# yzslab/gaussian-splatting-lightning

Hardware: AMD Instinct MI355X
Metric: training images/sec + fwd/bwd ms @1080p, 1M Gaussians, 1/2/4/8 MI355X (higher is better)
Workload: dtype f32

## Files before the change

gaussian-splatting-lightning_amd/csrc/composite_bwd.hip:

```cpp
#include "gspl_composite.h"

namespace gspl {

template <int D> struct BwdRec { static constexpr int STRIDE = 8 + ((D + 1 + 3) & ~3); static constexpr int HC = 8 + D; };

#ifndef GSPL_BWD2_CHUNK
#define GSPL_BWD2_CHUNK 64
#endif
#ifndef GSPL_BWD2_WAVES
#define GSPL_BWD2_WAVES 5
#endif
static constexpr int B2CHUNK = GSPL_BWD2_CHUNK;
static constexpr int P2_SLOTS = 4;
static constexpr int B2_NW = 2;
static constexpr int B2_NT = 64 * B2_NW;
static_assert(B2CHUNK <= B2_NT || B2_NW == 2, "a round is staged by one pass of the workgroup's threads");


template <int D, int MODE, bool CHW, bool ABS, bool PACKED, int SEGM = 0>
__global__ __launch_bounds__(B2_NT, GSPL_BWD2_WAVES) void composite_bwd2_kernel(
    int n_tiles, int tile_w, int width, int height, int64_t n_isects,
    const float* __restrict__ means2d, const float* __restrict__ conics, const float* __restrict__ colors,
    const float* __restrict__ opacities, const float* __restrict__ backgrounds,
    const int32_t* __restrict__ offsets, const int32_t* __restrict__ flatten_ids,
    const float* __restrict__ final_Ts, const int32_t* __restrict__ last_ids,
    const float* __restrict__ v_out_colors, const float* __restrict__ v_out_alphas,
    float* __restrict__ v_means2d, float* __restrict__ v_means2d_abs,
    float* __restrict__ v_conics, float* __restrict__ v_colors, float* __restrict__ v_opacities, int packed_stride,
    uint8_t* __restrict__ hit_flags, SegState seg) {
    using TR = ModeTraits<MODE>;
    constexpr int NV = BwdVals<D, ABS>::N;
    constexpr int RS = BwdRec<D>::STRIDE;
    constexpr bool VO_REGS = D <= 4;
    constexpr int SLAB = 2 * P2_SLOTS * 128;
    static_assert(NV <= 16, "one ds_add round per batch");
    __shared__ int s_id[B2CHUNK];
    __shared__ __attribute__((aligned(16))) float s_rec[B2CHUNK * RS];
    __shared__ float s_acc[B2CHUNK * NV];
    __shared__ __attribute__((aligned(16))) float s_slab[B2_NW * SLAB];
    __shared__ __attribute__((aligned(16))) float s_vo_keep[VO_REGS ? 4 : B2_NW * 128 * D];
    static_assert(!VO_REGS || B2_NW * 128 * D <= B2_NW * SLAB, "s_vo alias too small");
    float* s_vo = VO_REGS ? s_slab : s_vo_keep;
    __shared__ int s_last;

    const int t = threadIdx.x, w = t >> 6, l = t & 63;
    const int ws = w;
    int tile = 0, segidx = 0;
    if constexpr (SEGM == 2) {
        if (blockIdx.x >= min(*seg.count(), seg.slots)) return;
        const uint32_t item = seg.work()[blockIdx.x];
        tile = (int)(item >> 8); segidx = (int)(item & 255u);
    } else {
        tile = xcd_remap(blockIdx.x, n_tiles);
    }
    {
    const int tx = (tile % tile_w) * TILE, ty = (tile / tile_w) * TILE;
    const int pxA = tx + (l & 7), pxB = pxA + 8;
    const int py = ty + w * 8 + (l >> 3);
    const bool insideA = (pxA < width) && (py < height), insideB = (pxB < width) && (py < height);
    const v2f pxf2 = {(float)pxA + TR::kPixelCentre, (float)pxB + TR::kPixelCentre};
    const float pyf = (float)py + TR::kPixelCentre;
    const float hx0 = (float)tx + TR::kPixelCentre;
    const float hy0 = (float)(ty + w * 8) + TR::kPixelCentre;
    const int64_t pixA = (int64_t)py * width + pxA, pixB = pixA + 8;
    const int tl = (l & 7) * 8 + (l >> 3);
    constexpr int TLB = 64;
    const int ps = l >> 4, pc = l & 15;
    float* slab = s_slab + ws * SLAB;

    int start, end;
    tile_range(tile, n_tiles, n_isects, offsets, start, end);

    const int lastA = insideA ? last_ids[pixA] : start, lastB = insideB ? last_ids[pixB] : start;
    v2f T2 = {insideA ? final_Ts[pixA] : 1.f, insideB ? final_Ts[pixB] : 1.f};
    v2f vo[D];
    v2f bgdot = {0.f, 0.f};
#pragma unroll
    for (int c = 0; c < D; ++c) {
        vo[c] = (v2f){0.f, 0.f};
        if (insideA) vo[c].x = CHW ? v_out_colors[(int64_t)c * width * height + pixA] : v_out_colors[pixA * D + c];
        if (insideB) vo[c].y = CHW ? v_out_colors[(int64_t)c * width * height + pixB] : v_out_colors[pixB * D + c];
        if (backgrounds) bgdot += backgrounds[c] * vo[c];
        s_vo[((ws * 16 + (l & 7)) * D + c) * 8 + (l >> 3)] = vo[c].x;
        s_vo[((ws * 16 + 8 + (l & 7)) * D + c) * 8 + (l >> 3)] = vo[c].y;
    }
    const v2f v_out_a = {(insideA && v_out_alphas) ? v_out_alphas[pixA] : 0.f, (insideB && v_out_alphas) ? v_out_alphas[pixB] : 0.f};
    v2f R2 = T2 * (v_out_a - bgdot);

    if (t == 0) s_last = start;
    for (int k = t; k < B2CHUNK * NV; k += B2_NT) s_acc[k] = 0.f;
    __syncthreads();
    v2f vo2[VO_REGS ? 4 : 1][VO_REGS ? D : 1];
    if constexpr (VO_REGS) {
#pragma unroll
        for (int c = 0; c < D; ++c) {
            const float4* vp = reinterpret_cast<const float4*>(s_vo + ((ws * 16 + pc) * D + c) * 8);
            const float4 v0 = vp[0], v1 = vp[1];
            vo2[0][c] = (v2f){v0.x, v0.y}; vo2[1][c] = (v2f){v0.z, v0.w};
            vo2[2][c] = (v2f){v1.x, v1.y}; vo2[3][c] = (v2f){v1.z, v1.w};
        }
    }
    int wl = max(lastA, lastB);
#pragma unroll
    for (int off = 32; off > 0; off >>= 1) wl = max(wl, __shfl_xor(wl, off));
    if (l == 0) atomicMax(&s_last, wl);
    __syncthreads();
    const int block_last = s_last;
    const int wave_last = wl;
    int seg_lo = start, seg_hi = block_last;
    if constexpr (SEGM != 2) {
        if (seg.walk && t == 0 && block_last > start) {
            uint32_t* row = seg.walk + (size_t)((unsigned)tile & (SEG_WALK_SLOTS - 1)) * 4u;
            atomicAdd(row + 0, (uint32_t)(block_last - start));
            atomicMax(row + 1, (uint32_t)(block_last - start));
            atomicAdd(row + 2, 1u);
        }
    }
    if constexpr (SEGM != 0) {
        const int walked = block_last - start;
        const int nseg = walked > 0 ? min((walked + SEG - 1) >> SEG_LOG2, SEG_MAX) : 0;
        if constexpr (SEGM == 1) {
            if (nseg > 1 && t == 0) {
                const uint32_t pos = atomicAdd(seg.count(), (uint32_t)(nseg - 1));
                for (int sgm = 1; sgm < nseg; ++sgm)
                    if (pos + (uint32_t)(sgm - 1) < seg.slots) seg.work()[pos + (uint32_t)(sgm - 1)] = ((uint32_t)tile << 8) | (uint32_t)sgm;
            }
        }
        if (nseg > 1) {
            seg_lo = start + segidx * SEG;
            seg_hi = (segidx + 1 < nseg) ? start + (segidx + 1) * SEG : block_last;
            if (seg_hi < block_last) {
                const size_t slot = (size_t)((unsigned)seg_hi >> SEG_LOG2) * 256u;
                const int lasts[2] = {lastA, lastB};
                float Tn[2] = {T2.x, T2.y}, Rn[2] = {R2.x, R2.y};
#pragma unroll
                for (int e = 0; e < 2; ++e) {
                    if (lasts[e] > seg_hi) {
                        const float4 ck = seg.ckpt[slot + (unsigned)((2 * w + e) * 64 + l)];
                        const float ckc[4] = {ck.y, ck.z, ck.w, D == 4 ? seg.ckpt_x[slot + (unsigned)((2 * w + e) * 64 + l)] : 0.f};
                        float behind = 0.f;
#pragma unroll
                        for (int c = 0; c < D; ++c) behind = fmaf(e == 0 ? vo[c].x : vo[c].y, ckc[c < 4 ? c : 0], behind);
                        Tn[e] = ck.x;
                        Rn[e] = Rn[e] - behind;
                    }
                }
                T2 = (v2f){Tn[0], Tn[1]}; R2 = (v2f){Rn[0], Rn[1]};
            }
        } else if (segidx > 0) {
            seg_lo = seg_hi = start;
        }
    }

    int nb = 0;
    int batch_j = 0;

    auto phase2 = [&](int count) {
        __builtin_amdgcn_wave_barrier();
        float vals[NV];
#pragma unroll
        for (int k = 0; k < NV; ++k) vals[k] = 0.f;
        const int j = __builtin_amdgcn_ds_bpermute(ps << 2, batch_j);
        const bool live = ps < count;
        float ca = 0.f, cb = 0.f, cc_ = 0.f, co_ = 1.f;
        if (live) {
            const float* rec = s_rec + j * RS;
            const float4 r0 = *reinterpret_cast<const float4*>(rec);
            const float4 r1 = *reinterpret_cast<const float4*>(rec + 4);
            ca = 2.f * r0.z; cb = r1.w; cc_ = 2.f * rec[BwdRec<D>::HC]; co_ = r1.y;
            const float dx = r0.x - (hx0 + (float)pc);
            const float dy0 = r0.y - hy0;
            const v2f dy0v = {dy0, dy0};
            const float4* Fp = reinterpret_cast<const float4*>(slab + ps * 128 + pc * 8);
            const float4* Sp = reinterpret_cast<const float4*>(slab + P2_SLOTS * 128 + ps * 128 + pc * 8);
            const float4 f0 = Fp[0], f1 = Fp[1], q0 = Sp[0], q1 = Sp[1];
            const v2f F2[4] = {{f0.x, f0.y}, {f0.z, f0.w}, {f1.x, f1.y}, {f1.z, f1.w}};
            const v2f S2[4] = {{q0.x, q0.y}, {q0.z, q0.w}, {q1.x, q1.y}, {q1.z, q1.w}};
            v2f s02 = {0.f, 0.f}, sy2 = {0.f, 0.f}, syy2 = {0.f, 0.f};
            v2f rgb2[D];
            float ax = 0.f, ay = 0.f;
#pragma unroll
            for (int c = 0; c < D; ++c) rgb2[c] = (v2f){0.f, 0.f};
#pragma unroll
            for (int k = 0; k < 4; ++k) {
                const v2f dy2 = dy0v - (v2f){(float)(2 * k), (float)(2 * k + 1)};
#pragma unroll
                for (int c = 0; c < D; ++c) {
                    v2f vv;
                    if constexpr (VO_REGS) vv = vo2[k][c];
                    else vv = *reinterpret_cast<const v2f*>(s_vo + ((ws * 16 + pc) * D + c) * 8 + 2 * k);
                    rgb2[c] = __builtin_elementwise_fma(F2[k], vv, rgb2[c]);
                }
                s02 += S2[k];
                const v2f tq = S2[k] * dy2;
                sy2 += tq;
                syy2 = __builtin_elementwise_fma(tq, dy2, syy2);
                if constexpr (ABS) {
                    ax += fabsf(S2[k].x * (ca * dx + cb * dy2.x)) + fabsf(S2[k].y * (ca * dx + cb * dy2.y));
                    ay += fabsf(S2[k].x * (cb * dx + cc_ * dy2.x)) + fabsf(S2[k].y * (cb * dx + cc_ * dy2.y));
                }
            }
            const float S0 = s02.x + s02.y, Sy = sy2.x + sy2.y;
            const float Sx = S0 * dx;
            vals[0] = ca * Sx + cb * Sy;
            vals[1] = cb * Sx + cc_ * Sy;
            vals[2] = 0.5f * (Sx * dx);
            vals[3] = Sy * dx;
            vals[4] = 0.5f * (syy2.x + syy2.y);
            vals[5] = (co_ != 0.f) ? -S0 * __builtin_amdgcn_rcpf(co_) : 0.f;
#pragma unroll
            for (int c = 0; c < D; ++c) vals[6 + c] = rgb2[c].x + rgb2[c].y;
            if constexpr (ABS) { vals[6 + D] = ax; vals[7 + D] = ay; }
        }
#pragma unroll
        for (int k = 0; k < NV; ++k) {
            vals[k] = dpp_add<0xB1, 0xF>(vals[k]);
            vals[k] = dpp_add<0x4E, 0xF>(vals[k]);
        }
        constexpr int NK = (NV + 3) / 4;
        const int pq = pc & 3;
        float kept[NK];
#pragma unroll
        for (int m = 0; m < NK; ++m) {
            float v = vals[4 * m];
#pragma unroll
            for (int q = 1; q < 4; ++q) v = (pq == q) ? ((4 * m + q < NV) ? vals[(4 * m + q < NV) ? 4 * m + q : 0] : 0.f) : v;
            kept[m] = dpp_add<0x124, 0xF>(v);
        }
        row_ror8_add<NK>(kept);
#pragma unroll
        for (int m = 0; m < NK; ++m)
            if (live && pc < 4 && 4 * m + pc < NV) atomicAdd(&s_acc[j * NV + 4 * m + pc], kept[m]);
    };

    int g_next = (seg_hi - 1 - t >= seg_lo && t < B2CHUNK) ? flatten_ids[seg_hi - 1 - t] : 0;
    for (int hi = seg_hi; hi > seg_lo; hi -= B2CHUNK) {
        const int lo = max(seg_lo, hi - B2CHUNK);
        const int cnt = hi - lo;
        const int g = g_next;
        {
            const int i_next = hi - B2CHUNK - 1 - t;
            if (i_next >= seg_lo && t < B2CHUNK) g_next = flatten_ids[i_next];
        }
        if (t < cnt) {
            s_id[t] = g;
            const float ca = conics[g * 3 + 0], cb = conics[g * 3 + 1], cc = conics[g * 3 + 2], op = opacities[g];
            const float mx = means2d[g * 2 + 0], my = means2d[g * 2 + 1];
            const unsigned qm = band_half_mask<2>(mx, my, ca, cb, cc, op, (float)tx + TR::kPixelCentre, (float)ty + TR::kPixelCentre);
            float* rec = s_rec + t * RS;
            const SigmaCoef sc = sigma_coef(ca, cb, cc);
            *reinterpret_cast<float4*>(rec) = make_float4(mx, my, sc.ha, sc.k);
            *reinterpret_cast<float4*>(rec + 4) = make_float4(sc.hd, op, __uint_as_float(qm), cb);
#pragma unroll
            for (int c = 0; c < D; ++c) rec[8 + c] = colors[(int64_t)g * D + c];
            rec[BwdRec<D>::HC] = 0.5f * cc;
        }
        __syncthreads();
        if (wave_last > lo) {
#pragma unroll 1
            for (int kk = 0; kk < (B2CHUNK + 63) / 64; ++kk) {
                const int slot = kk * 64 + l;
                const unsigned qm = (slot < B2CHUNK) ? __float_as_uint(s_rec[slot * RS + 6]) : 0u;
                const bool cand = (slot < cnt) && (hi - 1 - slot < wave_last) && ((qm >> (2 * w)) & 3u);
                unsigned long long mask = __ballot(cand);
                while (mask) {
                    const int j = kk * 64 + (int)__builtin_ctzll(mask);
                    mask &= mask - 1;
                    const int idx = hi - 1 - j;
                    const float* rec = s_rec + j * RS;
                    const float4 r0 = *reinterpret_cast<const float4*>(rec);
                    const float2 r1 = *reinterpret_cast<const float2*>(rec + 4);
                    float col[D];
#pragma unroll
                    for (int c = 0; c < D; ++c) col[c] = rec[8 + c];
                    const v2f dx2 = (v2f){r0.x, r0.x} - pxf2;
                    const float dy = r0.y - pyf;
                    const float e = (r1.x * dy) * dy;
                    const v2f u2 = __builtin_elementwise_fma((v2f){r0.w, r0.w}, (v2f){dy, dy}, dx2);
                    const v2f sigma2 = __builtin_elementwise_fma((v2f){r0.z, r0.z} * u2, u2, (v2f){e, e});
                    const v2f arg2 = sigma2 * (v2f){-1.4426950408889634f, -1.4426950408889634f};
                    const v2f vis2 = {__builtin_amdgcn_exp2f(arg2.x), __builtin_amdgcn_exp2f(arg2.y)};
                    const v2f raw2 = (v2f){r1.y, r1.y} * vis2;
                    const bool validA = (idx < lastA) && (sigma2.x >= 0.f) && (raw2.x >= kAlphaMin);
                    const bool validB = (idx < lastB) && (sigma2.y >= 0.f) && (raw2.y >= kAlphaMin);
                    if (!__any(validA || validB)) continue;
                    if (hit_flags && l == 0) atomicOr(&s_id[j], (int)0x80000000);
                    const v2f rv2 = {validA ? raw2.x : 0.f, validB ? raw2.y : 0.f};
                    const v2f a2 = {fminf(TR::kAlphaMax, rv2.x), fminf(TR::kAlphaMax, rv2.y)};
                    v2f rw2 = rv2;
                    if (TR::kClampKillsGrad) rw2 = (v2f){(rv2.x <= TR::kAlphaMax) ? rv2.x : 0.f, (rv2.y <= TR::kAlphaMax) ? rv2.y : 0.f};
                    const v2f om2 = (v2f){1.f, 1.f} - a2;
                    v2f ra2 = {__builtin_amdgcn_rcpf(om2.x), __builtin_amdgcn_rcpf(om2.y)};
                    ra2 = __builtin_elementwise_fma(ra2, __builtin_elementwise_fma(-om2, ra2, (v2f){1.f, 1.f}), ra2);
                    T2 *= ra2;
                    const v2f fac2 = a2 * T2;
                    v2f cdot2 = (v2f){col[0], col[0]} * vo[0];
#pragma unroll
                    for (int c = 1; c < D; ++c) cdot2 = __builtin_elementwise_fma((v2f){col[c], col[c]}, vo[c], cdot2);
                    const v2f v_alpha2 = __builtin_elementwise_fma(cdot2, T2, R2 * ra2);
                    R2 = __builtin_elementwise_fma(-cdot2, fac2, R2);
                    const v2f sp2 = -rw2 * v_alpha2;
                    float* F = slab + nb * 128 + tl;
                    F[0] = fac2.x; F[TLB] = fac2.y;
                    F[P2_SLOTS * 128] = sp2.x; F[P2_SLOTS * 128 + TLB] = sp2.y;
                    batch_j = gspl_writelane_i32(j, nb, batch_j);
                    if (++nb == P2_SLOTS) { phase2(P2_SLOTS); nb = 0; }
                }
            }
            if (nb) { phase2(nb); nb = 0; }
        }
        __syncthreads();
        if constexpr (PACKED) {
            float* __restrict__ v_packed = v_means2d;
            const bool by_entry = packed_stride < 0;
            const int ps = by_entry ? -packed_stride : packed_stride;
            for (int e = t; e < cnt * NV; e += B2_NT) {
                const float v = s_acc[e];
                s_acc[e] = 0.f;
                const int row = e / NV;
                const int64_t dst_row = by_entry ? (int64_t)(hi - 1 - row) : (int64_t)(s_id[row] & 0x7fffffff);
                if (v != 0.f) atomicAdd(&v_packed[dst_row * ps + (e - row * NV)], v);
            }
        } else if (t < cnt) {
            const int g = s_id[t] & 0x7fffffff;
            float v[NV];
            bool any_nz = false;
#pragma unroll
            for (int k = 0; k < NV; ++k) {
                v[k] = s_acc[t * NV + k];
                s_acc[t * NV + k] = 0.f;
                any_nz = any_nz || (v[k] != 0.f);
            }
            if (any_nz) {
                atomicAdd(&v_means2d[g * 2 + 0], v[0]);
                atomicAdd(&v_means2d[g * 2 + 1], v[1]);
                atomicAdd(&v_conics[g * 3 + 0], v[2]);
                atomicAdd(&v_conics[g * 3 + 1], v[3]);
                atomicAdd(&v_conics[g * 3 + 2], v[4]);
                atomicAdd(&v_opacities[g], v[5]);
#pragma unroll
                for (int c = 0; c < D; ++c) atomicAdd(&v_colors[(int64_t)g * D + c], v[6 + c]);
                if constexpr (ABS) {
                    atomicAdd(&v_means2d_abs[g * 2 + 0], v[6 + D]);
                    atomicAdd(&v_means2d_abs[g * 2 + 1], v[7 + D]);
                }
            }
        }
        if (hit_flags && t < cnt && s_id[t] < 0) hit_flags[s_id[t] & 0x7fffffff] = 1;
        __syncthreads();
    }
    }
}

template <int D, int MODE, bool CHW, bool ABS, bool PACKED>
__global__ __launch_bounds__(64) void composite_bwd_block_kernel(
    int n_tiles, int tile_w, int width, int height, int64_t n_isects,
    const float* __restrict__ means2d, const float* __restrict__ conics, const float* __restrict__ colors,
    const float* __restrict__ opacities, const float* __restrict__ backgrounds,
    const int32_t* __restrict__ offsets, const int32_t* __restrict__ flatten_ids,
    const float* __restrict__ final_Ts, const int32_t* __restrict__ last_ids,
    const float* __restrict__ v_out_colors, const float* __restrict__ v_out_alphas,
    float* __restrict__ v_means2d, float* __restrict__ v_means2d_abs,
    float* __restrict__ v_conics, float* __restrict__ v_colors, float* __restrict__ v_opacities, int packed_stride,
    uint8_t* __restrict__ hit_flags, ListTiles lt) {
    using TR = ModeTraits<MODE>;
    constexpr int NV = BwdVals<D, ABS>::N;
    __shared__ float s_x[64], s_y[64], s_ha[64], s_b[64], s_hc[64], s_op[64], s_k[64], s_hd[64];
    __shared__ float s_col[64 * D];
    __shared__ int s_g[64], s_idx[64];

    const int unit = xcd_remap(blockIdx.x, 4 * n_tiles, 4 * GSPL_XCD_RUN);
    const int tile = unit >> 2, w = unit & 3, l = threadIdx.x;
    const int bx = (tile % tile_w) * 2 + (w & 1), by = (tile / tile_w) * 2 + (w >> 1);
    const int px = bx * 8 + (l & 7), py = by * 8 + (l >> 3);
    const bool inside = (px < width) && (py < height);
    const float pxf = (float)px + TR::kPixelCentre, pyf = (float)py + TR::kPixelCentre;
    const float qx0 = (float)(bx * 8) + TR::kPixelCentre, qy0 = (float)(by * 8) + TR::kPixelCentre;
    int start, end;
    block_list_range(lt, bx, by, width, height, n_isects, offsets, start, end);

    const int64_t pix = (int64_t)py * width + px;
    const int last = inside ? last_ids[pix] : start;
    float T = inside ? final_Ts[pix] : 1.f;
    float vo[D];
    float bgdot = 0.f;
#pragma unroll
    for (int c = 0; c < D; ++c) {
        vo[c] = inside ? (CHW ? v_out_colors[(int64_t)c * width * height + pix] : v_out_colors[pix * D + c]) : 0.f;
        if (backgrounds) bgdot += backgrounds[c] * vo[c];
    }
    float R = T * (((inside && v_out_alphas) ? v_out_alphas[pix] : 0.f) - bgdot);
    int block_last = last;
#pragma unroll
    for (int off = 32; off > 0; off >>= 1) block_last = max(block_last, __shfl_xor(block_last, off));

    for (int hi = block_last; hi > start; hi -= 64) {
        const int idx = hi - 1 - l;
        bool cand = false;
        int g = 0;
        float mx = 0.f, my = 0.f, ca = 0.f, cb = 0.f, cc = 0.f, op = 0.f;
        if (idx >= start) {
            g = flatten_ids[idx];
            ca = conics[g * 3 + 0]; cb = conics[g * 3 + 1]; cc = conics[g * 3 + 2]; op = opacities[g];
            mx = means2d[g * 2 + 0]; my = means2d[g * 2 + 1];
            cand = box_reachable(mx, my, ca, cb, cc, op, qx0, qx0 + 7.f, qy0, qy0 + 7.f);
        }
        const unsigned long long mask = __ballot(cand);
        const int ncand = __builtin_popcountll(mask);
        const int slot = __builtin_amdgcn_mbcnt_hi((unsigned)(mask >> 32), __builtin_amdgcn_mbcnt_lo((unsigned)mask, 0u));
        __syncthreads();
        if (cand) {
            const SigmaCoef sc = sigma_coef(ca, cb, cc);
            s_x[slot] = mx; s_y[slot] = my; s_ha[slot] = sc.ha; s_b[slot] = cb; s_hc[slot] = 0.5f * cc; s_op[slot] = op;
            s_k[slot] = sc.k; s_hd[slot] = sc.hd;
            s_g[slot] = g; s_idx[slot] = idx;
#pragma unroll
            for (int c = 0; c < D; ++c) s_col[slot * D + c] = colors[(int64_t)g * D + c];
        }
        __syncthreads();
        for (int k = 0; k < ncand; ++k) {
            const int kidx = s_idx[k];
            const float ha = s_ha[k], b = s_b[k], hc = s_hc[k], o = s_op[k];
            const float dx = s_x[k] - pxf, dy = s_y[k] - pyf;
            const float sigma = eval_sigma(ha, s_k[k], s_hd[k], dx, dy);
            const float vis = __builtin_amdgcn_exp2f(sigma * -1.4426950408889634f);
            const float raw = o * vis;
            const bool valid = (kidx < last) && (sigma >= 0.f) && (raw >= kAlphaMin);
            if (!__any(valid)) continue;
            const float rv = valid ? raw : 0.f;
            const float a = fminf(TR::kAlphaMax, rv);
            float rw = rv;
            if (TR::kClampKillsGrad) rw = (rv <= TR::kAlphaMax) ? rv : 0.f;
            const float om = 1.f - a;
            float ra = __builtin_amdgcn_rcpf(om);
            ra = fmaf(ra, fmaf(-om, ra, 1.f), ra);
            T *= ra;
            const float fac = a * T;
            float cdot = s_col[k * D] * vo[0];
#pragma unroll
            for (int c = 1; c < D; ++c) cdot = fmaf(s_col[k * D + c], vo[c], cdot);
            const float v_alpha = fmaf(cdot, T, R * ra);
            R = fmaf(-cdot, fac, R);
            const float sp = -rw * v_alpha;
            const float fa = 2.f * ha, fc = 2.f * hc;
            float vals[NV];
            vals[0] = sp * fmaf(fa, dx, b * dy);
            vals[1] = sp * fmaf(b, dx, fc * dy);
            vals[2] = 0.5f * sp * dx * dx;
            vals[3] = sp * dx * dy;
            vals[4] = 0.5f * sp * dy * dy;
            vals[5] = (o != 0.f) ? -sp * __builtin_amdgcn_rcpf(o) : 0.f;
#pragma unroll
            for (int c = 0; c < D; ++c) vals[6 + c] = fac * vo[c];
            if constexpr (ABS) { vals[6 + D] = fabsf(vals[0]); vals[7 + D] = fabsf(vals[1]); }
#pragma unroll
            for (int v = 0; v < NV; ++v) vals[v] = wave_sum_to_lane63(vals[v]);
            if (l == 63) {
                const int gk = s_g[k];
                if constexpr (PACKED) {
                    float* row = v_means2d + (int64_t)gk * packed_stride;
#pragma unroll
                    for (int v = 0; v < NV; ++v) if (vals[v] != 0.f) atomicAdd(&row[v], vals[v]);
                } else {
                    atomicAdd(&v_means2d[gk * 2 + 0], vals[0]);
                    atomicAdd(&v_means2d[gk * 2 + 1], vals[1]);
                    atomicAdd(&v_conics[gk * 3 + 0], vals[2]);
                    atomicAdd(&v_conics[gk * 3 + 1], vals[3]);
                    atomicAdd(&v_conics[gk * 3 + 2], vals[4]);
                    atomicAdd(&v_opacities[gk], vals[5]);
#pragma unroll
                    for (int c = 0; c < D; ++c) atomicAdd(&v_colors[(int64_t)gk * D + c], vals[6 + c]);
                    if constexpr (ABS) {
                        atomicAdd(&v_means2d_abs[gk * 2 + 0], vals[6 + D]);
                        atomicAdd(&v_means2d_abs[gk * 2 + 1], vals[7 + D]);
                    }
                }
                if (hit_flags) hit_flags[gk] = 1;
            }
        }
    }
}

template <int D, int MODE, bool CHW, bool PACKED = false>
static int launch_bwd(bool absgrad, int n_tiles, int tile_w, ImageSize image, const CompositeSplats& sp, const TileLists& lists,
                      const float* final_Ts, const int32_t* last_ids,
                      const float* v_out_colors, const float* v_out_alphas,
                      float* v_means2d, float* v_means2d_abs, float* v_conics, float* v_colors, float* v_opacities,
                      hipStream_t s, int packed_stride, uint8_t* hit_flags, ListTiles lt, const SegState* seg_in = nullptr) {
#define GSPL_BWD_ARGS n_tiles, tile_w, image.width, image.height, lists.n_isects, sp.means2d, sp.conics, sp.colors, sp.opacities, sp.backgrounds, \
                      lists.offsets, lists.flatten_ids, final_Ts, last_ids, v_out_colors, v_out_alphas, v_means2d, v_means2d_abs, v_conics, v_colors, v_opacities,   \
                      packed_stride, hit_flags
    if (lt.log2 != 4) {
        if (absgrad) hipLaunchKernelGGL((composite_bwd_block_kernel<D, MODE, CHW, true, PACKED>), dim3(4 * n_tiles), dim3(64), 0, s, GSPL_BWD_ARGS, lt);
        else hipLaunchKernelGGL((composite_bwd_block_kernel<D, MODE, CHW, false, PACKED>), dim3(4 * n_tiles), dim3(64), 0, s, GSPL_BWD_ARGS, lt);
        return check_launch("composite_bwd");
    }
    SegState plain = {};
    if (seg_in) { plain.host_flag = seg_in->host_flag; plain.walk = seg_in->walk; }
    if constexpr ((D == 3 || (D == 4 && MODE == GSPL_MODE_INRIA)) && CHW && PACKED) {
        if (seg_in && seg_in->ckpt && (D == 3 || seg_in->ckpt_x) && !absgrad && packed_stride > 0) {
            hipLaunchKernelGGL((composite_bwd2_kernel<D, MODE, CHW, false, PACKED, 1>), dim3(n_tiles), dim3(B2_NT), 0, s, GSPL_BWD_ARGS, *seg_in);
            hipLaunchKernelGGL((composite_bwd2_kernel<D, MODE, CHW, false, PACKED, 2>), dim3(seg_in->slots), dim3(B2_NT), 0, s, GSPL_BWD_ARGS, *seg_in);
            return check_launch("composite_bwd(segmented)");
        }
    }
    if (absgrad) hipLaunchKernelGGL((composite_bwd2_kernel<D, MODE, CHW, true, PACKED>), dim3(n_tiles), dim3(B2_NT), 0, s, GSPL_BWD_ARGS, plain);
    else hipLaunchKernelGGL((composite_bwd2_kernel<D, MODE, CHW, false, PACKED>), dim3(n_tiles), dim3(B2_NT), 0, s, GSPL_BWD_ARGS, plain);
#undef GSPL_BWD_ARGS
    return check_launch("composite_bwd");
}

}

extern "C" int gspl_composite_bwd(int N, int64_t n_isects, int D, int mode, int layout,
                                  const float* means2d, const float* conics, const float* colors,
                                  const float* opacities, const float* backgrounds,
                                  int width, int height, int tile_size, int tile_w, int tile_h,
                                  const int32_t* offsets, const int32_t* flatten_ids,
                                  const float* final_Ts, const int32_t* last_ids,
                                  const float* v_out_colors, const float* v_out_alphas,
                                  float* v_means2d, float* v_means2d_abs,
                                  float* v_conics, float* v_colors, float* v_opacities, uint8_t* hit_flags, void* stream) {
    using namespace gspl;
    const ImageSize image{width, height};
    const TileGrid grid{tile_size, tile_w, tile_h};
    int rc = check_composite_args(N, n_isects, D, mode, layout, image, grid, "composite_bwd: bad argument");
    if (rc != GSPL_OK) return rc;
    if (n_isects == 0 || N == 0) return GSPL_OK;
    if (!means2d || !conics || !colors || !opacities || !offsets || !flatten_ids || !final_Ts || !last_ids ||
        !v_out_colors || !v_means2d || !v_conics || !v_colors || !v_opacities)
        return fail_arg("composite_bwd: NULL required pointer");
    const ListTiles lt = list_tiles(grid);
    const int ctw = (width + TILE - 1) / TILE, n_tiles = ctw * ((height + TILE - 1) / TILE);
    hipStream_t s = (hipStream_t)stream;
    const bool absgrad = v_means2d_abs != nullptr;
    return dispatch_composite(D, mode, layout, [&](auto d, auto m, auto chw) {
        return launch_bwd<d(), m(), chw()>(absgrad, n_tiles, ctw, image, CompositeSplats{means2d, conics, colors, opacities, backgrounds},
                                           TileLists{offsets, flatten_ids, n_isects}, final_Ts, last_ids, v_out_colors, v_out_alphas, v_means2d, v_means2d_abs, v_conics, v_colors, v_opacities, s, 0,
                                           hit_flags, lt);
    });
}

#include "gspl_sort.h"
namespace gspl {
static int g_deterministic = 0;

__global__ __launch_bounds__(256) void iota_ids_kernel(int64_t n, const int32_t* __restrict__ ids, uint32_t* __restrict__ keys, uint32_t* __restrict__ pos) {
    const int64_t i = (int64_t)blockIdx.x * 256 + threadIdx.x;
    if (i < n) { keys[i] = (uint32_t)ids[i]; pos[i] = (uint32_t)i; }
}
static constexpr int ORDERED_MAX_NV = 18;
__global__ __launch_bounds__(256) void ordered_reduce_kernel(int64_t n, const uint32_t* __restrict__ keys, const uint32_t* __restrict__ pos,
                                                             const float* __restrict__ entries, int nv, float* __restrict__ rows, int row_stride) {
    const int64_t i = (int64_t)blockIdx.x * 256 + threadIdx.x;
    if (i >= n) return;
    const uint32_t g = keys[i];
    if (i > 0 && keys[i - 1] == g) return;
    float acc[ORDERED_MAX_NV];
#pragma unroll
    for (int k = 0; k < ORDERED_MAX_NV; ++k) acc[k] = 0.f;
    for (int64_t j = i; j < n && keys[j] == g; ++j) {
        const float* row = entries + (int64_t)pos[j] * nv;
#pragma unroll
        for (int k = 0; k < ORDERED_MAX_NV; ++k) if (k < nv) acc[k] += row[k];
    }
    float* out = rows + (int64_t)g * row_stride;
#pragma unroll
    for (int k = 0; k < ORDERED_MAX_NV; ++k) if (k < nv) out[k] += acc[k];
}

OrderedScratch ordered_scratch(int N, int64_t n_isects, int nv) {
    OrderedScratch o;
    o.id_bits = 1;
    while (o.id_bits < 32 && (1ll << o.id_bits) < (long long)N) ++o.id_bits;
    o.sort_ws_bytes = gspl_radix_sort_workspace_bytes(n_isects, 4, 0, o.id_bits);
    Carve c;
    (void)c.take((size_t)n_isects * nv * sizeof(float));
    o.keys = c.take((size_t)n_isects * 4 * sizeof(uint32_t));
    o.sort_ws = c.take(o.sort_ws_bytes ? o.sort_ws_bytes : 16);
    o.total = c.off;
    return o;
}

int ordered_reduce(int N, int64_t n_isects, int nv, const int32_t* flatten_ids, void* block, float* rows, int row_stride, hipStream_t s, const char* who) {
    if (nv > ORDERED_MAX_NV) return fail_arg(who);
    const OrderedScratch o = ordered_scratch(N, n_isects, nv);
    uint32_t *k0 = (uint32_t*)((char*)block + o.keys), *k1 = k0 + n_isects, *p0 = k1 + n_isects, *p1 = p0 + n_isects;
    const unsigned grid = (unsigned)((n_isects + 255) / 256);
    hipLaunchKernelGGL(iota_ids_kernel, dim3(grid), dim3(256), 0, s, n_isects, flatten_ids, k0, p0);
    int which = 0;
    const int rc = gspl_radix_sort_pairs_u32(n_isects, k0, k1, p0, p1, 0, o.id_bits, &which, (char*)block + o.sort_ws, o.sort_ws_bytes, s);
    if (rc != GSPL_OK) return rc;
    hipLaunchKernelGGL(ordered_reduce_kernel, dim3(grid), dim3(256), 0, s, n_isects, which ? k1 : k0, which ? p1 : p0,
                       (const float*)block, nv, rows, row_stride);
    return check_launch(who);
}
}

extern "C" int gspl_set_deterministic(int on) { const int was = gspl::g_deterministic; gspl::g_deterministic = on ? 1 : 0; return was; }
extern "C" int gspl_get_deterministic(void) { return gspl::g_deterministic; }

extern "C" int gspl_composite_bwd_packed(int N, int64_t n_isects, int D, int mode, int layout,
                                         const float* means2d, const float* conics, const float* colors,
                                         const float* opacities, const float* backgrounds,
                                         int width, int height, int tile_size, int tile_w, int tile_h,
                                         const int32_t* offsets, const int32_t* flatten_ids,
                                         const float* final_Ts, const int32_t* last_ids,
                                         const float* v_out_colors, const float* v_out_alphas,
                                         float* v_packed, int packed_stride, int absgrad, uint8_t* hit_flags, void* stream) {
    using namespace gspl;
    return composite_bwd_packed_impl(N, D, mode, layout, CompositeSplats{means2d, conics, colors, opacities, backgrounds}, ImageSize{width, height},
                                     TileGrid{tile_size, tile_w, tile_h}, TileLists{offsets, flatten_ids, n_isects}, final_Ts, last_ids, v_out_colors,
                                     v_out_alphas, v_packed, packed_stride, absgrad, hit_flags, stream, nullptr);
}

int gspl::composite_bwd_packed_impl(int N, int D, int mode, int layout, const CompositeSplats& sp, ImageSize image, TileGrid grid, const TileLists& lists,
                                    const float* final_Ts, const int32_t* last_ids, const float* v_out_colors, const float* v_out_alphas,
                                    float* v_packed, int packed_stride, int absgrad, uint8_t* hit_flags, void* stream, const SegState* seg) {
    using namespace gspl;
    const int64_t n_isects = lists.n_isects;
    int rc = check_composite_args(N, n_isects, D, mode, layout, image, grid, "composite_bwd_packed: bad argument");
    if (rc != GSPL_OK) return rc;
    if (packed_stride < 6 + D + (absgrad ? 2 : 0)) return fail_arg("composite_bwd_packed: packed_stride smaller than the row");
    if (n_isects == 0 || N == 0) return GSPL_OK;
    if (!sp.means2d || !sp.conics || !sp.colors || !sp.opacities || !lists.offsets || !lists.flatten_ids || !final_Ts || !last_ids || !v_out_colors || !v_packed)
        return fail_arg("composite_bwd_packed: NULL required pointer");
    const ListTiles lt = list_tiles(grid);
    const int ctw = (image.width + TILE - 1) / TILE, n_tiles = ctw * ((image.height + TILE - 1) / TILE);
    hipStream_t s = (hipStream_t)stream;
    const bool ag = absgrad != 0;
    const int nv = 6 + D + (ag ? 2 : 0);
    const bool ordered = gspl_get_deterministic() != 0 && lt.log2 == 4 && n_isects > 0;
    float* entries = nullptr;
    float* const v_packed_out = v_packed;
    const int packed_stride_out = packed_stride;
    if (ordered) {
        if (n_isects < 0) return fail_arg("composite_bwd_packed: the deterministic mode needs the list length on the host (n_isects >= 0)");
        hipError_t e = hipMallocAsync((void**)&entries, ordered_scratch(N, n_isects, nv).total, s);
        if (e == hipSuccess) e = hipMemsetAsync(entries, 0, (size_t)n_isects * nv * sizeof(float), s);
        if (e != hipSuccess) return check_hip(e, "composite_bwd_packed(deterministic): scratch");
        v_packed = entries;
        packed_stride = -nv;
        seg = nullptr;
    }
    rc = dispatch_composite(D, mode, layout, [&](auto d, auto m, auto chw) {
        return launch_bwd<d(), m(), chw(), true>(ag, n_tiles, ctw, image, sp, lists,
                                                 final_Ts, last_ids, v_out_colors, v_out_alphas, v_packed, nullptr, nullptr, nullptr, nullptr, s, packed_stride,
                                                 hit_flags, lt, seg);
    });
    if (ordered) {
        if (rc == GSPL_OK) rc = ordered_reduce(N, n_isects, nv, lists.flatten_ids, entries, v_packed_out, packed_stride_out, s, "composite_bwd_packed(ordered reduce)");
        (void)hipFreeAsync(entries, s);
    }
    return rc;
}

extern "C" const char* gspl_composite_bwd_kernel_name(void) { return "composite_bwd2_kernel"; }
```

gaussian-splatting-lightning_amd/csrc/fused.hip:

```cpp
#include <cstdlib>
#include <cstring>
#include <mutex>
#include <unordered_map>
#include <utility>
#include <vector>
#include "gspl_composite.h"
#include "gspl_sort.h"

namespace gspl {

struct GeomLayout {
    size_t radii, means2d, depths, conics, colors, clamped, cov3d, sh_jac, order, cum, big_list, spans, opac, colors4, total;
};
static GeomLayout geom_layout(size_t n, bool invdepth = false) {
    GeomLayout g;
    Carve c;
    g.means2d = c.take(8 * n); g.depths = c.take(4 * n); g.conics = c.take(12 * n); g.colors = c.take(12 * n);
    g.clamped = c.take(3 * n); g.cov3d = c.take(24 * n); g.sh_jac = c.take(36 * n);
    g.order = c.take(4 * n); g.cum = c.take(8 * (n + 1)); g.big_list = c.take(4 * n); g.spans = c.take((size_t)GSPL_BIN_SPAN_BYTES * n);
    g.opac = c.take(4 * n);
    g.colors4 = invdepth ? c.take(16 * n) : 0;
    g.radii = 0;
    g.total = c.off;
    return g;
}
struct ImageLayout { size_t alphas, final_Ts, last_ids, offsets, total; };
static ImageLayout image_layout(size_t pixels, size_t tiles) {
    ImageLayout m;
    Carve c;
    m.alphas = c.take(4 * pixels); m.final_Ts = c.take(4 * pixels); m.last_ids = c.take(4 * pixels); m.offsets = c.take(4 * (tiles + 1));
    m.total = c.off;
    return m;
}

static bool wait_for_ticket(const int64_t* host, unsigned long long ticket, hipStream_t s) {
    const volatile unsigned long long* flag = (const volatile unsigned long long*)(host + 2);
    for (unsigned spins = 1;; ++spins) {
        if (__atomic_load_n((const unsigned long long*)flag, __ATOMIC_ACQUIRE) == ticket) return true;
        __builtin_ia32_pause();
        if ((spins & 0xffffu) == 0u) {
            const hipError_t q = hipStreamQuery(s);
            if (q == hipSuccess) return __atomic_load_n((const unsigned long long*)flag, __ATOMIC_ACQUIRE) == ticket;
            if (q != hipErrorNotReady) { (void)hipGetLastError(); return false; }
        }
    }
}
template <class T>
struct PerDevice {
    std::mutex mu;
    T slot[64] = {};
    bool ready[64] = {};
    template <class R, class Init, class F>
    R with(R fallback, Init&& init, F&& f) {
        int dev = 0;
        if (hipGetDevice(&dev) != hipSuccess || dev < 0 || dev >= 64) return fallback;
        std::lock_guard<std::mutex> lk(mu);
        if (!ready[dev]) {
            if (!init(slot[dev])) { (void)hipGetLastError(); return fallback; }
            ready[dev] = true;
        }
        return f(slot[dev]);
    }
};

static constexpr unsigned SEG_RING = 16;
struct SegAdaptive {
    uint32_t* ring = nullptr;
    uint32_t slot_ticket[SEG_RING] = {};
    uintptr_t slot_view[SEG_RING] = {};
    uint32_t next = 1;
    uintptr_t prev_view = 0;
    int sticky = 0;
    std::unordered_map<uintptr_t, uint8_t> verdict;
};
static PerDevice<SegAdaptive> g_seg;
static bool seg_decide(bool force, uintptr_t view, uint32_t** slot_out, uint32_t* ticket_out) {
    *slot_out = nullptr; *ticket_out = 0u;
    auto ring = [](SegAdaptive& a) {
        void* q = nullptr;
        if (hipHostMalloc(&q, SEG_RING * sizeof(uint32_t), hipHostMallocDefault) != hipSuccess) return false;
        a.ring = (uint32_t*)q;
        for (unsigned i = 0; i < SEG_RING; ++i) a.ring[i] = 0u;
        return true;
    };
    return g_seg.with(force, ring, [&](SegAdaptive& a) {
        for (unsigned i = 0; i < SEG_RING; ++i) {
            if (!a.slot_ticket[i]) continue;
            const uint32_t v = __atomic_load_n(a.ring + i, __ATOMIC_RELAXED);
            if ((v >> 1) != (a.slot_ticket[i] & 0x7fffffffu)) continue;
            const bool tail = (v & 1u) != 0u;
            if (a.slot_view[i]) {
                if (a.verdict.size() > 65536) a.verdict.clear();
                a.verdict[a.slot_view[i]] = tail ? 1 : 0;
            }
            if (tail) a.sticky = 64;
            a.slot_ticket[i] = 0u;
        }
        bool on = force;
        const auto it = view ? a.verdict.find(view) : a.verdict.end();
        if (it != a.verdict.end()) on = on || it->second != 0;
        else on = on || a.sticky > 0;
        if (a.sticky > 0) --a.sticky;
        const unsigned slot = a.next % SEG_RING;
        const uint32_t ticket = a.next & 0x7fffffffu;
        ++a.next; if ((a.next & 0x7fffffffu) == 0u) a.next = 1;
        a.slot_ticket[slot] = ticket;
        a.slot_view[slot] = a.prev_view;
        a.prev_view = view;
        *slot_out = a.ring + slot; *ticket_out = ticket;
        return on;
    });
}
static PerDevice<uint32_t*> g_seg_walk;
static uint32_t* seg_walk_words() {
    auto zeroed = [](uint32_t*& words) {
        void* q = nullptr;
        const size_t bytes = (size_t)SEG_WALK_SLOTS * 4 * sizeof(uint32_t);
        if (hipMalloc(&q, bytes) != hipSuccess || hipMemset(q, 0, bytes) != hipSuccess || hipDeviceSynchronize() != hipSuccess) {
            if (q) (void)hipFree(q);
            return false;
        }
        words = (uint32_t*)q;
        return true;
    };
    return g_seg_walk.with((uint32_t*)nullptr, zeroed, [](uint32_t* words) { return words; });
}

static unsigned long long next_ticket() {
    static thread_local unsigned long long t = 0ull;
    return ++t;
}

#ifndef GSPL_EVENT_FLAGS
#define GSPL_EVENT_FLAGS hipEventDisableTiming
#endif
struct FrameEvents { hipEvent_t geo = nullptr, col = nullptr, cnt = nullptr, fork = nullptr, filled = nullptr; bool ok = false; };
static FrameEvents& frame_events() {
    static thread_local FrameEvents ev;
    if (!ev.ok)
        ev.ok = hipEventCreateWithFlags(&ev.geo, GSPL_EVENT_FLAGS) == hipSuccess && hipEventCreateWithFlags(&ev.col, GSPL_EVENT_FLAGS) == hipSuccess &&
                hipEventCreateWithFlags(&ev.cnt, hipEventDisableTiming) == hipSuccess &&
                hipEventCreateWithFlags(&ev.fork, GSPL_EVENT_FLAGS) == hipSuccess && hipEventCreateWithFlags(&ev.filled, GSPL_EVENT_FLAGS) == hipSuccess;
    return ev;
}

static PerDevice<hipStream_t> g_low_priority_streams;
extern "C" void* gspl_low_priority_stream(void) {
    auto create = [](hipStream_t& st) {
        int least = 0, greatest = 0;
        (void)hipDeviceGetStreamPriorityRange(&least, &greatest);
        if (hipStreamCreateWithPriority(&st, hipStreamNonBlocking, least) == hipSuccess) return true;
        st = nullptr;
        return false;
    };
    return g_low_priority_streams.with((void*)nullptr, create, [](hipStream_t st) { return (void*)st; });
}

struct ProfSlot { std::vector<std::pair<hipEvent_t, hipEvent_t>> ev; };
static int g_prof_period[2] = {0, 0};
static unsigned g_prof_seen[2] = {0u, 0u};
static std::mutex g_prof_mu;
static ProfSlot g_prof[2];
struct ProfScope {
    int which; hipStream_t s; hipEvent_t a = nullptr, b = nullptr;
    ProfScope(int w, hipStream_t st) : which(w), s(st) {
        if (g_prof_period[w] <= 0) return;
        if ((g_prof_seen[w]++ % (unsigned)g_prof_period[w]) != 0u) return;
        if (hipEventCreate(&a) != hipSuccess || hipEventCreate(&b) != hipSuccess) { a = b = nullptr; return; }
        (void)hipEventRecord(a, s);
    }
    ~ProfScope() {
        if (!a) return;
        (void)hipEventRecord(b, s);
        std::lock_guard<std::mutex> lk(g_prof_mu);
        g_prof[which].ev.emplace_back(a, b);
    }
};

}

extern "C" int gspl_profile_enable2(int period_fwd, int period_bwd) {
    std::lock_guard<std::mutex> lk(gspl::g_prof_mu);
    gspl::g_prof_period[0] = period_fwd > 0 ? period_fwd : 0;
    gspl::g_prof_period[1] = period_bwd > 0 ? period_bwd : 0;
    gspl::g_prof_seen[0] = gspl::g_prof_seen[1] = 0u;
    for (auto& slot : gspl::g_prof) {
        for (auto& e : slot.ev) { (void)hipEventDestroy(e.first); (void)hipEventDestroy(e.second); }
        slot.ev.clear();
    }
    return GSPL_OK;
}

extern "C" int gspl_profile_enable(int period) { return gspl_profile_enable2(period, period); }

extern "C" int gspl_profile_read(int which, int* count, float* total_ms) {
    using namespace gspl;
    if (which < 0 || which > 1 || !count || !total_ms) return fail_arg("profile_read: bad argument");
    std::lock_guard<std::mutex> lk(g_prof_mu);
    float tot = 0.f;
    for (auto& e : g_prof[which].ev) {
        float ms = 0.f;
        if (hipEventSynchronize(e.second) != hipSuccess || hipEventElapsedTime(&ms, e.first, e.second) != hipSuccess) return check_hip(hipGetLastError(), "profile_read");
        tot += ms;
    }
    *count = (int)g_prof[which].ev.size();
    *total_ms = tot;
    return GSPL_OK;
}

extern "C" size_t gspl_rasterize_inria_geometry_bytes(int N) { return gspl::geom_layout((size_t)(N > 0 ? N : 1)).total; }
extern "C" size_t gspl_rasterize_inria_image_bytes(int width, int height) {
    return gspl::image_layout((size_t)width * height, (size_t)((width + 15) / 16) * ((height + 15) / 16)).total;
}

namespace gspl {

static void carve_inria_state(gspl_inria_state* st, char* geom, const GeomLayout& g, char* img, const ImageLayout& im) {
    st->means2d = (float*)(geom + g.means2d); st->depths = (float*)(geom + g.depths); st->conics = (float*)(geom + g.conics);
    st->colors = (float*)(geom + g.colors); st->clamped = (uint8_t*)(geom + g.clamped); st->cov3d = (float*)(geom + g.cov3d);
    st->sh_jac = (float*)(geom + g.sh_jac);
    st->alphas = (float*)(img + im.alphas); st->final_Ts = (float*)(img + im.final_Ts); st->last_ids = (int32_t*)(img + im.last_ids);
    st->offsets = (int32_t*)(img + im.offsets);
}

struct TicketWait {
    const int64_t* host; hipStream_t s;
    const unsigned long long ticket = next_ticket();
    bool waited = false, arrived = false;
    TicketWait(const int64_t* h, hipStream_t st) : host(h), s(st) {}
    TicketWait(const TicketWait&) = delete;
    bool wait() {
        if (!waited) { arrived = wait_for_ticket(host, ticket, s); waited = true; }
        return arrived;
    }
    ~TicketWait() { (void)wait(); }
};
static int list_length_never_arrived(hipStream_t s) {
    const char* what = "rasterize_inria_fwd: the list length never arrived";
    return check_hip(hipStreamSynchronize(s), what) ? GSPL_ERR_LAUNCH : fail_arg(what);
}

struct SegPlan {
    bool adaptive = false, want = false;
    uint32_t* verdict_slot = nullptr;
    uint32_t verdict_ticket = 0u;
    uint4* packed_zero = nullptr;
    uint32_t packed_n16 = 0u;
    SegState seg = {};
    void ask_packed_rows(size_t row_bytes, gspl_alloc_fn alloc, void* alloc_ctx, gspl_inria_state* st) {
        const size_t bytes = (row_bytes + 15) & ~(size_t)15;
        packed_zero = (uint4*)alloc(alloc_ctx, GSPL_BUF_PACKED, bytes);
        if (packed_zero && bytes / 16 <= 0xffffffffull) { packed_n16 = (uint32_t)(bytes / 16); st->flags |= GSPL_INRIA_PACKED_READY; }
        else packed_zero = nullptr;
    }
    const SegState* for_capacity(int64_t cap, bool invd, gspl_alloc_fn alloc, void* alloc_ctx, gspl_inria_state* st) {
        seg = SegState{};
        seg.zero_p = packed_zero; seg.zero_n16 = packed_n16;
        if (adaptive) { seg.walk = seg_walk_words(); seg.host_flag = verdict_slot; seg.ticket = verdict_ticket; }
        st->seg_ckpt = nullptr; st->seg_words = nullptr; st->seg_slots = 0u;
        if (!want || cap <= SEG) return (adaptive || packed_zero) ? &seg : nullptr;
        const uint32_t slots = (uint32_t)(cap >> SEG_LOG2) + 2u;
        const size_t words = 2 + (size_t)slots;
        const size_t head = up256(words * sizeof(uint32_t));
        char* blk = (char*)alloc(alloc_ctx, GSPL_BUF_CHECKPOINTS, head + (size_t)slots * 256 * (sizeof(float4) + (invd ? sizeof(float) : 0)));
        if (!blk) return (adaptive || packed_zero) ? &seg : nullptr;
        uint32_t* wds = (uint32_t*)blk;
        seg.words = wds; seg.slots = slots;
        seg.ckpt = (float4*)(blk + head);
        seg.ckpt_x = invd ? (float*)(seg.ckpt + (size_t)slots * 256) : nullptr;
        st->seg_ckpt = seg.ckpt; st->seg_words = wds; st->seg_slots = slots;
        return &seg;
    }
};

static int inria_colours_launch(int N, const InriaParams& p, const InriaCamera& cam, const float* colors_precomp, int32_t* radii, gspl_inria_state* st,
                                float* colors3, hipStream_t s, hipStream_t ss, hipEvent_t* ev_col) {
    FrameEvents& fe = frame_events();
    if (!fe.ok) return check_hip(hipGetLastError(), "rasterize_inria_fwd: event");
    const bool side = ss && ss != s;
    if (side) {
        (void)hipEventRecord(fe.geo, s);
        (void)hipStreamWaitEvent(ss, fe.geo, 0);
    }
    hipStream_t cs = side ? ss : s;
    int rc = gspl_inria_preprocess_fwd(N, p.degree, p.n_coeffs, p.means, p.scales, p.quats, p.cov3d, p.shs, p.shs_rest, colors_precomp, cam.viewmatrix,
                                       cam.projmatrix, cam.campos, cam.width, cam.height, 16, cam.tanfovx, cam.tanfovy, cam.scale_modifier, radii, st->means2d,
                                       st->depths, st->conics, colors3, st->clamped, st->cov3d, st->sh_jac, GSPL_INRIA_COLOURS, cs);
    if (rc == GSPL_OK && (st->flags & GSPL_INRIA_INVDEPTH)) rc = inria_invdepth_rows_launch(N, radii, colors3, st->depths, st->colors, cs);
    if (rc == GSPL_OK && side) { (void)hipEventRecord(fe.col, cs); *ev_col = fe.col; }
    return rc;
}

static int inria_composite_launch(int N, int D, const gspl_inria_state* st, const float* bg, int64_t n_isects, float* out_color,
                                  hipEvent_t ev_col, hipStream_t s, const SegState* sg) {
    if (ev_col) (void)hipStreamWaitEvent(s, ev_col, 0);
    ProfScope prof(0, s);
    return composite_fwd_impl(N, D, GSPL_MODE_INRIA, GSPL_LAYOUT_CHW, CompositeSplats{st->means2d, st->conics, st->colors, st->opacities, bg},
                              ImageSize{st->width, st->height}, tile_grid16(st->width, st->height), TileLists{st->offsets, st->flatten_ids, n_isects},
                              out_color, st->alphas, st->final_Ts, st->last_ids, nullptr, s, sg);
}

}

extern "C" int gspl_rasterize_inria_fwd(
    int N, int degree, int n_coeffs,
    const float* means3D, const float* scales, const float* rotations, const float* cov3D_precomp,
    const float* shs, const float* shs_rest, const float* colors_precomp, const float* opacities,
    const float* viewmatrix, const float* projmatrix, const float* campos, const float* bg,
    int width, int height, float tanfovx, float tanfovy, float scale_modifier,
    gspl_alloc_fn alloc, void* alloc_ctx, int64_t capacity_hint,
    float* out_color, int32_t* radii, gspl_inria_state* st, void* stream, void* side_stream) {
    using namespace gspl;
    const char* no_block = "rasterize_inria_fwd: allocation call-back returned NULL";
    if (N < 0 || width <= 0 || height <= 0 || !alloc || !st || !out_color) return fail_arg("rasterize_inria_fwd: bad argument");
    if (N > 0 && (!means3D || !opacities || !radii || !viewmatrix || !projmatrix || !campos)) return fail_arg("rasterize_inria_fwd: NULL required pointer");
    const TileGrid grid = tile_grid16(width, height);
    hipStream_t s = (hipStream_t)stream, ss = (hipStream_t)side_stream;
    const int flags = st->flags;
    if (flags & ~(GSPL_INRIA_RAW_PARAMS | GSPL_INRIA_NO_SEGMENTS | GSPL_INRIA_FORCE_SEGMENTS | GSPL_INRIA_WILL_BACKWARD | GSPL_INRIA_ANTIALIAS |
                  GSPL_INRIA_INVDEPTH)) return fail_arg("rasterize_inria_fwd: unknown state->flags (zero the struct before the call)");
    const bool raw = (flags & GSPL_INRIA_RAW_PARAMS) != 0;
    const bool aa = (flags & GSPL_INRIA_ANTIALIAS) != 0, invd = (flags & GSPL_INRIA_INVDEPTH) != 0;
    const int D = invd ? 4 : 3;
    const int prow = invd ? 10 : 9;
    if (raw && (cov3D_precomp || (N > 0 && (!scales || !rotations)))) return fail_arg("rasterize_inria_fwd: raw parameters need scales and rotations");
    memset(st, 0, sizeof(*st));
    st->flags = flags;
    st->N = N; st->width = width; st->height = height;
    const size_t n = (size_t)(N > 0 ? N : 1);
    const GeomLayout g = geom_layout(n, invd);
    const ImageLayout im = image_layout((size_t)width * height, (size_t)grid.n());
    char* geom = (char*)alloc(alloc_ctx, GSPL_BUF_GEOMETRY, g.total);
    char* img = (char*)alloc(alloc_ctx, GSPL_BUF_IMAGE, im.total);
    if (!geom || !img) return fail_arg(no_block);
    carve_inria_state(st, geom, g, img, im);
    float* colors3 = st->colors;
    if (invd) st->colors = (float*)(geom + g.colors4);
    const float* raw_opacities = (raw || aa) ? opacities : nullptr;
    if (raw || aa) opacities = (float*)(geom + g.opac);
    st->opacities = const_cast<float*>(opacities);
    SegPlan plan;
    plan.adaptive = !(flags & GSPL_INRIA_NO_SEGMENTS) && gspl_get_deterministic() == 0;
    plan.want = plan.adaptive && seg_decide((flags & GSPL_INRIA_FORCE_SEGMENTS) != 0, (uintptr_t)viewmatrix, &plan.verdict_slot, &plan.verdict_ticket);
    if ((flags & GSPL_INRIA_WILL_BACKWARD) && N > 0) plan.ask_packed_rows((size_t)N * prow * sizeof(float), alloc, alloc_ctx, st);
    const BinSplats bins{N, GSPL_MODE_INRIA, st->means2d, radii, st->depths, st->conics, opacities};
    const BinOrder ord{(int32_t*)(geom + g.order), (int64_t*)(geom + g.cum), (int32_t*)(geom + g.big_list), geom + g.spans};
    if (N == 0) {
        const int rc = bin_lists_known(BinSplats{0, GSPL_MODE_INRIA}, BinOrder{}, grid, 0, alloc, alloc_ctx, &st->flatten_ids, st->offsets, s, "rasterize_inria_fwd");
        return rc != GSPL_OK ? rc : inria_composite_launch(N, D, st, bg, 0, out_color, nullptr, s, nullptr);
    }
    const size_t ws1_bytes = gspl_bin_workspace_bytes(N, 0);
    char* ws1 = (char*)alloc(alloc_ctx, GSPL_BUF_BINNING, ws1_bytes);
    if (!ws1) return fail_arg(no_block);
    const int64_t capacity = capacity_hint > 0 ? capacity_hint : 0;
    const size_t ws2_bytes = capacity ? gspl_bin_workspace_bytes(N, capacity) : 0;
    char* ws2 = capacity ? (char*)alloc(alloc_ctx, GSPL_BUF_LISTS_WORK, ws2_bytes) : nullptr;
    if (capacity && !ws2) return fail_arg(no_block);
    int64_t* host = pinned_words();
    if (!host) return fail_arg("rasterize_inria_fwd: no pinned host word");
    if (!viewmatrix || !projmatrix) return fail_arg("rasterize_inria_fwd: NULL required pointer");
    if (!cov3D_precomp && (!scales || !rotations)) return fail_arg("rasterize_inria_fwd: need scales+rotations or cov3D_precomp");
    ZeroJob zero_depth, zero_tile;
    int rc = bin_depth_header(N, grid.n(), ws1, zero_depth);
    if (rc == GSPL_OK && ws2) rc = bin_tile_header(N, capacity, grid.n(), ws2, zero_tile);
    if (rc != GSPL_OK) return rc;
    const InriaParams params{means3D, scales, rotations, cov3D_precomp, shs, shs_rest, degree, n_coeffs};
    const InriaCamera cam{viewmatrix, projmatrix, campos, width, height, tanfovx, tanfovy, scale_modifier};
    rc = inria_geometry_launch(N, params, cam, grid.size, radii, st->means2d, st->depths, st->conics, st->cov3d, raw_opacities, st->opacities, s, zero_depth,
                               flags & (GSPL_INRIA_RAW_PARAMS | GSPL_INRIA_ANTIALIAS));
    if (rc != GSPL_OK) return rc;
    hipEvent_t ev_col = nullptr;
    rc = inria_colours_launch(N, params, cam, colors_precomp, radii, st, colors3, s, ss, &ev_col);
    if (rc != GSPL_OK) return rc;
    TicketWait scan(host, s);
    rc = bin_count_ticket(bins, grid, ord, host, ws1, ws1_bytes, s, scan.ticket, true, zero_tile);
    if (rc != GSPL_OK) return rc;
    int64_t n_isects = 0;
    if (ws2) {
        rc = bin_emit_impl(bins, ord, grid, capacity, ws2, ws2_bytes, s, true);
        if (rc != GSPL_OK) return rc;
        st->flatten_ids = (int32_t*)alloc(alloc_ctx, GSPL_BUF_LISTS, 4 * (size_t)capacity);
        if (!st->flatten_ids) return fail_arg(no_block);
        const SegState* sg = plan.for_capacity(capacity, invd, alloc, alloc_ctx, st);
        rc = gspl_bin_sort_device_count(N, grid.w, grid.h, ord.cum + (N - 1), capacity, st->flatten_ids, st->offsets, ws2, ws2_bytes, s);
        if (rc != GSPL_OK) return rc;
        rc = inria_composite_launch(N, D, st, bg, -1, out_color, ev_col, s, sg);
        const bool arrived = scan.wait();
        n_isects = host[0];
        if (rc != GSPL_OK) return rc;
        if (!arrived) return list_length_never_arrived(s);
        if (n_isects <= capacity) { st->n_isects = n_isects; return GSPL_OK; }
    } else {
        if (!scan.wait()) return list_length_never_arrived(s);
        n_isects = host[0];
    }
    rc = bin_lists_known(bins, ord, grid, n_isects, alloc, alloc_ctx, &st->flatten_ids, st->offsets, s, "rasterize_inria_fwd");
    if (rc != GSPL_OK) return rc;
    st->n_isects = n_isects;
    return inria_composite_launch(N, D, st, bg, n_isects, out_color, ev_col, s, plan.for_capacity(n_isects, invd, alloc, alloc_ctx, st));
}

namespace gspl {
#ifndef GSPL_FILL_BLOCKS
#define GSPL_FILL_BLOCKS 32
#endif
static int fill_blocks() {
    static const int n = [] { const char* e = getenv("GSPL_FILL_BLOCKS"); const int v = e ? atoi(e) : 0; return v > 0 && v <= 65536 ? v : GSPL_FILL_BLOCKS; }();
    return n;
}
struct FillJob {
    struct Span { float* p; uint64_t n; } a[9];
    int count = 0;
    void add(float* p, uint64_t n) { if (p && n) a[count++] = Span{p, n}; }
};
__global__ __launch_bounds__(256) void zero_fill_kernel(FillJob job) {
    typedef float v4f __attribute__((ext_vector_type(4)));
    const uint64_t tid = (uint64_t)blockIdx.x * 256 + threadIdx.x, stride = (uint64_t)gridDim.x * 256;
    for (int k = 0; k < job.count; ++k) {
        float* p = job.a[k].p;
        const uint64_t n = job.a[k].n;
        const uint64_t head = min(n, (uint64_t)(((16u - (unsigned)((uintptr_t)p & 15u)) & 15u) >> 2));
        const uint64_t n4 = (n - head) >> 2, tail0 = head + (n4 << 2);
        v4f* q = reinterpret_cast<v4f*>(p + head);
        const v4f z = {0.f, 0.f, 0.f, 0.f};
        for (uint64_t i = tid; i < n4; i += stride) __builtin_nontemporal_store(z, q + i);
        if (tid < head) p[tid] = 0.f;
        if (tid < n - tail0) p[tail0 + tid] = 0.f;
    }
}
struct FillJoin {
    hipStream_t s; hipEvent_t ev = nullptr;
    explicit FillJoin(hipStream_t st) : s(st) {}
    FillJoin(const FillJoin&) = delete;
    void join() { if (ev) (void)hipStreamWaitEvent(s, ev, 0); ev = nullptr; }
    ~FillJoin() { join(); }
};
static int zero_grads_beside(int N, const InriaParams& p, const InriaGrads& v, hipStream_t s, FillJoin& fill) {
    FillJob job;
    const uint64_t n = (uint64_t)N, sh_rows = (uint64_t)(p.n_coeffs > 0 ? p.n_coeffs : 0);
    job.add(v.means, 3 * n); job.add(v.means2d_ndc, 3 * n); job.add(v.opacities, n);
    job.add(v.scales, 3 * n); job.add(v.quats, 4 * n); job.add(v.cov3d_precomp, 6 * n); job.add(v.colors_precomp, 3 * n);
    if (v.shs_rest) { job.add(v.shs, 3 * n); job.add(v.shs_rest, 3 * (sh_rows > 0 ? sh_rows - 1 : 0) * n); }
    else job.add(v.shs, 3 * sh_rows * n);
    FrameEvents& fe = frame_events();
    if (!fe.ok) return check_hip(hipGetLastError(), "rasterize_inria_bwd: event");
    hipStream_t ls = (hipStream_t)gspl_low_priority_stream();
    const bool side = ls && ls != s;
    if (side) {
        (void)hipEventRecord(fe.fork, s);
        (void)hipStreamWaitEvent(ls, fe.fork, 0);
    }
    hipLaunchKernelGGL(zero_fill_kernel, dim3(fill_blocks()), dim3(256), 0, side ? ls : s, job);
    const int rc = check_launch("rasterize_inria_bwd: clear the gradients");
    if (side) { (void)hipEventRecord(fe.filled, ls); fill.ev = fe.filled; }
    return rc;
}

static int rasterize_inria_bwd_impl(InriaParams p, const float* opacities, InriaCamera cam, const float* bg,
                                    const int32_t* radii, const gspl_inria_state* st, const float* v_out_color,
                                    float* packed , uint8_t* hit_flags,
                                    const InriaGrads& v, void* stream, const gspl_bwd_adam_plan* plan, uint8_t* grad_rows = nullptr) {
    if (!st || st->N < 0) return fail_arg("rasterize_inria_bwd: bad state");
    const int N = st->N;
    if (N == 0) return GSPL_OK;
    if (!packed || !v_out_color || !v.means || !v.means2d_ndc || !v.opacities) return fail_arg("rasterize_inria_bwd: NULL required pointer");
    cam.width = st->width; cam.height = st->height;
    p.cov3d = st->cov3d;
    hipStream_t s = (hipStream_t)stream;
    hipError_t e = hipSuccess;
    const bool aa = (st->flags & GSPL_INRIA_ANTIALIAS) != 0, invd = (st->flags & GSPL_INRIA_INVDEPTH) != 0;
    const int D = invd ? 4 : 3, prow = invd ? 10 : 9;
    const float* caller_opacities = opacities;
    FillJoin fill(s);
    if (grad_rows) {
        if (plan) return fail_arg("rasterize_inria_bwd: grad_rows and the optimizer inside the backward exclude each other");
        const int rc = zero_grads_beside(N, p, v, s, fill);
        if (rc != GSPL_OK) return rc;
    }
    if (!(st->flags & GSPL_INRIA_PACKED_READY)) {
        e = hipMemsetAsync(packed, 0, (size_t)N * prow * sizeof(float), s);
        if (e != hipSuccess) return check_hip(e, "rasterize_inria_bwd: clear");
    }
    if (hit_flags) {
        e = hipMemsetAsync(hit_flags, 0, (size_t)N, s);
        if (e != hipSuccess) return check_hip(e, "rasterize_inria_bwd: clear");
    }
    const bool raw = (st->flags & GSPL_INRIA_RAW_PARAMS) != 0;
    if (raw) {
        if (!st->opacities || !v.scales || !v.quats) return fail_arg("rasterize_inria_bwd: raw parameters need the forward's state, v_scales and v_rotations");
        opacities = st->opacities;
    }
    if (aa) {
        if (!st->opacities) return fail_arg("rasterize_inria_bwd: anti-aliasing needs the forward's state");
        opacities = st->opacities;
    }
    if (st->n_isects > 0) {
        SegState seg = {};
        if (st->seg_ckpt && st->seg_words) {
            seg.ckpt = (float4*)st->seg_ckpt;
            seg.words = st->seg_words; seg.slots = st->seg_slots;
            if (invd) seg.ckpt_x = (float*)(seg.ckpt + (size_t)seg.slots * 256);
        }
        if (!(st->flags & GSPL_INRIA_NO_SEGMENTS) && gspl_get_deterministic() == 0) seg.walk = seg_walk_words();
        ProfScope prof(1, s);
        const int rc = composite_bwd_packed_impl(N, D, GSPL_MODE_INRIA, GSPL_LAYOUT_CHW, CompositeSplats{st->means2d, st->conics, st->colors, opacities, bg},
                                                 ImageSize{cam.width, cam.height}, tile_grid16(cam.width, cam.height),
                                                 TileLists{st->offsets, st->flatten_ids, st->n_isects}, st->final_Ts, st->last_ids, v_out_color, nullptr,
                                                 packed, prow, 0, hit_flags, s, &seg);
        if (rc != GSPL_OK) return rc;
    }
    fill.join();
    return inria_preprocess_bwd_impl(N, p, cam, radii, st->clamped, SplatGradRows::packed(packed, prow), v, st->sh_jac,
                                     aa ? caller_opacities : (raw ? st->opacities : nullptr), s, plan, BwdStats{st->stats_accum, st->stats_denom, st->stats_max_radii},
                                     st->flags & (GSPL_INRIA_RAW_PARAMS | GSPL_INRIA_ANTIALIAS | GSPL_INRIA_INVDEPTH), grad_rows);
}
}

extern "C" int gspl_rasterize_inria_bwd(
    int degree, int n_coeffs,
    const float* means3D, const float* scales, const float* rotations, const float* shs, const float* shs_rest, const float* opacities,
    const float* viewmatrix, const float* projmatrix, const float* campos, const float* bg,
    float tanfovx, float tanfovy, float scale_modifier,
    const int32_t* radii, const gspl_inria_state* st, const float* v_out_color,
    float* packed, uint8_t* hit_flags,
    float* v_means3D, float* v_means2D_ndc, float* v_shs, float* v_shs_rest, float* v_colors_precomp, float* v_opacities,
    float* v_scales, float* v_rotations, float* v_cov3D, void* stream) {
    using namespace gspl;
    return rasterize_inria_bwd_impl(InriaParams{means3D, scales, rotations, nullptr, shs, shs_rest, degree, n_coeffs}, opacities,
                                    InriaCamera{viewmatrix, projmatrix, campos, 0, 0, tanfovx, tanfovy, scale_modifier}, bg, radii, st, v_out_color, packed, hit_flags,
                                    InriaGrads{v_means3D, v_scales, v_rotations, v_cov3D, v_shs, v_shs_rest, v_colors_precomp, v_means2D_ndc, v_opacities}, stream, nullptr);
}

extern "C" int gspl_rasterize_inria_bwd_sparse(
    int degree, int n_coeffs,
    const float* means3D, const float* scales, const float* rotations, const float* shs, const float* shs_rest, const float* opacities,
    const float* viewmatrix, const float* projmatrix, const float* campos, const float* bg,
    float tanfovx, float tanfovy, float scale_modifier,
    const int32_t* radii, const gspl_inria_state* st, const float* v_out_color,
    float* packed, uint8_t* hit_flags,
    float* v_means3D, float* v_means2D_ndc, float* v_shs, float* v_shs_rest, float* v_colors_precomp, float* v_opacities,
    float* v_scales, float* v_rotations, float* v_cov3D, uint8_t* grad_rows, void* stream) {
    using namespace gspl;
    if (!grad_rows) return fail_arg("rasterize_inria_bwd_sparse: NULL grad_rows");
    return rasterize_inria_bwd_impl(InriaParams{means3D, scales, rotations, nullptr, shs, shs_rest, degree, n_coeffs}, opacities,
                                    InriaCamera{viewmatrix, projmatrix, campos, 0, 0, tanfovx, tanfovy, scale_modifier}, bg, radii, st, v_out_color, packed, hit_flags,
                                    InriaGrads{v_means3D, v_scales, v_rotations, v_cov3D, v_shs, v_shs_rest, v_colors_precomp, v_means2D_ndc, v_opacities}, stream, nullptr,
                                    grad_rows);
}

extern "C" int gspl_rasterize_inria_bwd_adam(
    int degree, int n_coeffs,
    float* means3D, float* scales, float* rotations, float* shs, float* shs_rest, float* opacities,
    const float* viewmatrix, const float* projmatrix, const float* campos, const float* bg,
    float tanfovx, float tanfovy, float scale_modifier,
    const int32_t* radii, const gspl_inria_state* st, const float* v_out_color,
    float* packed, uint8_t* hit_flags, float* scratch_means, float* v_means2D_ndc, const gspl_bwd_adam_plan* plan, void* stream) {
    using namespace gspl;
    if (!plan) return fail_arg("rasterize_inria_bwd_adam: NULL plan");
    if (!scales || !rotations || !shs || !opacities) return fail_arg("rasterize_inria_bwd_adam: needs scales, rotations, SH coefficients and opacities");
    if (st && (st->flags & (GSPL_INRIA_ANTIALIAS | GSPL_INRIA_INVDEPTH)))
        return fail_arg("rasterize_inria_bwd_adam: a frame rendered with GSPL_INRIA_ANTIALIAS or GSPL_INRIA_INVDEPTH takes gspl_rasterize_inria_bwd and a separate optimizer");
    return rasterize_inria_bwd_impl(InriaParams{means3D, scales, rotations, nullptr, shs, shs_rest, degree, n_coeffs}, opacities,
                                    InriaCamera{viewmatrix, projmatrix, campos, 0, 0, tanfovx, tanfovy, scale_modifier}, bg, radii, st, v_out_color, packed, hit_flags,
                                    InriaGrads{scratch_means, scales, rotations, nullptr, shs, shs_rest, nullptr, v_means2D_ndc, opacities}, stream, plan);
}
```

gaussian-splatting-lightning_amd/csrc/gspl_composite.h:

```cpp
#pragma once
#include "gspl_device.h"
#include "gspl_host.h"

namespace gspl {

static constexpr int TILE = 16;

typedef float v2f __attribute__((ext_vector_type(2)));

struct SigmaCoef { float ha, k, hd; };
__device__ __forceinline__ SigmaCoef sigma_coef(float a, float b, float c) {
    SigmaCoef s;
    s.ha = 0.5f * a;
    if (a != 0.f) {
        s.k = b / a;
        s.hd = (0.5f * conic_det(a, b, c)) * __builtin_amdgcn_rcpf(a);
    } else {
        s.k = 0.f;
        s.hd = (b == 0.f) ? 0.5f * c : __builtin_nanf("");
    }
    return s;
}
__device__ __forceinline__ float eval_sigma(float ha, float k, float hd, float dx, float dy) {
    const float u = fmaf(k, dy, dx);
    return fmaf(ha * u, u, (hd * dy) * dy);
}

__device__ __forceinline__ v2f eval_sigma2(v2f ha, v2f k, v2f hd, v2f dx, v2f dy) {
    const v2f u = __builtin_elementwise_fma(k, dy, dx);
    return __builtin_elementwise_fma(ha * u, u, (hd * dy) * dy);
}

__device__ __forceinline__ bool box_reachable(float mx, float my, float a, float b, float c, float opacity,
                                              float x0, float x1, float y0, float y1) {
    const float tau = __logf(255.f * opacity) * 1.0002f + 2e-4f;
    if (!(tau > 0.f)) return false;
    const float det = conic_det(a, b, c);
    if (!(det > 0.f) || !(a > 0.f) || !(c > 0.f)) return true;
    const float two_tau = 2.f * tau;
    const float rdet = __builtin_amdgcn_rcpf(det);
    const float hy = __builtin_amdgcn_sqrtf(two_tau * a * rdet) * 1.0004f + 1e-3f;
    float lo = y0 - my, hi = y1 - my;
    if (hi < -hy || lo > hy) return false;
    lo = fmaxf(lo, -hy); hi = fminf(hi, hy);
    const float tta = two_tau * a;
    const float rlo = __builtin_amdgcn_sqrtf(fmaxf(0.f, tta - det * lo * lo));
    const float rhi = __builtin_amdgcn_sqrtf(fmaxf(0.f, tta - det * hi * hi));
    const float hx = __builtin_amdgcn_sqrtf(two_tau * c * rdet);
    const float dys = b * __builtin_amdgcn_sqrtf(two_tau * rdet * __builtin_amdgcn_rcpf(c));
    const float inv_a = __builtin_amdgcn_rcpf(a);
    const float right = (-dys >= lo && -dys <= hi) ? hx : fmaxf((-b * lo + rlo) * inv_a, (-b * hi + rhi) * inv_a);
    const float left = (dys >= lo && dys <= hi) ? -hx : fminf((-b * lo - rlo) * inv_a, (-b * hi - rhi) * inv_a);
    const float eps = 2e-3f + 5e-4f * hx;
    return (mx + right + eps >= x0) && (mx + left - eps <= x1);
}

template <int BANDS>
__device__ __forceinline__ unsigned band_half_mask(float mx, float my, float a, float b, float c, float opacity, float tx0, float ty0) {
    constexpr float BH = (float)(TILE / BANDS);
    const float tau = __logf(255.f * opacity) * 1.0002f + 2e-4f;
    if (!(tau > 0.f)) return 0u;
    const float det = conic_det(a, b, c);
    if (!(det > 0.f) || !(a > 0.f) || !(c > 0.f)) return (1u << (2 * BANDS)) - 1u;
    const float two_tau = 2.f * tau;
    const float rdet = __builtin_amdgcn_rcpf(det);
    const float hy = __builtin_amdgcn_sqrtf(two_tau * a * rdet) * 1.0004f + 1e-3f;
    const float tta = two_tau * a;
    const float hx = __builtin_amdgcn_sqrtf(two_tau * c * rdet);
    const float dys = b * __builtin_amdgcn_sqrtf(two_tau * rdet * __builtin_amdgcn_rcpf(c));
    const float inv_a = __builtin_amdgcn_rcpf(a);
    const float eps = 2e-3f + 5e-4f * hx;
    unsigned m = 0u;
#pragma unroll
    for (int band = 0; band < BANDS; ++band) {
        const float y0 = ty0 + BH * (float)band;
        float lo = y0 - my, hi = (y0 + (BH - 1.f)) - my;
        if (hi < -hy || lo > hy) continue;
        lo = fmaxf(lo, -hy); hi = fminf(hi, hy);
        const float rlo = __builtin_amdgcn_sqrtf(fmaxf(0.f, tta - det * lo * lo));
        const float rhi = __builtin_amdgcn_sqrtf(fmaxf(0.f, tta - det * hi * hi));
        const float right = (-dys >= lo && -dys <= hi) ? hx : fmaxf((-b * lo + rlo) * inv_a, (-b * hi + rhi) * inv_a);
        const float left = (dys >= lo && dys <= hi) ? -hx : fminf((-b * lo - rlo) * inv_a, (-b * hi - rhi) * inv_a);
        const float xr = mx + right + eps, xl = mx + left - eps;
        if (xr >= tx0 && xl <= tx0 + 7.f) m |= 1u << (2 * band);
        if (xr >= tx0 + 8.f && xl <= tx0 + 15.f) m |= 2u << (2 * band);
    }
    return m;
}

#ifndef GSPL_SEG_LOG2
#define GSPL_SEG_LOG2 8
#endif
static constexpr int SEG_LOG2 = GSPL_SEG_LOG2;
static constexpr int SEG = 1 << SEG_LOG2;
static constexpr int SEG_TRIGGER = 3 * SEG;
static constexpr int SEG_TAIL_X2 = 9;
static constexpr int SEG_WALK_SLOTS = 64;
static constexpr int SEG_MAX = 255;
struct SegState {
    float4* ckpt;
    uint32_t* words;
    uint32_t* host_flag;
    uint32_t ticket;
    uint32_t* walk;
    uint4* zero_p;
    uint32_t zero_n16;
    uint32_t slots;
    float* ckpt_x;
    __host__ __device__ uint32_t* count() const { return words; }
    __host__ __device__ uint32_t* work() const { return words + 2; }
};

__device__ __forceinline__ void tile_range(int tile, int n_tiles, int64_t n_isects,
                                           const int32_t* __restrict__ offsets, int& start, int& end) {
    start = offsets[tile];
    end = (tile + 1 < n_tiles || n_isects < 0) ? offsets[tile + 1] : (int)n_isects;
}

struct ListTiles {
    int log2;
    int w;
    int n;
};
static inline ListTiles list_tiles(TileGrid grid) {
    ListTiles lt;
    lt.log2 = grid.size == 8 ? 3 : (grid.size == 32 ? 5 : 4);
    lt.w = grid.w;
    lt.n = grid.n();
    return lt;
}
__device__ __forceinline__ void block_list_range(const ListTiles& lt, int bx, int by, int width, int height, int64_t n_isects,
                                                 const int32_t* __restrict__ offsets, int& start, int& end) {
    if (bx * 8 >= width || by * 8 >= height) { start = end = 0; return; }
    const int t = (by >> (lt.log2 - 3)) * lt.w + (bx >> (lt.log2 - 3));
    start = offsets[t];
    end = (t + 1 < lt.n || n_isects < 0) ? offsets[t + 1] : (int)n_isects;
}

template <int D, bool ABS> struct BwdVals { static constexpr int N = 6 + D + (ABS ? 2 : 0); };

struct CompositeSplats { const float* means2d; const float* conics; const float* colors; const float* opacities; const float* backgrounds; };
struct ImageSize { int width, height; };
struct TileLists { const int32_t* offsets; const int32_t* flatten_ids; int64_t n_isects; };

int check_composite_args(int N, int64_t n_isects, int D, int mode, int layout, ImageSize image, TileGrid grid, const char* who);

int composite_fwd_impl(int N, int D, int mode, int layout, const CompositeSplats& splats, ImageSize image, TileGrid grid, const TileLists& lists,
                       float* out_colors, float* out_alphas, float* final_Ts, int32_t* last_ids, uint8_t* hit_flags, void* stream, const SegState* seg);
int composite_bwd_packed_impl(int N, int D, int mode, int layout, const CompositeSplats& splats, ImageSize image, TileGrid grid, const TileLists& lists,
                              const float* final_Ts, const int32_t* last_ids, const float* v_out_colors, const float* v_out_alphas,
                              float* v_packed, int packed_stride, int absgrad, uint8_t* hit_flags, void* stream, const SegState* seg);

template <class F>
static int dispatch_composite(int D, int mode, int layout, F&& f) {
    auto with_d = [&](auto mode_c, auto chw_c) -> int {
        switch (D) {
            case 1: return f(std::integral_constant<int, 1>{}, mode_c, chw_c);
            case 2: return f(std::integral_constant<int, 2>{}, mode_c, chw_c);
            case 3: return f(std::integral_constant<int, 3>{}, mode_c, chw_c);
            case 4: return f(std::integral_constant<int, 4>{}, mode_c, chw_c);
            case 8: return f(std::integral_constant<int, 8>{}, mode_c, chw_c);
        }
        return GSPL_ERR_UNSUPPORTED;
    };
    return dispatch_bools([&](auto inria, auto chw) { return with_d(std::integral_constant<int, decltype(inria)::value ? GSPL_MODE_INRIA : GSPL_MODE_GSPLAT>{}, chw); },
                          mode != GSPL_MODE_GSPLAT, layout != GSPL_LAYOUT_HWC);
}

struct OrderedScratch { size_t keys, sort_ws, sort_ws_bytes, total; int id_bits; };
OrderedScratch ordered_scratch(int N, int64_t n_isects, int nv);
int ordered_reduce(int N, int64_t n_isects, int nv, const int32_t* flatten_ids, void* block, float* rows, int row_stride, hipStream_t s, const char* who);

}
```

gaussian-splatting-lightning_amd/csrc/gspl_device.h:

```cpp
#pragma once
#include <hip/hip_runtime.h>
#include <stdint.h>

#include "../../include/gspl_hip.h"

namespace gspl {

template <int MODE> struct ModeTraits;
template <> struct ModeTraits<GSPL_MODE_GSPLAT> {
    static constexpr float kAlphaMax = 0.999f;
    static constexpr float kPixelCentre = 0.5f;
    static constexpr bool kStopInclusive = true;
    static constexpr bool kClampKillsGrad = true;
};
template <> struct ModeTraits<GSPL_MODE_INRIA> {
    static constexpr float kAlphaMax = 0.99f;
    static constexpr float kPixelCentre = 0.0f;
    static constexpr bool kStopInclusive = false;
    static constexpr bool kClampKillsGrad = false;
};
static constexpr float kAlphaMin = 1.0f / 255.0f;
static constexpr float kTStop = 1e-4f;

template <int MODE>
// ... 61 lines not shown
    float tx, ty;
    bool  in_x, in_y;
    float ux, uy;
};

__device__ __forceinline__ void ewa_fwd(const float pc[3], const float S6[6], const float W[9],
                                        float fx, float fy, float limx, float limy,
                                        float& a0, float& b0, float& c0, EwaCtx& ctx) {
    const float z = pc[2];
    const float rz = 1.f / z;
    const float txtz = pc[0] * rz, tytz = pc[1] * rz;
    ctx.in_x = (txtz >= -limx) && (txtz <= limx);
    ctx.in_y = (tytz >= -limy) && (tytz <= limy);
    ctx.ux = fminf(limx, fmaxf(-limx, txtz));
    ctx.uy = fminf(limy, fmaxf(-limy, tytz));
    ctx.tx = ctx.ux * z;
    ctx.ty = ctx.uy * z;
    const float J00 = fx * rz, J02 = -fx * ctx.tx * rz * rz;
    const float J11 = fy * rz, J12 = -fy * ctx.ty * rz * rz;
#pragma unroll
    for (int j = 0; j < 3; ++j) {
        ctx.T0[j] = J00 * W[0 * 3 + j] + J02 * W[2 * 3 + j];
        ctx.T1[j] = J11 * W[1 * 3 + j] + J12 * W[2 * 3 + j];
    }
    const float s0x = S6[0] * ctx.T0[0] + S6[1] * ctx.T0[1] + S6[2] * ctx.T0[2];
    const float s0y = S6[1] * ctx.T0[0] + S6[3] * ctx.T0[1] + S6[4] * ctx.T0[2];
    const float s0z = S6[2] * ctx.T0[0] + S6[4] * ctx.T0[1] + S6[5] * ctx.T0[2];
    const float s1x = S6[0] * ctx.T1[0] + S6[1] * ctx.T1[1] + S6[2] * ctx.T1[2];
    const float s1y = S6[1] * ctx.T1[0] + S6[3] * ctx.T1[1] + S6[4] * ctx.T1[2];
    const float s1z = S6[2] * ctx.T1[0] + S6[4] * ctx.T1[1] + S6[5] * ctx.T1[2];
    a0 = ctx.T0[0] * s0x + ctx.T0[1] * s0y + ctx.T0[2] * s0z;
    b0 = ctx.T0[0] * s1x + ctx.T0[1] * s1y + ctx.T0[2] * s1z;
    c0 = ctx.T1[0] * s1x + ctx.T1[1] * s1y + ctx.T1[2] * s1z;
}

template <bool EXACT_CLAMP>
__device__ __forceinline__ void ewa_bwd(const float pc[3], const float S6[6], const float W[9],
                                        float fx, float fy, const EwaCtx& ctx,
                                        float va, float vb, float vc,
                                        float v_pc[3], float G6[6]) {
    const float* T0 = ctx.T0;
    const float* T1 = ctx.T1;
    const float hb = 0.5f * vb;
    G6[0] = va * T0[0] * T0[0] + vb * T0[0] * T1[0] + vc * T1[0] * T1[0];
    G6[3] = va * T0[1] * T0[1] + vb * T0[1] * T1[1] + vc * T1[1] * T1[1];
    G6[5] = va * T0[2] * T0[2] + vb * T0[2] * T1[2] + vc * T1[2] * T1[2];
    G6[1] = va * T0[0] * T0[1] + hb * (T0[0] * T1[1] + T1[0] * T0[1]) + vc * T1[0] * T1[1];
    G6[2] = va * T0[0] * T0[2] + hb * (T0[0] * T1[2] + T1[0] * T0[2]) + vc * T1[0] * T1[2];
    G6[4] = va * T0[1] * T0[2] + hb * (T0[1] * T1[2] + T1[1] * T0[2]) + vc * T1[1] * T1[2];

    const float s0[3] = {S6[0] * T0[0] + S6[1] * T0[1] + S6[2] * T0[2],
                         S6[1] * T0[0] + S6[3] * T0[1] + S6[4] * T0[2],
                         S6[2] * T0[0] + S6[4] * T0[1] + S6[5] * T0[2]};
    const float s1[3] = {S6[0] * T1[0] + S6[1] * T1[1] + S6[2] * T1[2],
                         S6[1] * T1[0] + S6[3] * T1[1] + S6[4] * T1[2],
                         S6[2] * T1[0] + S6[4] * T1[1] + S6[5] * T1[2]};
    float vT0[3], vT1[3];
#pragma unroll
    for (int j = 0; j < 3; ++j) {
        vT0[j] = 2.f * va * s0[j] + vb * s1[j];
        vT1[j] = 2.f * vc * s1[j] + vb * s0[j];
    }
    const float vJ00 = vT0[0] * W[0] + vT0[1] * W[1] + vT0[2] * W[2];
    const float vJ02 = vT0[0] * W[6] + vT0[1] * W[7] + vT0[2] * W[8];
    const float vJ11 = vT1[0] * W[3] + vT1[1] * W[4] + vT1[2] * W[5];
    const float vJ12 = vT1[0] * W[6] + vT1[1] * W[7] + vT1[2] * W[8];

    const float z = pc[2];
    const float rz = 1.f / z, rz2 = rz * rz, rz3 = rz2 * rz;
    float vz = -fx * rz2 * vJ00 - fy * rz2 * vJ11 + 2.f * fx * ctx.tx * rz3 * vJ02 + 2.f * fy * ctx.ty * rz3 * vJ12;
    const float vtx = -fx * rz2 * vJ02;
    const float vty = -fy * rz2 * vJ12;
    if (EXACT_CLAMP) {
        if (ctx.in_x) v_pc[0] += vtx; else vz += vtx * ctx.ux;
        if (ctx.in_y) v_pc[1] += vty; else vz += vty * ctx.uy;
    } else {
        if (ctx.in_x) v_pc[0] += vtx;
        if (ctx.in_y) v_pc[1] += vty;
    }
    v_pc[2] += vz;
}

enum { GSPL_CAM_PINHOLE_ = 0, GSPL_CAM_ORTHO_ = 1, GSPL_CAM_FISHEYE_ = 2 };
static constexpr float FISHEYE_EPS = 1e-7f;

struct FisheyeTerms { float x, y, z, r, x2, y2, xy, s, q, theta, a, b; };

__device__ __forceinline__ void fisheye_terms(const float pc[3], FisheyeTerms& t) {
    t.x = pc[0]; t.y = pc[1]; t.z = pc[2];
    t.r = sqrtf(t.x * t.x + t.y * t.y) + FISHEYE_EPS;
    t.x2 = t.x * t.x + FISHEYE_EPS;
    t.y2 = t.y * t.y;
    t.xy = t.x * t.y;
    t.s = t.x2 + t.y2;
    t.q = 1.f / (t.s + t.z * t.z);
    t.theta = atan2f(t.r, t.z);
    t.b = t.theta / t.r / t.s;
    t.a = t.z * t.q / t.s;
}

template <int CAM>
__device__ __forceinline__ void cam_project(const float pc[3], float fx, float fy, float J[6], float& mx, float& my) {
    if (CAM == GSPL_CAM_ORTHO_) {
        J[0] = fx; J[1] = 0.f; J[2] = 0.f; J[3] = 0.f; J[4] = fy; J[5] = 0.f;
        mx = fx * pc[0]; my = fy * pc[1];
    } else {
        FisheyeTerms t;
        fisheye_terms(pc, t);
        const float thm = atan2f(t.r, t.z + FISHEYE_EPS);
        mx = t.x * fx * thm / t.r;
        my = t.y * fy * thm / t.r;
        J[0] = fx * (t.x2 * t.a + t.y2 * t.b); J[1] = fx * t.xy * (t.a - t.b); J[2] = -fx * t.x * t.q;
        J[3] = fy * t.xy * (t.a - t.b); J[4] = fy * (t.y2 * t.a + t.x2 * t.b); J[5] = -fy * t.y * t.q;
    }
}

template <int CAM>
__device__ __forceinline__ void cam_project_bwd(const float pc[3], float fx, float fy, const float vJ[6], float vmx, float vmy, float v_pc[3]) {
    if (CAM == GSPL_CAM_ORTHO_) {
        v_pc[0] += fx * vmx;
        v_pc[1] += fy * vmy;
        return;
    }
    FisheyeTerms t;
    fisheye_terms(pc, t);
    const float x = t.x, y = t.y, z = t.z, r = t.r;
    const float r0 = fmaxf(r - FISHEYE_EPS, 1e-30f);
    const float drdx = x / r0, drdy = y / r0;
    {
        const float ze = z + FISHEYE_EPS;
        const float den = 1.f / (r * r + ze * ze);
        const float thm = atan2f(r, ze);
        const float g = thm / r;
        const float dg_dr = (ze * den) / r - thm / (r * r);
        const float dg_dz = (-r * den) / r;
        const float wx = fx * vmx, wy = fy * vmy;
        const float common = (wx * x + wy * y) * dg_dr;
        v_pc[0] += wx * g + common * drdx;
        v_pc[1] += wy * g + common * drdy;
        v_pc[2] += (wx * x + wy * y) * dg_dz;
    }
    const float s = t.s, q = t.q, a = t.a, b = t.b, th = t.theta;
    const float den = 1.f / (r * r + z * z);
    const float dth_dr = z * den, dth_dz = -r * den;
    const float dq[3] = {-q * q * 2.f * x, -q * q * 2.f * y, -q * q * 2.f * z};
    const float ds[3] = {2.f * x, 2.f * y, 0.f};
    const float dr[3] = {drdx, drdy, 0.f};
    float da[3], db[3];
#pragma unroll
    for (int k = 0; k < 3; ++k) {
        da[k] = z * dq[k] / s - z * q / (s * s) * ds[k];
        db[k] = dth_dr * dr[k] / (r * s) - th / (r * r * s) * dr[k] - th / (r * s * s) * ds[k];
    }
    da[2] += q / s;
    db[2] += dth_dz / (r * s);
    const float amb = a - b;
    const float dx2[3] = {2.f * x, 0.f, 0.f}, dy2[3] = {0.f, 2.f * y, 0.f}, dxy[3] = {y, x, 0.f};
    const float dxk[3] = {1.f, 0.f, 0.f}, dyk[3] = {0.f, 1.f, 0.f};
#pragma unroll
    for (int k = 0; k < 3; ++k) {
        const float dJ00 = fx * (dx2[k] * a + t.x2 * da[k] + dy2[k] * b + t.y2 * db[k]);
        const float dJ01 = fx * (dxy[k] * amb + t.xy * (da[k] - db[k]));
        const float dJ02 = -fx * (dxk[k] * q + x * dq[k]);
        const float dJ10 = fy * (dxy[k] * amb + t.xy * (da[k] - db[k]));
        const float dJ11 = fy * (dy2[k] * a + t.y2 * da[k] + dx2[k] * b + t.x2 * db[k]);
        const float dJ12 = -fy * (dyk[k] * q + y * dq[k]);
        v_pc[k] += vJ[0] * dJ00 + vJ[1] * dJ01 + vJ[2] * dJ02 + vJ[3] * dJ10 + vJ[4] * dJ11 + vJ[5] * dJ12;
    }
}

__device__ __forceinline__ void ewa_fwd_general(const float J[6], const float S6[6], const float W[9],
                                                float& a0, float& b0, float& c0, float T0[3], float T1[3]) {
#pragma unroll
    for (int j = 0; j < 3; ++j) {
        T0[j] = J[0] * W[0 * 3 + j] + J[1] * W[1 * 3 + j] + J[2] * W[2 * 3 + j];
        T1[j] = J[3] * W[0 * 3 + j] + J[4] * W[1 * 3 + j] + J[5] * W[2 * 3 + j];
    }
    const float s0x = S6[0] * T0[0] + S6[1] * T0[1] + S6[2] * T0[2];
    const float s0y = S6[1] * T0[0] + S6[3] * T0[1] + S6[4] * T0[2];
    const float s0z = S6[2] * T0[0] + S6[4] * T0[1] + S6[5] * T0[2];
    const float s1x = S6[0] * T1[0] + S6[1] * T1[1] + S6[2] * T1[2];
    const float s1y = S6[1] * T1[0] + S6[3] * T1[1] + S6[4] * T1[2];
    const float s1z = S6[2] * T1[0] + S6[4] * T1[1] + S6[5] * T1[2];
    a0 = T0[0] * s0x + T0[1] * s0y + T0[2] * s0z;
    b0 = T0[0] * s1x + T0[1] * s1y + T0[2] * s1z;
    c0 = T1[0] * s1x + T1[1] * s1y + T1[2] * s1z;
}

__device__ __forceinline__ void ewa_bwd_general(const float S6[6], const float W[9], const float T0[3], const float T1[3],
                                                float va, float vb, float vc, float vJ[6], float G6[6]) {
    const float hb = 0.5f * vb;
    G6[0] = va * T0[0] * T0[0] + vb * T0[0] * T1[0] + vc * T1[0] * T1[0];
    G6[3] = va * T0[1] * T0[1] + vb * T0[1] * T1[1] + vc * T1[1] * T1[1];
    G6[5] = va * T0[2] * T0[2] + vb * T0[2] * T1[2] + vc * T1[2] * T1[2];
    G6[1] = va * T0[0] * T0[1] + hb * (T0[0] * T1[1] + T1[0] * T0[1]) + vc * T1[0] * T1[1];
    G6[2] = va * T0[0] * T0[2] + hb * (T0[0] * T1[2] + T1[0] * T0[2]) + vc * T1[0] * T1[2];
    G6[4] = va * T0[1] * T0[2] + hb * (T0[1] * T1[2] + T1[1] * T0[2]) + vc * T1[1] * T1[2];
    const float s0[3] = {S6[0] * T0[0] + S6[1] * T0[1] + S6[2] * T0[2],
                         S6[1] * T0[0] + S6[3] * T0[1] + S6[4] * T0[2],
                         S6[2] * T0[0] + S6[4] * T0[1] + S6[5] * T0[2]};
    const float s1[3] = {S6[0] * T1[0] + S6[1] * T1[1] + S6[2] * T1[2],
                         S6[1] * T1[0] + S6[3] * T1[1] + S6[4] * T1[2],
                         S6[2] * T1[0] + S6[4] * T1[1] + S6[5] * T1[2]};
#pragma unroll
    for (int k = 0; k < 3; ++k) {
        float v0 = 0.f, v1 = 0.f;
#pragma unroll
        for (int j = 0; j < 3; ++j) {
            v0 += (2.f * va * s0[j] + vb * s1[j]) * W[k * 3 + j];
            v1 += (2.f * vc * s1[j] + vb * s0[j]) * W[k * 3 + j];
        }
        vJ[k] = v0;
        vJ[3 + k] = v1;
    }
}

__device__ __forceinline__ void conic_bwd(float a, float b, float c, float vA, float vB, float vC,
                                          float& va, float& vb, float& vc) {
    const float det = a * c - b * b;
    const float rd2 = 1.f / (det * det);
    va = rd2 * (-c * c * vA + b * c * vB - b * b * vC);
    vc = rd2 * (-b * b * vA + a * b * vB - a * a * vC);
    vb = rd2 * (2.f * b * c * vA - (a * c + b * b) * vB + 2.f * a * b * vC);
}

__device__ int gspl_writelane_i32(int value, int lane, int old) __asm("llvm.amdgcn.writelane.i32");
template <int CTRL, int ROW_MASK>
__device__ __forceinline__ float dpp_add(float v) {
    const int moved = __builtin_amdgcn_update_dpp(0, __float_as_int(v), CTRL, ROW_MASK, 0xF, false);
    return v + __int_as_float(moved);
}
__device__ __forceinline__ float row_sum(float v) {
    v = dpp_add<0xB1, 0xF>(v);
    v = dpp_add<0x4E, 0xF>(v);
    v = dpp_add<0x141, 0xF>(v);
    v = dpp_add<0x140, 0xF>(v);
    return v;
}
#define GSPL_DPP_ADD_INPLACE(NAME, CTRL)                                                                         \
    template <int N>                                                                                             \
    __device__ __forceinline__ void NAME(float (&v)[N]) {                                                        \
        int k = 0;                                                                                               \
        _Pragma("unroll") for (; k + 4 <= N; k += 4)                                                             \
            asm volatile("s_nop 1\n\t"                                                                           \
                         "v_add_f32_dpp %0, %0, %0 " CTRL " row_mask:0xf bank_mask:0xf bound_ctrl:1\n\t"         \
                         "v_add_f32_dpp %1, %1, %1 " CTRL " row_mask:0xf bank_mask:0xf bound_ctrl:1\n\t"         \
                         "v_add_f32_dpp %2, %2, %2 " CTRL " row_mask:0xf bank_mask:0xf bound_ctrl:1\n\t"         \
                         "v_add_f32_dpp %3, %3, %3 " CTRL " row_mask:0xf bank_mask:0xf bound_ctrl:1"               \
                         : "+v"(v[k]), "+v"(v[k + 1]), "+v"(v[k + 2]), "+v"(v[k + 3]));                          \
        _Pragma("unroll") for (; k < N; ++k)                                                                     \
            asm volatile("s_nop 1\n\tv_add_f32_dpp %0, %0, %0 " CTRL " row_mask:0xf bank_mask:0xf bound_ctrl:1"  \
                         : "+v"(v[k]));                                                                          \
    }
GSPL_DPP_ADD_INPLACE(row_mirror_add, "row_mirror")
GSPL_DPP_ADD_INPLACE(row_ror8_add, "row_ror:8")
GSPL_DPP_ADD_INPLACE(quad_xor1_add, "quad_perm:[1,0,3,2]")
GSPL_DPP_ADD_INPLACE(quad_xor2_add, "quad_perm:[2,3,0,1]")
GSPL_DPP_ADD_INPLACE(half_mirror_add, "row_half_mirror")

__device__ __forceinline__ float wave_sum_to_lane63(float v) {
    v = dpp_add<0xB1, 0xF>(v);
    v = dpp_add<0x4E, 0xF>(v);
    v = dpp_add<0x141, 0xF>(v);
    v = dpp_add<0x140, 0xF>(v);
    v = dpp_add<0x142, 0xA>(v);
    v = dpp_add<0x143, 0xC>(v);
    return v;
}

__device__ __forceinline__ void zero_table(uint4* __restrict__ p, uint32_t n16) {
    const uint32_t stride = gridDim.x * blockDim.x;
    for (uint32_t i = blockIdx.x * blockDim.x + threadIdx.x; i < n16; i += stride) p[i] = make_uint4(0u, 0u, 0u, 0u);
}

__device__ __forceinline__ float conic_det(float a, float b, float c) {
    const float w = b * b;
    const float e = fmaf(-b, b, w);
    const float f = fmaf(a, c, -w);
    return f + e;
}

struct AdamHyper { float step, b1, b2, inv_bc2, eps; };
struct AdamTarget { float* p; float* m; float* v; AdamHyper h; };
__device__ __forceinline__ void adam_elem(float& p, float g, float& m, float& v, float step, float b1, float b2, float inv_bc2, float eps) {
    m = fmaf(b1, m, (1.f - b1) * g);
    v = fmaf(b2, v, ((1.f - b2) * g) * g);
    p -= (step * m) / fmaf(sqrtf(v), inv_bc2, eps);
}
__device__ __forceinline__ void adam_elem(float& p, float g, float& m, float& v, const AdamHyper& h) {
    adam_elem(p, g, m, v, h.step, h.b1, h.b2, h.inv_bc2, h.eps);
}

#ifndef GSPL_XCD_RUN
#define GSPL_XCD_RUN 32
#endif
__device__ __forceinline__ int xcd_remap(int b, int n, int run = GSPL_XCD_RUN) {
    const int group = 8 * run;
    const int body = (n / group) * group;
    if (b >= body) return b;
    const int x = b & 7, i = b >> 3;
    return ((i / run) * 8 + x) * run + (i % run);
}

}
```

gaussian-splatting-lightning_amd/csrc/gspl_host.h:

```cpp
#pragma once
#include <hip/hip_runtime.h>
#include <type_traits>
#include "../../include/gspl_hip.h"

namespace gspl {

void set_error(const char* where, const char* what);

inline int fail_arg(const char* msg) {
    set_error(msg, "invalid argument");
    return GSPL_ERR_INVALID_ARG;
}
inline int fail_ws(const char* msg) {
    set_error(msg, "workspace too small");
    return GSPL_ERR_WORKSPACE;
}
inline int check_launch(const char* where) {
    const hipError_t e = hipGetLastError();
    if (e != hipSuccess) {
        set_error(where, hipGetErrorString(e));
        return GSPL_ERR_LAUNCH;
    }
    return GSPL_OK;
}
inline int check_hip(hipError_t e, const char* where) {
    if (e != hipSuccess) {
        set_error(where, hipGetErrorString(e));
        return GSPL_ERR_LAUNCH;
    }
    return GSPL_OK;
}

inline size_t up256(size_t x) { return (x + 255) & ~(size_t)255; }

struct Carve {
    size_t off = 0;
    size_t take(size_t bytes) { const size_t o = off; off = up256(off + bytes); return o; }
};

template <class F>
auto dispatch_bools(F&& f) { return f(); }
template <class F, class... Bs>
auto dispatch_bools(F&& f, bool b, Bs... rest) {
    auto bound = [&](auto c) { return dispatch_bools([&](auto... cs) { return f(c, cs...); }, rest...); };
    return b ? bound(std::true_type{}) : bound(std::false_type{});
}

template <class F>
auto dispatch_mode(int mode, F&& f) {
    if (mode == GSPL_MODE_GSPLAT) return f(std::integral_constant<int, GSPL_MODE_GSPLAT>{});
    return f(std::integral_constant<int, GSPL_MODE_INRIA>{});
}

inline int64_t* pinned_words() {
    static thread_local int64_t* p = nullptr;
    if (!p) {
        void* q = nullptr;
        if (hipHostMalloc(&q, 4 * sizeof(int64_t), hipHostMallocDefault) != hipSuccess) { (void)hipGetLastError(); return nullptr; }
        p = (int64_t*)q;
    }
    return p;
}

}

namespace gspl {
struct TileGrid {
    int size, w, h;
    int n() const { return w * h; }
};
inline TileGrid tile_grid16(int width, int height) { return TileGrid{16, (width + 15) / 16, (height + 15) / 16}; }
struct BinSplats { int N, mode; const float* means2d; const int32_t* radii; const float* depths; const float* conics; const float* opacities; };
struct BinOrder { int32_t* order; int64_t* cum; int32_t* big_list; void* spans; };

struct ShCoeffs { const float* dc; int dc_stride; const float* rest; int rest_stride; };
struct ShGrads { float* dc; float* rest; };
inline ShCoeffs sh_coeffs(const float* shs, const float* shs_rest, int n_coeffs) {
    const int stride = 3 * n_coeffs;
    return shs_rest ? ShCoeffs{shs, 3, shs_rest, stride - 3} : ShCoeffs{shs, stride, shs + 3, stride};
}
inline ShGrads sh_grads(float* v_shs, float* v_shs_rest) { return v_shs_rest ? ShGrads{v_shs, v_shs_rest} : ShGrads{v_shs, v_shs + 3}; }

struct InriaCamera {
    const float* viewmatrix; const float* projmatrix; const float* campos;
    int width, height;
    float tanfovx, tanfovy, scale_modifier;
};
struct InriaParams {
    const float* means; const float* scales; const float* quats; const float* cov3d;
    const float* shs; const float* shs_rest;
    int degree, n_coeffs;
};
struct SplatGradRows {
    const float* xy; const float* conic; const float* colour; const float* opacity; int stride;
    static SplatGradRows packed(const float* base, int stride) { return SplatGradRows{base, base + 2, base + 6, base + 5, stride}; }
};
struct InriaGrads {
    float* means; float* scales; float* quats; float* cov3d_precomp; float* shs; float* shs_rest; float* colors_precomp;
    float* means2d_ndc; float* opacities;
};
}

namespace gspl {
int sh_fwd_launch(int N, int C, int degree, const float* dirs, const float* origin, ShCoeffs sh,
                  const uint8_t* mask, const int32_t* mask32, int flags,
                  float* colors, uint8_t* clamped, void* stream, float* jac );
typedef gspl_bwd_adam_tensor ShAdamTargetHost;
struct ShAdamHost { ShAdamTargetHost dc, rest; };
int sh_bwd_launch(int N, int C, int degree, int n_coeffs, const float* dirs, const float* origin, ShCoeffs sh,
                  const uint8_t* mask, const int32_t* mask32, int flags, const uint8_t* clamped,
                  const float* v_colors, int vc_stride, ShGrads v_sh, float* v_dirs, void* stream,
                  const float* jac ,
                  const ShAdamHost* adam ,
                  bool prezeroed = false );
struct ZeroJob { uint4* p = nullptr; uint32_t n16 = 0; };
int bin_count_ticket(const BinSplats& in, TileGrid grid, const BinOrder& ord, int64_t* host_counts,
                     void* workspace, size_t workspace_bytes, void* stream, unsigned long long ticket,
                     bool depth_header_zeroed = false, ZeroJob then_zero = ZeroJob());
int bin_depth_header(int N, int n_tiles, void* count_workspace, ZeroJob& job);
int bin_tile_header(int N, int64_t capacity, int n_tiles, void* workspace, ZeroJob& job);
int bin_emit_impl(const BinSplats& in, const BinOrder& ord, TileGrid grid, int64_t capacity, void* workspace, size_t workspace_bytes, void* stream,
                  bool tile_header_zeroed);
int bin_lists_known(const BinSplats& in, const BinOrder& ord, TileGrid grid, int64_t n_isects, gspl_alloc_fn alloc, void* alloc_ctx,
                    int32_t** flatten_ids, int32_t* offsets, void* stream, const char* who);
struct BwdStats { float* accum = nullptr; float* denom = nullptr; float* max_radii = nullptr; };
int inria_geometry_launch(int N, const InriaParams& p, const InriaCamera& cam, int tile_size,
                          int32_t* radii, float* means2d, float* depths, float* conics, float* cov3d,
                          const float* raw_opacities , float* opacities_out,
                          hipStream_t s, ZeroJob zero = ZeroJob() ,
                          int ext = 0 );
int inria_invdepth_rows_launch(int N, const int32_t* radii, const float* colors3, const float* depths, float* colors4, hipStream_t s);
int inria_preprocess_bwd_impl(int N, const InriaParams& p, const InriaCamera& cam,
                              const int32_t* radii, const uint8_t* clamped, const SplatGradRows& rows, const InriaGrads& v, const float* sh_jac,
                              const float* opac_act , void* stream,
                              const gspl_bwd_adam_plan* adam = nullptr ,
                              BwdStats stats = BwdStats(),
                              int ext = 0 ,
                              uint8_t* grad_rows = nullptr );
}
```

gaussian-splatting-lightning_amd/csrc/inria.hip:

```cpp
#pragma clang fp contract(on)
#include "gspl_device.h"
#include "gspl_host.h"

namespace gspl {

struct InriaCam {
    float V[16];
    float P[16];
};

__device__ __forceinline__ void load_inria_cam(const float* __restrict__ viewmatrix, const float* __restrict__ projmatrix, InriaCam& c) {
#pragma unroll
    for (int i = 0; i < 16; ++i) { c.V[i] = viewmatrix[i]; c.P[i] = projmatrix[i]; }
}

template <int NT>
__device__ __forceinline__ void rows_to_lds(const float* __restrict__ g, int64_t row0, int rows, int W, float* __restrict__ s) {
    const float* base = g + row0 * W;
    const int total = rows * W;
    if ((reinterpret_cast<uintptr_t>(base) & 15) == 0) {
        const int n4 = total >> 2;
        typedef float v4f_ __attribute__((ext_vector_type(4)));
        for (int i = threadIdx.x; i < n4; i += NT) reinterpret_cast<v4f_*>(s)[i] = __builtin_nontemporal_load(reinterpret_cast<const v4f_*>(base) + i);
        for (int i = (n4 << 2) + threadIdx.x; i < total; i += NT) s[i] = base[i];
    } else {
        for (int i = threadIdx.x; i < total; i += NT) s[i] = base[i];
    }
}
template <int NT>
__device__ __forceinline__ void lds_to_rows(float* __restrict__ g, int64_t row0, int rows, int W, const float* __restrict__ s) {
    float* base = g + row0 * W;
    const int total = rows * W;
    if ((reinterpret_cast<uintptr_t>(base) & 15) == 0) {
        const int n4 = total >> 2;
        for (int i = threadIdx.x; i < n4; i += NT) reinterpret_cast<float4*>(base)[i] = reinterpret_cast<const float4*>(s)[i];
        for (int i = (n4 << 2) + threadIdx.x; i < total; i += NT) base[i] = s[i];
    } else {
        for (int i = threadIdx.x; i < total; i += NT) base[i] = s[i];
    }
}

struct InriaGeom {
    float pv[3];
    float hom[4];
    float S6[6];
    float Wstd[9];
    EwaCtx ctx;
    float a, b, c;
    float a0, c0;
    float det;
    float fx, fy;
};

__device__ __forceinline__ bool inria_geom(const InriaCam& cam, const float p[3], const float* S6_in,
                                           int width, int height, float tanfovx, float tanfovy, InriaGeom& G) {
#pragma unroll
    for (int c = 0; c < 3; ++c) G.pv[c] = p[0] * cam.V[0 * 4 + c] + p[1] * cam.V[1 * 4 + c] + p[2] * cam.V[2 * 4 + c] + cam.V[12 + c];
    if (G.pv[2] <= 0.2f) return false;
#pragma unroll
    for (int c = 0; c < 4; ++c) G.hom[c] = p[0] * cam.P[0 * 4 + c] + p[1] * cam.P[1 * 4 + c] + p[2] * cam.P[2 * 4 + c] + cam.P[12 + c];
#pragma unroll
    for (int k = 0; k < 6; ++k) G.S6[k] = S6_in[k];
#pragma unroll
    for (int i = 0; i < 3; ++i)
#pragma unroll
        for (int j = 0; j < 3; ++j) G.Wstd[i * 3 + j] = cam.V[j * 4 + i];
    G.fx = (float)width / (2.f * tanfovx);
    G.fy = (float)height / (2.f * tanfovy);
    float a0, b0, c0;
    ewa_fwd(G.pv, G.S6, G.Wstd, G.fx, G.fy, 1.3f * tanfovx, 1.3f * tanfovy, a0, b0, c0, G.ctx);
    G.a0 = a0; G.c0 = c0;
    G.a = a0 + 0.3f; G.b = b0; G.c = c0 + 0.3f;
    G.det = G.a * G.c - G.b * G.b;
    return G.det != 0.f;
}

__device__ __forceinline__ float act_sigmoid(float x) { return 1.f / (1.f + expf(-x)); }
__device__ __forceinline__ float act_quat_norm(const float q[4]) { return fmaxf(sqrtf(q[0] * q[0] + q[1] * q[1] + q[2] * q[2] + q[3] * q[3]), 1e-12f); }

__device__ __forceinline__ float aa_compensation(const InriaGeom& G, float& ratio) {
    const float det0 = G.a0 * G.c0 - G.b * G.b;
    ratio = det0 / G.det;
    return sqrtf(fmaxf(2.5e-5f, ratio));
}

template <bool RAW, bool AA = false>
__global__ __launch_bounds__(256) void inria_preprocess_fwd_kernel(
    int N,
    const float* __restrict__ means, const float* __restrict__ scales, const float* __restrict__ quats,
    const float* __restrict__ cov3d_precomp,
    const float* __restrict__ viewmatrix, const float* __restrict__ projmatrix,
    int width, int height, int tile_size, float tanfovx, float tanfovy, float scale_modifier,
    int32_t* __restrict__ radii, float* __restrict__ means2d, float* __restrict__ depths,
    float* __restrict__ conics, float* __restrict__ cov3d,
    const float* __restrict__ raw_opacities, float* __restrict__ opacities_out, uint4* __restrict__ zero_p, uint32_t zero_n16) {
    zero_table(zero_p, zero_n16);
    __shared__ __attribute__((aligned(16))) float s_buf[256 * 11];
    const int t = threadIdx.x;
    const int64_t row0 = (int64_t)blockIdx.x * 256;
    const int rows = (int)min((int64_t)256, (int64_t)N - row0);
    const int g = (int)row0 + t;
    float* s_means = s_buf;
    float* s_a = s_buf + 256 * 3;
    float* s_q = s_buf + 256 * 6;
    rows_to_lds<256>(means, row0, rows, 3, s_means);
    if (cov3d_precomp) rows_to_lds<256>(cov3d_precomp, row0, rows, 6, s_a);
    else { rows_to_lds<256>(scales, row0, rows, 3, s_a); rows_to_lds<256>(quats, row0, rows, 4, s_q); }
    __syncthreads();

    float S6[6] = {0.f, 0.f, 0.f, 0.f, 0.f, 0.f};
    int o_radius = 0;
    float o_xy[2] = {0.f, 0.f}, o_depth = 0.f, o_conic[3] = {0.f, 0.f, 0.f};
    float o_comp = 1.f;
    if (t < rows) {
        InriaCam cam;
        load_inria_cam(viewmatrix, projmatrix, cam);
        const float p[3] = {s_means[t * 3 + 0], s_means[t * 3 + 1], s_means[t * 3 + 2]};
        if (cov3d_precomp) {
#pragma unroll
            for (int k = 0; k < 6; ++k) S6[k] = s_a[t * 6 + k];
        } else {
            float s[3] = {s_a[t * 3 + 0], s_a[t * 3 + 1], s_a[t * 3 + 2]};
            const float4 qv = *reinterpret_cast<const float4*>(s_q + t * 4);
            float q[4] = {qv.x, qv.y, qv.z, qv.w};
            if constexpr (RAW) {
#pragma unroll
                for (int j = 0; j < 3; ++j) s[j] = expf(s[j]);
                const float inv = 1.f / act_quat_norm(q);
#pragma unroll
                for (int j = 0; j < 4; ++j) q[j] *= inv;
            }
#pragma unroll
            for (int j = 0; j < 3; ++j) s[j] *= scale_modifier;
            float R[9];
            quat_to_rotmat(q, R);
            cov3d_from_scale_rot(s, R, S6);
        }
        InriaGeom G;
        if (inria_geom(cam, p, S6, width, height, tanfovx, tanfovy, G)) {
            if constexpr (AA) { float ratio; o_comp = aa_compensation(G, ratio); }
            const float inv_det = 1.f / G.det;
            const float mid = 0.5f * (G.a + G.c);
            const float lambda = mid + sqrtf(fmaxf(0.1f, mid * mid - G.det));
            const int radius = (int)ceilf(3.f * sqrtf(lambda));
            const float pw = 1.f / (G.hom[3] + 1e-7f);
            const float x2d = ((G.hom[0] * pw + 1.f) * (float)width - 1.f) * 0.5f;
            const float y2d = ((G.hom[1] * pw + 1.f) * (float)height - 1.f) * 0.5f;
            int minx, miny, maxx, maxy;
            tile_rect<GSPL_MODE_INRIA>(x2d, y2d, radius, tile_size, (width + tile_size - 1) / tile_size, (height + tile_size - 1) / tile_size,
                                       minx, miny, maxx, maxy);
            if ((maxx - minx) * (maxy - miny) > 0) {
                o_radius = radius;
                o_xy[0] = x2d; o_xy[1] = y2d;
                o_depth = G.pv[2];
                o_conic[0] = G.c * inv_det; o_conic[1] = -G.b * inv_det; o_conic[2] = G.a * inv_det;
            }
        }
        radii[g] = o_radius;
        depths[g] = o_depth;
        if constexpr (AA) opacities_out[g] = (RAW ? act_sigmoid(raw_opacities[g]) : raw_opacities[g]) * o_comp;
        else if constexpr (RAW) opacities_out[g] = act_sigmoid(raw_opacities[g]);
    }
    __syncthreads();
    float* s_cov = s_buf;
    float* s_xy = s_buf + 256 * 6;
    float* s_con = s_buf + 256 * 8;
    if (t < rows) {
#pragma unroll
        for (int k = 0; k < 6; ++k) s_cov[t * 6 + k] = S6[k];
        s_xy[t * 2 + 0] = o_xy[0]; s_xy[t * 2 + 1] = o_xy[1];
        s_con[t * 3 + 0] = o_conic[0]; s_con[t * 3 + 1] = o_conic[1]; s_con[t * 3 + 2] = o_conic[2];
    }
    __syncthreads();
    lds_to_rows<256>(cov3d, row0, rows, 6, s_cov);
    lds_to_rows<256>(means2d, row0, rows, 2, s_xy);
    lds_to_rows<256>(conics, row0, rows, 3, s_con);
}

struct PreAdam { AdamTarget means, scales, quats, opac; };
__device__ __forceinline__ void pre_adam_pass(const AdamTarget& T, int64_t base, int total, const float* grad) {
    const int t = threadIdx.x;
    float* gp = T.p + base;
    float* gm = T.m + base;
    float* gv = T.v + base;
    int done = 0;
    if ((((uintptr_t)gp | (uintptr_t)gm | (uintptr_t)gv) & 15u) == 0) {
        const int n4 = total >> 2;
        for (int e4 = t; e4 < n4; e4 += 256) {
            float4 p = reinterpret_cast<const float4*>(gp)[e4], m = reinterpret_cast<const float4*>(gm)[e4], v = reinterpret_cast<const float4*>(gv)[e4];
            const float4 g = reinterpret_cast<const float4*>(grad)[e4];
            adam_elem(p.x, g.x, m.x, v.x, T.h);
            adam_elem(p.y, g.y, m.y, v.y, T.h);
            adam_elem(p.z, g.z, m.z, v.z, T.h);
            adam_elem(p.w, g.w, m.w, v.w, T.h);
            reinterpret_cast<float4*>(gp)[e4] = p;
            reinterpret_cast<float4*>(gm)[e4] = m;
            reinterpret_cast<float4*>(gv)[e4] = v;
        }
        done = n4 << 2;
    }
    for (int e = done + t; e < total; e += 256) {
        float p = gp[e], m = gm[e], v = gv[e];
        adam_elem(p, grad[e], m, v, T.h);
        gp[e] = p; gm[e] = m; gv[e] = v;
    }
}
template <bool ACCUM, bool RAW, bool ADAM = false, bool AA = false, bool INVD = false, bool PREZEROED = false>
__global__ __launch_bounds__(256) void inria_preprocess_bwd_kernel(
    int N,
    const float* means, const float* scales, const float* quats,
    const float* __restrict__ cov3d,
    const float* __restrict__ viewmatrix, const float* __restrict__ projmatrix,
    int width, int height, float tanfovx, float tanfovy, float scale_modifier,
    const int32_t* __restrict__ radii,
    const float* __restrict__ v_means2d, const float* __restrict__ v_conics, int gs2, int gs3,
    float* __restrict__ v_means, float* __restrict__ v_scales, float* __restrict__ v_quats,
    float* __restrict__ v_cov3d_precomp, float* __restrict__ v_means2d_ndc,
    const float* __restrict__ v_opac_src, float* __restrict__ v_opac_dst, const float* __restrict__ opac_act, PreAdam adam, BwdStats stats,
    uint8_t* __restrict__ grad_rows) {
    __shared__ __attribute__((aligned(16))) float s_grad[ADAM ? 256 * 11 : 4];
    int g = blockIdx.x * blockDim.x + threadIdx.x;
    if (!ADAM && !PREZEROED && g >= N) return;
    static_assert(!(ADAM && (AA || INVD)), "the optimizer inside the backward takes neither anti-aliasing nor inverse depth");
    static_assert(!(ADAM && PREZEROED), "the optimizer inside the backward writes no gradient rows");
    if constexpr (PREZEROED) {
        __shared__ int s_rows[256], s_wave[4];
        bool nz = false;
        if (g < N) {
            const float* prow = v_means2d + (int64_t)g * gs2;
            float pv[INVD ? 10 : 9];
#pragma unroll
            for (int k = 0; k < (INVD ? 10 : 9); ++k) pv[k] = prow[k];
            const int32_t radius = radii[g];
            const float denom = stats.accum ? stats.denom[g] : 0.f;
            const float max_radius = (stats.accum && stats.max_radii) ? stats.max_radii[g] : 0.f;
#pragma unroll
            for (int k = 0; k < (INVD ? 10 : 9); ++k) nz = nz || pv[k] != 0.f;
            grad_rows[g] = nz ? 1 : 0;
            if (!nz && stats.accum && radius > 0) {
                stats.denom[g] = denom + 1.f;
                if (stats.max_radii) stats.max_radii[g] = fmaxf(max_radius, (float)radius);
            }
        }
        const unsigned long long mine = __ballot(nz);
        const int lane = threadIdx.x & 63, wave = threadIdx.x >> 6;
        if (lane == 0) s_wave[wave] = __popcll(mine);
        __syncthreads();
        int before = 0, total = 0;
#pragma unroll
        for (int k = 0; k < 4; ++k) { before += k < wave ? s_wave[k] : 0; total += s_wave[k]; }
        if (nz) s_rows[before + __popcll(mine & ((1ull << lane) - 1ull))] = g;
        __syncthreads();
        if ((int)threadIdx.x >= total) return;
        g = s_rows[threadIdx.x];
    }
    const bool row = g < N;
    float aa_g = 0.f, aa_o = 0.f, aa_comp = 1.f;
    if constexpr (AA) { aa_g = v_opac_src[(int64_t)g * gs2]; aa_o = RAW ? act_sigmoid(opac_act[g]) : opac_act[g]; }
    if (!AA && (ADAM || v_opac_dst)) {
        float v = row ? v_opac_src[(int64_t)g * gs2] : 0.f;
        if constexpr (RAW) { const float o = row ? opac_act[g] : 0.f; v *= o * (1.f - o); }
        if constexpr (ADAM) s_grad[256 * 10 + threadIdx.x] = v;
        else v_opac_dst[g] = v;
    }
    float vp[3] = {0.f, 0.f, 0.f}, vs[3] = {0.f, 0.f, 0.f}, vq[4] = {0.f, 0.f, 0.f, 0.f};
    float G6[6] = {0.f, 0.f, 0.f, 0.f, 0.f, 0.f};
    float ndc[2] = {0.f, 0.f};
    if (row && radii[g] > 0) {
        InriaCam cam;
        load_inria_cam(viewmatrix, projmatrix, cam);
        const float p[3] = {means[g * 3 + 0], means[g * 3 + 1], means[g * 3 + 2]};
        float S6[6];
#pragma unroll
        for (int k = 0; k < 6; ++k) S6[k] = cov3d[g * 6 + k];
        InriaGeom G;
        inria_geom(cam, p, S6, width, height, tanfovx, tanfovy, G);

        ndc[0] = v_means2d[(int64_t)g * gs2 + 0] * 0.5f * (float)width;
        ndc[1] = v_means2d[(int64_t)g * gs2 + 1] * 0.5f * (float)height;
        if (stats.accum) {
            stats.accum[g] += sqrtf(fmaf(ndc[0], ndc[0], ndc[1] * ndc[1]));
            stats.denom[g] += 1.f;
            if (stats.max_radii) stats.max_radii[g] = fmaxf(stats.max_radii[g], (float)radii[g]);
        }
        const float mw = 1.f / (G.hom[3] + 1e-7f);
        const float vh0 = ndc[0] * mw, vh1 = ndc[1] * mw;
        const float vh3 = -(ndc[0] * G.hom[0] + ndc[1] * G.hom[1]) * mw * mw;
#pragma unroll
        for (int r = 0; r < 3; ++r) vp[r] = cam.P[r * 4 + 0] * vh0 + cam.P[r * 4 + 1] * vh1 + cam.P[r * 4 + 3] * vh3;

        float va, vb, vc;
        conic_bwd(G.a, G.b, G.c, v_conics[(int64_t)g * gs3 + 0], v_conics[(int64_t)g * gs3 + 1], v_conics[(int64_t)g * gs3 + 2], va, vb, vc);
        if constexpr (AA) {
            float ratio;
            aa_comp = aa_compensation(G, ratio);
            if (ratio > 2.5e-5f) {
                const float k = aa_g * aa_o * 0.5f / aa_comp / G.det;
                va += k * (G.c0 - ratio * G.c);
                vc += k * (G.a0 - ratio * G.a);
                vb += k * 2.f * G.b * (ratio - 1.f);
            }
        }
        float vpv[3] = {0.f, 0.f, 0.f};
        ewa_bwd<false>(G.pv, S6, G.Wstd, G.fx, G.fy, G.ctx, va, vb, vc, vpv, G6);
        if constexpr (INVD) vpv[2] -= v_means2d[(int64_t)g * gs2 + 9] / (G.pv[2] * G.pv[2]);
#pragma unroll
        for (int r = 0; r < 3; ++r) vp[r] += cam.V[r * 4 + 0] * vpv[0] + cam.V[r * 4 + 1] * vpv[1] + cam.V[r * 4 + 2] * vpv[2];

        if (ADAM || v_scales) {
            float s[3] = {scales[g * 3 + 0], scales[g * 3 + 1], scales[g * 3 + 2]};
            float q[4] = {quats[g * 4 + 0], quats[g * 4 + 1], quats[g * 4 + 2], quats[g * 4 + 3]};
            float act_s[3] = {1.f, 1.f, 1.f}, inv_norm = 1.f;
            if constexpr (RAW) {
#pragma unroll
                for (int j = 0; j < 3; ++j) { act_s[j] = expf(s[j]); s[j] = act_s[j]; }
                inv_norm = 1.f / act_quat_norm(q);
#pragma unroll
                for (int j = 0; j < 4; ++j) q[j] *= inv_norm;
            }
#pragma unroll
            for (int j = 0; j < 3; ++j) s[j] *= scale_modifier;
            cov3d_bwd(s, q, G6, vs, vq);
#pragma unroll
            for (int j = 0; j < 3; ++j) vs[j] *= scale_modifier;
            if constexpr (RAW) {
#pragma unroll
                for (int j = 0; j < 3; ++j) vs[j] *= act_s[j];
                const float qv = q[0] * vq[0] + q[1] * vq[1] + q[2] * vq[2] + q[3] * vq[3];
#pragma unroll
                for (int j = 0; j < 4; ++j) vq[j] = (vq[j] - q[j] * qv) * inv_norm;
            }
        }
    }
    if constexpr (ADAM) {
        const int t = threadIdx.x;
#pragma unroll
        for (int j = 0; j < 3; ++j) s_grad[t * 3 + j] = row ? (ACCUM ? v_means[g * 3 + j] + vp[j] : vp[j]) : 0.f;
#pragma unroll
        for (int j = 0; j < 3; ++j) s_grad[256 * 3 + t * 3 + j] = vs[j];
#pragma unroll
        for (int j = 0; j < 4; ++j) s_grad[256 * 6 + t * 4 + j] = vq[j];
        if (row) { v_means2d_ndc[g * 3 + 0] = ndc[0]; v_means2d_ndc[g * 3 + 1] = ndc[1]; v_means2d_ndc[g * 3 + 2] = 0.f; }
        __syncthreads();
        const int n0 = blockIdx.x * 256, rows = min(256, N - n0);
        pre_adam_pass(adam.means, (int64_t)n0 * 3, rows * 3, s_grad);
        pre_adam_pass(adam.scales, (int64_t)n0 * 3, rows * 3, s_grad + 256 * 3);
        pre_adam_pass(adam.quats, (int64_t)n0 * 4, rows * 4, s_grad + 256 * 6);
        pre_adam_pass(adam.opac, (int64_t)n0, rows, s_grad + 256 * 10);
        return;
    }
    if constexpr (AA) {
        float v = aa_g * aa_comp;
        if constexpr (RAW) v *= aa_o * (1.f - aa_o);
        v_opac_dst[g] = v;
    }
#pragma unroll
    for (int j = 0; j < 3; ++j) {
        if (ACCUM) v_means[g * 3 + j] += vp[j];
        else v_means[g * 3 + j] = vp[j];
    }
    if (v_scales) {
#pragma unroll
        for (int j = 0; j < 3; ++j) v_scales[g * 3 + j] = vs[j];
#pragma unroll
        for (int j = 0; j < 4; ++j) v_quats[g * 4 + j] = vq[j];
    }
    if (v_cov3d_precomp) {
        v_cov3d_precomp[g * 6 + 0] = G6[0]; v_cov3d_precomp[g * 6 + 1] = 2.f * G6[1]; v_cov3d_precomp[g * 6 + 2] = 2.f * G6[2];
        v_cov3d_precomp[g * 6 + 3] = G6[3]; v_cov3d_precomp[g * 6 + 4] = 2.f * G6[4]; v_cov3d_precomp[g * 6 + 5] = G6[5];
    }
    v_means2d_ndc[g * 3 + 0] = ndc[0]; v_means2d_ndc[g * 3 + 1] = ndc[1]; v_means2d_ndc[g * 3 + 2] = 0.f;
}

__global__ __launch_bounds__(256) void masked_copy3_kernel(int N, const int32_t* __restrict__ radii,
                                                           const float* __restrict__ src, int src_stride, float* __restrict__ dst,
                                                           uint8_t* __restrict__ clamped) {
    const int g = blockIdx.x * blockDim.x + threadIdx.x;
    if (g >= N) return;
    const bool live = radii[g] > 0;
#pragma unroll
    for (int c = 0; c < 3; ++c) {
        dst[g * 3 + c] = live ? src[(int64_t)g * src_stride + c] : 0.f;
        if (clamped) clamped[g * 3 + c] = 0;
    }
}

__global__ __launch_bounds__(256) void invdepth_rows_kernel(int N, const int32_t* __restrict__ radii, const float* __restrict__ colors3,
                                                            const float* __restrict__ depths, float4* __restrict__ colors4) {
    const int g = blockIdx.x * blockDim.x + threadIdx.x;
    if (g >= N) return;
    const bool live = radii[g] > 0;
    colors4[g] = make_float4(colors3[g * 3 + 0], colors3[g * 3 + 1], colors3[g * 3 + 2], live ? 1.f / depths[g] : 0.f);
}

int inria_invdepth_rows_launch(int N, const int32_t* radii, const float* colors3, const float* depths, float* colors4, hipStream_t s) {
    if (N <= 0) return GSPL_OK;
    hipLaunchKernelGGL(invdepth_rows_kernel, dim3((N + 255) / 256), dim3(256), 0, s, N, radii, colors3, depths, reinterpret_cast<float4*>(colors4));
    return check_launch("inria_invdepth_rows");
}

int inria_geometry_launch(int N, const InriaParams& p, const InriaCamera& cam, int tile_size,
                          int32_t* radii, float* means2d, float* depths, float* conics, float* cov3d,
                          const float* raw_opacities, float* opacities_out, hipStream_t s, ZeroJob zero, int ext) {
    const float* cov3d_precomp = p.cov3d;
    const bool raw = (ext & GSPL_INRIA_RAW_PARAMS) != 0, aa = (ext & GSPL_INRIA_ANTIALIAS) != 0;
    if (aa && (!raw_opacities || !opacities_out || (raw && cov3d_precomp)))
        return fail_arg("inria_preprocess_fwd(antialias): needs the opacities and room for the effective ones (raw: scales + rotations)");
    if (raw && (cov3d_precomp || !raw_opacities || !opacities_out)) return fail_arg("inria_preprocess_fwd: raw parameters need scales + rotations and room for the opacities");
    dispatch_bools([&](auto R, auto AA) {
        hipLaunchKernelGGL((inria_preprocess_fwd_kernel<R(), AA()>), dim3((N + 255) / 256), dim3(256), 0, s,
                           N, p.means, p.scales, p.quats, cov3d_precomp, cam.viewmatrix, cam.projmatrix, cam.width, cam.height, tile_size,
                           cam.tanfovx, cam.tanfovy, cam.scale_modifier, radii, means2d, depths, conics, cov3d, raw_opacities, opacities_out, zero.p, zero.n16);
    }, raw, aa);
    return check_launch("inria_preprocess_fwd");
}

}

extern "C" int gspl_inria_preprocess_fwd(int N, int degree, int n_coeffs,
                                         const float* means, const float* scales, const float* quats,
                                         const float* cov3d_precomp, const float* shs, const float* shs_rest, const float* colors_precomp,
                                         const float* viewmatrix, const float* projmatrix, const float* campos,
                                         int width, int height, int tile_size,
                                         float tanfovx, float tanfovy, float scale_modifier,
                                         int32_t* radii, float* means2d, float* depths, float* conics,
                                         float* colors, uint8_t* clamped, float* cov3d, float* sh_jac, int phases, void* stream) {
    using namespace gspl;
    if (N < 0 || width <= 0 || height <= 0 || tile_size <= 0) return fail_arg("inria_preprocess_fwd: bad sizes");
    if ((phases & ~GSPL_INRIA_ALL) || phases == 0) return fail_arg("inria_preprocess_fwd: bad phases");
    if (N == 0) return GSPL_OK;
    if (!means || !viewmatrix || !projmatrix || !radii || !means2d || !depths || !conics || !colors || !clamped || !cov3d)
        return fail_arg("inria_preprocess_fwd: NULL required pointer");
    if (!cov3d_precomp && (!scales || !quats)) return fail_arg("inria_preprocess_fwd: need scales+quats or cov3d_precomp");
    if (!colors_precomp && (!shs || !campos)) return fail_arg("inria_preprocess_fwd: need shs+campos or colors_precomp");
    if (shs && !colors_precomp && (degree < 0 || degree > 4 || n_coeffs < (degree + 1) * (degree + 1)))
        return fail_arg("inria_preprocess_fwd: bad degree / n_coeffs");
    hipStream_t s = (hipStream_t)stream;
    const int grid = (N + 255) / 256;
    if (phases & GSPL_INRIA_GEOMETRY) {
        int rc = inria_geometry_launch(N, InriaParams{means, scales, quats, cov3d_precomp, shs, shs_rest, degree, n_coeffs},
                                       InriaCamera{viewmatrix, projmatrix, campos, width, height, tanfovx, tanfovy, scale_modifier}, tile_size,
                                       radii, means2d, depths, conics, cov3d, nullptr, nullptr, s);
        if (rc != GSPL_OK) return rc;
    }
    if (!(phases & GSPL_INRIA_COLOURS)) return GSPL_OK;
    if (colors_precomp) {
        hipLaunchKernelGGL(masked_copy3_kernel, dim3(grid), dim3(256), 0, s, N, radii, colors_precomp, 3, colors, clamped);
        return check_launch("inria_preprocess_fwd(colors_precomp)");
    }
    return sh_fwd_launch(N, 1, degree, means, campos, sh_coeffs(shs, shs_rest, n_coeffs), nullptr, radii, GSPL_SH_ADD_HALF_CLAMP, colors, clamped, stream, sh_jac);
}

namespace gspl {
int inria_preprocess_bwd_impl(int N, const InriaParams& p, const InriaCamera& cam,
                              const int32_t* radii, const uint8_t* clamped, const SplatGradRows& rows, const InriaGrads& v, const float* sh_jac,
                              const float* opac_act, void* stream, const gspl_bwd_adam_plan* plan, BwdStats stats, int ext, uint8_t* grad_rows) {
    const float *means = p.means, *scales = p.scales, *quats = p.quats, *cov3d = p.cov3d, *shs = p.shs, *shs_rest = p.shs_rest;
    const int degree = p.degree, n_coeffs = p.n_coeffs, width = cam.width, height = cam.height, grad_stride = rows.stride;
    const float *v_means2d = rows.xy, *v_conics = rows.conic, *v_colors = rows.colour, *v_opacities_packed = rows.opacity;
    float *v_means = v.means, *v_scales = v.scales, *v_quats = v.quats, *v_cov3d_precomp = v.cov3d_precomp, *v_shs = v.shs, *v_shs_rest = v.shs_rest;
    float *v_colors_precomp = v.colors_precomp, *v_means2d_ndc = v.means2d_ndc, *v_opacities = v.opacities;
    if (N < 0 || width <= 0 || height <= 0) return fail_arg("inria_preprocess_bwd: bad sizes");
    if (ext & ~(GSPL_INRIA_RAW_PARAMS | GSPL_INRIA_ANTIALIAS | GSPL_INRIA_INVDEPTH)) return fail_arg("inria_preprocess_bwd: unknown extension bits");
    if ((ext & (GSPL_INRIA_ANTIALIAS | GSPL_INRIA_INVDEPTH)) && plan) return fail_arg("inria_preprocess_bwd(adam): neither anti-aliasing nor inverse depth is supported with the optimizer inside the backward");
    if ((ext & GSPL_INRIA_ANTIALIAS) && (!opac_act || !v_opacities)) return fail_arg("inria_preprocess_bwd(antialias): needs the opacities and v_opacities");
    if ((ext & GSPL_INRIA_INVDEPTH) && grad_stride < 10) return fail_arg("inria_preprocess_bwd(invdepth): needs the packed rows with the 4th colour column");
    if ((stats.accum == nullptr) != (stats.denom == nullptr) || (stats.max_radii && !stats.accum))
        return fail_arg("inria_preprocess_bwd: the statistics' accum and denom go together (max_radii is optional beside them)");
    if (plan) {
        if (!v_shs || !v_scales || !v_quats || !v_opacities || v_cov3d_precomp || v_colors_precomp || grad_stride <= 0)
            return fail_arg("inria_preprocess_bwd(adam): needs SH coefficients, scales + rotations and the packed gradient buffer");
        if (v_scales != scales || v_quats != quats || v_shs != shs || v_shs_rest != shs_rest)
            return fail_arg("inria_preprocess_bwd(adam): the update targets must be the parameters the backward reads");
        const gspl_bwd_adam_tensor* all[6] = {&plan->means, &plan->scales, &plan->rotations, &plan->opacities, &plan->shs, &plan->shs_rest};
        for (int k = 0; k < 6; ++k) {
            if (k == 5 && !shs_rest) continue;
            if (!all[k]->exp_avg || !all[k]->exp_avg_sq || !(all[k]->bias_correction1 > 0.f) || !(all[k]->bias_correction2_sqrt > 0.f))
                return fail_arg("inria_preprocess_bwd(adam): moments missing or bias corrections not positive (1 = none)");
        }
    }
    if (v_opacities && (!v_opacities_packed || grad_stride <= 0)) return fail_arg("inria_preprocess_bwd: v_opacities needs the packed gradient buffer");
    if (grad_rows && (plan || grad_stride < ((ext & GSPL_INRIA_INVDEPTH) ? 10 : 9) || v_conics != v_means2d + 2 || v_colors != v_means2d + 6 ||
                      v_opacities_packed != v_means2d + 5))
        return fail_arg("inria_preprocess_bwd: grad_rows needs the packed gradient rows and no optimizer plan");
    if (N == 0) return GSPL_OK;
    if (!means || !cov3d || !cam.viewmatrix || !cam.projmatrix || !radii || !v_means2d || !v_conics || !v_colors || !v_means || !v_means2d_ndc)
        return fail_arg("inria_preprocess_bwd: NULL required pointer");
    if ((v_scales == nullptr) != (v_quats == nullptr)) return fail_arg("inria_preprocess_bwd: v_scales and v_quats go together");
    if (v_scales && (!scales || !quats)) return fail_arg("inria_preprocess_bwd: scales/quats missing");
    hipStream_t s = (hipStream_t)stream;
    const int grid = (N + 255) / 256;
    const int gs2 = grad_stride > 0 ? grad_stride : 2, gs3 = grad_stride > 0 ? grad_stride : 3;
    bool accum = false;
    if (v_shs) {
        if (!shs || !cam.campos || !clamped) return fail_arg("inria_preprocess_bwd: shs/campos/clamped missing");
        if (degree < 0 || degree > 4 || n_coeffs < (degree + 1) * (degree + 1)) return fail_arg("inria_preprocess_bwd: bad degree / n_coeffs");
        if ((shs_rest == nullptr) != (v_shs_rest == nullptr)) return fail_arg("inria_preprocess_bwd: shs_rest and v_shs_rest go together");
        ShAdamHost sh_adam;
        if (plan) { sh_adam.dc = plan->shs; sh_adam.rest = shs_rest ? plan->shs_rest : plan->shs; }
        const ShAdamHost* sha = plan ? &sh_adam : nullptr;
        int rc = sh_bwd_launch(N, 1, degree, n_coeffs, means, cam.campos, sh_coeffs(shs, shs_rest, n_coeffs), nullptr, radii,
                               GSPL_SH_ADD_HALF_CLAMP, clamped, v_colors, gs3, sh_grads(v_shs, v_shs_rest), v_means, stream, sh_jac, sha, grad_rows != nullptr);
        if (rc != GSPL_OK) return rc;
        accum = true;
    }
    if (v_colors_precomp) {
        hipLaunchKernelGGL(masked_copy3_kernel, dim3(grid), dim3(256), 0, s, N, radii, v_colors, gs3, v_colors_precomp, (uint8_t*)nullptr);
        int rc = check_launch("inria_preprocess_bwd(colors_precomp)");
        if (rc != GSPL_OK) return rc;
    }
    const bool aa = (ext & GSPL_INRIA_ANTIALIAS) != 0, invd = (ext & GSPL_INRIA_INVDEPTH) != 0;
    const bool raw = (ext & GSPL_INRIA_RAW_PARAMS) != 0;
    if (raw && (!opac_act || !v_scales || !v_opacities || v_cov3d_precomp)) return fail_arg("inria_preprocess_bwd: raw parameters need v_scales, v_quats and v_opacities");
    PreAdam pre = {};
    if (plan) {
        auto target = [](float* p, const gspl_bwd_adam_tensor& t) {
            return AdamTarget{p, t.exp_avg, t.exp_avg_sq, AdamHyper{t.lr * (1.f / t.bias_correction1), t.beta1, t.beta2, 1.f / t.bias_correction2_sqrt, t.eps}};
        };
        pre.means = target(const_cast<float*>(means), plan->means);
        pre.scales = target(v_scales, plan->scales);
        pre.quats = target(v_quats, plan->rotations);
        pre.opac = target(v_opacities, plan->opacities);
    }
    dispatch_bools([&](auto A, auto R, auto AD, auto AAF, auto INVDF, auto PZ) {
        if constexpr (!AD() || (A() && !AAF() && !INVDF() && !PZ()))
            hipLaunchKernelGGL((inria_preprocess_bwd_kernel<A(), R(), AD(), AAF(), INVDF(), PZ()>), dim3(grid), dim3(256), 0, s,
                               N, means, scales, quats, cov3d, cam.viewmatrix, cam.projmatrix, width, height, cam.tanfovx, cam.tanfovy, cam.scale_modifier,
                               radii, v_means2d, v_conics, gs2, gs3, v_means, v_scales, v_quats, v_cov3d_precomp, v_means2d_ndc, v_opacities_packed,
                               v_opacities, opac_act, pre, stats, grad_rows);
    }, accum, raw, plan != nullptr, aa, invd, grad_rows != nullptr);
    return check_launch("inria_preprocess_bwd");
}
}

extern "C" int gspl_inria_preprocess_bwd(int N, int degree, int n_coeffs,
                                         const float* means, const float* scales, const float* quats,
                                         const float* cov3d, const float* shs, const float* shs_rest,
                                         const float* viewmatrix, const float* projmatrix, const float* campos,
                                         int width, int height, float tanfovx, float tanfovy, float scale_modifier,
                                         const int32_t* radii, const uint8_t* clamped,
                                         const float* v_means2d, const float* v_conics, const float* v_colors, int grad_stride,
                                         float* v_means, float* v_scales, float* v_quats,
                                         float* v_cov3d_precomp, float* v_shs, float* v_shs_rest, float* v_colors_precomp,
                                         float* v_means2d_ndc, const float* v_opacities_packed, float* v_opacities, const float* sh_jac, void* stream) {
    using namespace gspl;
    return inria_preprocess_bwd_impl(N, InriaParams{means, scales, quats, cov3d, shs, shs_rest, degree, n_coeffs},
                                     InriaCamera{viewmatrix, projmatrix, campos, width, height, tanfovx, tanfovy, scale_modifier}, radii, clamped,
                                     SplatGradRows{v_means2d, v_conics, v_colors, v_opacities_packed, grad_stride},
                                     InriaGrads{v_means, v_scales, v_quats, v_cov3d_precomp, v_shs, v_shs_rest, v_colors_precomp, v_means2d_ndc, v_opacities},
                                     sh_jac, nullptr, stream, nullptr, BwdStats(), 0, nullptr);
}
```

gaussian-splatting-lightning_amd/csrc/sh.hip:

```cpp
#pragma clang fp contract(on)
#include "gspl_device.h"
#include "gspl_host.h"

namespace gspl {

#ifndef GSPL_SH_U
#define GSPL_SH_U 6
#endif
#ifndef GSPL_SH_BLOCK
#define GSPL_SH_BLOCK 256
#endif
#ifndef GSPL_SH_ADAM_U
#define GSPL_SH_ADAM_U 2
#endif
static constexpr int SH_BLOCK = GSPL_SH_BLOCK;
static constexpr int SH_MAX_K = 25;

__device__ __constant__ const float kC0 = 0.28209479177387814f;
__device__ __constant__ const float kC1 = 0.4886025119029199f;

__device__ __forceinline__ void sh_basis(int degree, float x, float y, float z, float* b) {
    b[0] = 0.28209479177387814f;
    if (degree < 1) return;
    b[1] = -0.4886025119029199f * y;
    b[2] = 0.4886025119029199f * z;
    b[3] = -0.4886025119029199f * x;
    if (degree < 2) return;
    const float xx = x * x, yy = y * y, zz = z * z, xy = x * y, yz = y * z, xz = x * z;
    b[4] = 1.0925484305920792f * xy;
    b[5] = -1.0925484305920792f * yz;
    b[6] = 0.31539156525252005f * (2.f * zz - xx - yy);
    b[7] = -1.0925484305920792f * xz;
    b[8] = 0.5462742152960396f * (xx - yy);
    if (degree < 3) return;
    b[9] = -0.5900435899266435f * y * (3.f * xx - yy);
    b[10] = 2.890611442640554f * xy * z;
    b[11] = -0.4570457994644658f * y * (4.f * zz - xx - yy);
    b[12] = 0.3731763325901154f * z * (2.f * zz - 3.f * xx - 3.f * yy);
    b[13] = -0.4570457994644658f * x * (4.f * zz - xx - yy);
    b[14] = 1.445305721320277f * z * (xx - yy);
    b[15] = -0.5900435899266435f * x * (xx - 3.f * yy);
    if (degree < 4) return;
    b[16] = 2.5033429417967046f * xy * (xx - yy);
    b[17] = -1.7701307697799304f * yz * (3.f * xx - yy);
    b[18] = 0.9461746957575601f * xy * (7.f * zz - 1.f);
    b[19] = -0.6690465435572892f * yz * (7.f * zz - 3.f);
    b[20] = 0.10578554691520431f * (zz * (35.f * zz - 30.f) + 3.f);
    b[21] = -0.6690465435572892f * xz * (7.f * zz - 3.f);
    b[22] = 0.47308734787878004f * (xx - yy) * (7.f * zz - 1.f);
    b[23] = -1.7701307697799304f * xz * (xx - 3.f * yy);
    b[24] = 0.6258357354491761f * (xx * (xx - 3.f * yy) - yy * (3.f * xx - yy));
}

__device__ __forceinline__ void sh_basis_grad(int degree, float x, float y, float z, const float* w,
                                              float& gx, float& gy, float& gz) {
    gx = gy = gz = 0.f;
    if (degree < 1) return;
    gy += -0.4886025119029199f * w[1];
    gz += 0.4886025119029199f * w[2];
    gx += -0.4886025119029199f * w[3];
    if (degree < 2) return;
    const float xx = x * x, yy = y * y, zz = z * z, xy = x * y, yz = y * z, xz = x * z;
    { const float c = 1.0925484305920792f * w[4]; gx += c * y; gy += c * x; }
    { const float c = -1.0925484305920792f * w[5]; gy += c * z; gz += c * y; }
    { const float c = 0.31539156525252005f * w[6]; gx += -2.f * c * x; gy += -2.f * c * y; gz += 4.f * c * z; }
    { const float c = -1.0925484305920792f * w[7]; gx += c * z; gz += c * x; }
    { const float c = 0.5462742152960396f * w[8]; gx += 2.f * c * x; gy += -2.f * c * y; }
    if (degree < 3) return;
    { const float c = -0.5900435899266435f * w[9]; gx += c * 6.f * xy; gy += c * (3.f * xx - 3.f * yy); }
    { const float c = 2.890611442640554f * w[10]; gx += c * yz; gy += c * xz; gz += c * xy; }
    { const float c = -0.4570457994644658f * w[11]; gx += c * (-2.f * xy); gy += c * (4.f * zz - xx - 3.f * yy); gz += c * 8.f * yz; }
    { const float c = 0.3731763325901154f * w[12]; gx += c * (-6.f * xz); gy += c * (-6.f * yz); gz += c * (6.f * zz - 3.f * xx - 3.f * yy); }
    { const float c = -0.4570457994644658f * w[13]; gx += c * (4.f * zz - 3.f * xx - yy); gy += c * (-2.f * xy); gz += c * 8.f * xz; }
    { const float c = 1.445305721320277f * w[14]; gx += c * 2.f * xz; gy += c * (-2.f * yz); gz += c * (xx - yy); }
    { const float c = -0.5900435899266435f * w[15]; gx += c * (3.f * xx - 3.f * yy); gy += c * (-6.f * xy); }
    if (degree < 4) return;
    { const float c = 2.5033429417967046f * w[16]; gx += c * (3.f * xx * y - yy * y); gy += c * (xx * x - 3.f * x * yy); }
    { const float c = -1.7701307697799304f * w[17]; gx += c * 6.f * xy * z; gy += c * (3.f * xx * z - 3.f * yy * z); gz += c * (3.f * xx * y - yy * y); }
    { const float c = 0.9461746957575601f * w[18]; gx += c * (7.f * y * zz - y); gy += c * (7.f * x * zz - x); gz += c * 14.f * xy * z; }
    { const float c = -0.6690465435572892f * w[19]; gy += c * (7.f * zz * z - 3.f * z); gz += c * (21.f * y * zz - 3.f * y); }
    { const float c = 0.10578554691520431f * w[20]; gz += c * (140.f * zz * z - 60.f * z); }
    { const float c = -0.6690465435572892f * w[21]; gx += c * (7.f * zz * z - 3.f * z); gz += c * (21.f * x * zz - 3.f * x); }
    { const float c = 0.47308734787878004f * w[22]; gx += c * 2.f * x * (7.f * zz - 1.f); gy += c * (-2.f) * y * (7.f * zz - 1.f); gz += c * 14.f * z * (xx - yy); }
    { const float c = -1.7701307697799304f * w[23]; gx += c * (3.f * xx * z - 3.f * yy * z); gy += c * (-6.f * xy * z); gz += c * (xx * x - 3.f * x * yy); }
    { const float c = 0.6258357354491761f * w[24]; gx += c * (4.f * xx * x - 12.f * x * yy); gy += c * (-12.f * xx * y + 4.f * yy * y); }
}

typedef float sh_v4f __attribute__((ext_vector_type(4)));
__device__ __forceinline__ float4 sh_load16(const float4* p) {
    const sh_v4f t = __builtin_nontemporal_load(reinterpret_cast<const sh_v4f*>(p));
    return make_float4(t.x, t.y, t.z, t.w);
}
__device__ __forceinline__ void sh_store16(float4* p, const float4& q) {
    const sh_v4f t = {q.x, q.y, q.z, q.w};
    __builtin_nontemporal_store(t, reinterpret_cast<sh_v4f*>(p));
}

__device__ __forceinline__ void tile_load(const float* __restrict__ g, int rows, int rs, int ls, float inv_rs,
                                          float* lds, bool vec_ok) {
    const int total = rows * rs;
    const int t = threadIdx.x;
    int done = 0;
    if (vec_ok) {
        const int n4 = total >> 2;
        const float4* g4 = reinterpret_cast<const float4*>(g);
        constexpr int U = GSPL_SH_U;
        for (int b4 = t; b4 < n4; b4 += SH_BLOCK * U) {
            float4 v[U];
#pragma unroll
            for (int u = 0; u < U; ++u) {
                const int e4 = b4 + u * SH_BLOCK;
                v[u] = (e4 < n4) ? sh_load16(g4 + e4) : make_float4(0.f, 0.f, 0.f, 0.f);
            }
#pragma unroll
            for (int u = 0; u < U; ++u) {
                const int e4 = b4 + u * SH_BLOCK;
                if (e4 < n4) {
                    const float vv[4] = {v[u].x, v[u].y, v[u].z, v[u].w};
#pragma unroll
                    for (int k = 0; k < 4; ++k) {
                        const int e = e4 * 4 + k;
                        const int row = (int)(((float)e + 0.5f) * inv_rs);
                        lds[row * ls + (e - row * rs)] = vv[k];
                    }
                }
            }
        }
        done = n4 << 2;
    }
    for (int e = done + t; e < total; e += SH_BLOCK) {
        const int row = (int)(((float)e + 0.5f) * inv_rs);
        lds[row * ls + (e - row * rs)] = g[e];
    }
}
__device__ __forceinline__ void tile_store(float* __restrict__ g, int rows, int rs, int ls, float inv_rs,
                                           const float* lds, bool vec_ok) {
    const int total = rows * rs;
    const int t = threadIdx.x;
    int done = 0;
    if (vec_ok) {
        const int n4 = total >> 2;
        float4* g4 = reinterpret_cast<float4*>(g);
        for (int e4 = t; e4 < n4; e4 += SH_BLOCK) {
            float vv[4];
#pragma unroll
            for (int k = 0; k < 4; ++k) {
                const int e = e4 * 4 + k;
                const int row = (int)(((float)e + 0.5f) * inv_rs);
                vv[k] = lds[row * ls + (e - row * rs)];
            }
            sh_store16(g4 + e4, make_float4(vv[0], vv[1], vv[2], vv[3]));
        }
        done = n4 << 2;
    }
    for (int e = done + t; e < total; e += SH_BLOCK) {
        const int row = (int)(((float)e + 0.5f) * inv_rs);
        g[e] = lds[row * ls + (e - row * rs)];
    }
}

__device__ __forceinline__ void tile_adam(const AdamTarget& T, int64_t base, int rows, int rs, int ls, float inv_rs, const float* lds, bool vec_ok) {
    const int total = rows * rs;
    const int t = threadIdx.x;
    float* __restrict__ gp = T.p + base;
    float* __restrict__ gm = T.m + base;
    float* __restrict__ gv = T.v + base;
    int done = 0;
    if (vec_ok) {
        const int n4 = total >> 2;
        float4* p4 = reinterpret_cast<float4*>(gp);
        float4* m4 = reinterpret_cast<float4*>(gm);
        float4* v4 = reinterpret_cast<float4*>(gv);
        constexpr int U = GSPL_SH_ADAM_U;
        for (int b4 = t; b4 < n4; b4 += U * SH_BLOCK) {
            float4 p[U], m[U], v[U];
#pragma unroll
            for (int u = 0; u < U; ++u) {
                const int e4 = b4 + u * SH_BLOCK;
                if (e4 < n4) { p[u] = sh_load16(p4 + e4); m[u] = sh_load16(m4 + e4); v[u] = sh_load16(v4 + e4); }
            }
#pragma unroll
            for (int u = 0; u < U; ++u) {
                const int e4 = b4 + u * SH_BLOCK;
                if (e4 >= n4) continue;
                float g[4];
#pragma unroll
                for (int k = 0; k < 4; ++k) {
                    const int e = e4 * 4 + k;
                    const int row = (int)(((float)e + 0.5f) * inv_rs);
                    g[k] = lds[row * ls + (e - row * rs)];
                }
                adam_elem(p[u].x, g[0], m[u].x, v[u].x, T.h);
                adam_elem(p[u].y, g[1], m[u].y, v[u].y, T.h);
                adam_elem(p[u].z, g[2], m[u].z, v[u].z, T.h);
                adam_elem(p[u].w, g[3], m[u].w, v[u].w, T.h);
                p4[e4] = p[u];
                sh_store16(m4 + e4, m[u]);
                sh_store16(v4 + e4, v[u]);
            }
        }
        done = n4 << 2;
    }
    for (int e = done + t; e < total; e += SH_BLOCK) {
        const int row = (int)(((float)e + 0.5f) * inv_rs);
        float p = gp[e], m = gm[e], v = gv[e];
        adam_elem(p, lds[row * ls + (e - row * rs)], m, v, T.h);
        gp[e] = p; gm[e] = m; gv[e] = v;
    }
}

struct ShAdam { AdamTarget tile, dc; };

struct ShTile {
    int rs;
    int ls;
    int merged;
};

template <int DEG>
__global__ __launch_bounds__(SH_BLOCK) void sh_fwd_kernel(
    int N, int C,
    const float* __restrict__ dirs, const float* __restrict__ origin,
    const float* __restrict__ dc, int dc_stride, const float* __restrict__ rest,
    const uint8_t* __restrict__ mask, const int32_t* __restrict__ mask32, int flags, ShTile tile, int vec_ok,
    float* __restrict__ colors, uint8_t* __restrict__ clamped, float* __restrict__ jac) {
    extern __shared__ __attribute__((aligned(16))) float lds[];
    const int n0 = blockIdx.x * SH_BLOCK;
    const int rows = min(SH_BLOCK, N - n0);
    constexpr int degree = DEG;
    constexpr int K = (DEG + 1) * (DEG + 1);
    if (degree > 0) {
        const float* base = tile.merged ? dc + (int64_t)n0 * tile.rs : rest + (int64_t)n0 * tile.rs;
        tile_load(base, rows, tile.rs, tile.ls, 1.f / (float)tile.rs, lds, vec_ok != 0);
        __syncthreads();
    }
    const int r = threadIdx.x;
    if (r >= rows) return;
    const int n = n0 + r;
    const float px = dirs[n * 3 + 0], py = dirs[n * 3 + 1], pz = dirs[n * 3 + 2];
    for (int cam = 0; cam < C; ++cam) {
        const int64_t cn = (int64_t)cam * N + n;
        float out[3] = {0.f, 0.f, 0.f};
        uint8_t cl[3] = {0, 0, 0};
        const bool live = ((mask == nullptr) || (mask[cn] != 0)) && ((mask32 == nullptr) || (mask32[cn] > 0));
        if (live) {
            float dx = px, dy = py, dz = pz;
            if (origin) { dx -= origin[cam * 3 + 0]; dy -= origin[cam * 3 + 1]; dz -= origin[cam * 3 + 2]; }
            const float inv = rsqrtf(dx * dx + dy * dy + dz * dz);
            dx *= inv; dy *= inv; dz *= inv;
            float b[K];
            sh_basis(degree, dx, dy, dz, b);
            const float* d0 = (tile.merged && degree > 0) ? (lds + r * tile.ls) : (dc + (int64_t)n * dc_stride);
#pragma unroll
            for (int c = 0; c < 3; ++c) out[c] = b[0] * d0[c];
            const float* row = lds + r * tile.ls + (tile.merged ? 3 : 0);
#pragma unroll
            for (int k = 1; k < K; ++k) {
#pragma unroll
                for (int c = 0; c < 3; ++c) out[c] += b[k] * row[(k - 1) * 3 + c];
            }
            if (flags & GSPL_SH_ADD_HALF_CLAMP) {
#pragma unroll
                for (int c = 0; c < 3; ++c) {
                    out[c] += 0.5f;
                    if (out[c] < 0.f) { out[c] = 0.f; cl[c] = 1; }
                }
            }
            if (jac && degree > 0) {
#pragma unroll
                for (int c = 0; c < 3; ++c) {
                    float w[K];
                    w[0] = 0.f;
#pragma unroll
                    for (int k = 1; k < K; ++k) w[k] = row[(k - 1) * 3 + c];
                    float gx, gy, gz;
                    sh_basis_grad(degree, dx, dy, dz, w, gx, gy, gz);
                    jac[(int64_t)n * 9 + c * 3 + 0] = gx; jac[(int64_t)n * 9 + c * 3 + 1] = gy; jac[(int64_t)n * 9 + c * 3 + 2] = gz;
                }
            }
        }
#pragma unroll
        for (int c = 0; c < 3; ++c) colors[cn * 3 + c] = out[c];
        if (clamped) {
#pragma unroll
            for (int c = 0; c < 3; ++c) clamped[cn * 3 + c] = cl[c];
        }
    }
}

template <int DEG, bool WITH_DIRS, bool ADAM = false, bool PREZEROED = false>
__global__ __launch_bounds__(SH_BLOCK) void sh_bwd_kernel(
    int N, int C, int n_coeffs,
    const float* __restrict__ dirs, const float* __restrict__ origin,
    const float* __restrict__ dc, int dc_stride, const float* __restrict__ rest,
    const uint8_t* __restrict__ mask, const int32_t* __restrict__ mask32, int flags, const uint8_t* __restrict__ clamped,
    const float* __restrict__ v_colors, int vc_stride, ShTile tile, int vec_ok_in, int vec_ok_out,
    float* __restrict__ v_dc, float* __restrict__ v_rest, float* __restrict__ v_dirs, const float* __restrict__ jac, ShAdam adam) {
    extern __shared__ __attribute__((aligned(16))) float lds[];
    const int n0 = blockIdx.x * SH_BLOCK;
    const int rows = min(SH_BLOCK, N - n0);
    constexpr int degree = DEG;
    constexpr int K = (DEG + 1) * (DEG + 1);
    const int r = threadIdx.x;
    const int n = n0 + r;
    const bool has_tile = n_coeffs > 1;

    float vc[3] = {0.f, 0.f, 0.f};
    float dx = 0.f, dy = 0.f, dz = 1.f, inv = 1.f;
    float b[K];
#pragma unroll
    for (int k = 0; k < K; ++k) b[k] = 0.f;
    bool live = false;
    auto load_camera = [&](int cam) {
        const int64_t cn = (int64_t)cam * N + n;
        live = ((mask == nullptr) || (mask[cn] != 0)) && ((mask32 == nullptr) || (mask32[cn] > 0));
#pragma unroll
        for (int c = 0; c < 3; ++c) vc[c] = 0.f;
        if (live) {
#pragma unroll
            for (int c = 0; c < 3; ++c) {
                vc[c] = v_colors[cn * vc_stride + c];
                if ((flags & GSPL_SH_ADD_HALF_CLAMP) && clamped && clamped[cn * 3 + c]) vc[c] = 0.f;
            }
            if constexpr (PREZEROED) live = vc[0] != 0.f || vc[1] != 0.f || vc[2] != 0.f;
        }
        if (live) {
            dx = dirs[n * 3 + 0]; dy = dirs[n * 3 + 1]; dz = dirs[n * 3 + 2];
            if (origin) { dx -= origin[cam * 3 + 0]; dy -= origin[cam * 3 + 1]; dz -= origin[cam * 3 + 2]; }
            inv = rsqrtf(dx * dx + dy * dy + dz * dz);
            dx *= inv; dy *= inv; dz *= inv;
            sh_basis(degree, dx, dy, dz, b);
        }
    };
    if (r < rows) load_camera(0);

    if (WITH_DIRS && jac) {
        if (r < rows) {
            float g[3] = {0.f, 0.f, 0.f};
            if (live && degree > 0) {
                float gx = 0.f, gy = 0.f, gz = 0.f;
#pragma unroll
                for (int c = 0; c < 3; ++c) {
                    gx += vc[c] * jac[(int64_t)n * 9 + c * 3 + 0];
                    gy += vc[c] * jac[(int64_t)n * 9 + c * 3 + 1];
                    gz += vc[c] * jac[(int64_t)n * 9 + c * 3 + 2];
                }
                const float dot = gx * dx + gy * dy + gz * dz;
                g[0] = (gx - dx * dot) * inv; g[1] = (gy - dy * dot) * inv; g[2] = (gz - dz * dot) * inv;
            }
            if (!PREZEROED || live) { v_dirs[n * 3 + 0] = g[0]; v_dirs[n * 3 + 1] = g[1]; v_dirs[n * 3 + 2] = g[2]; }
        }
    } else if (WITH_DIRS) {
        if (degree > 0) {
            const float* base = tile.merged ? dc + (int64_t)n0 * tile.rs : rest + (int64_t)n0 * tile.rs;
            tile_load(base, rows, tile.rs, tile.ls, 1.f / (float)tile.rs, lds, vec_ok_in != 0);
            __syncthreads();
        }
        if (r < rows) {
            float g[3] = {0.f, 0.f, 0.f};
            if (live && degree > 0) {
                float w[K];
                const float* row = lds + r * tile.ls + (tile.merged ? 3 : 0);
                w[0] = 0.f;
#pragma unroll
                for (int k = 1; k < K; ++k)
                    w[k] = row[(k - 1) * 3 + 0] * vc[0] + row[(k - 1) * 3 + 1] * vc[1] + row[(k - 1) * 3 + 2] * vc[2];
                float gx, gy, gz;
                sh_basis_grad(degree, dx, dy, dz, w, gx, gy, gz);
                const float dot = gx * dx + gy * dy + gz * dz;
                g[0] = (gx - dx * dot) * inv; g[1] = (gy - dy * dot) * inv; g[2] = (gz - dz * dot) * inv;
            }
            if (!PREZEROED || live) { v_dirs[n * 3 + 0] = g[0]; v_dirs[n * 3 + 1] = g[1]; v_dirs[n * 3 + 2] = g[2]; }
        }
        __syncthreads();
    }

    if (r < rows && (!PREZEROED || live)) {
        float d0[3];
#pragma unroll
        for (int c = 0; c < 3; ++c) d0[c] = live ? b[0] * vc[c] : 0.f;
        float* row = lds + r * tile.ls;
        const int col0 = (has_tile && tile.merged) ? 3 : 0;
        if (has_tile) {
#pragma unroll
            for (int k = 1; k < K; ++k) {
                const float bk = live ? b[k] : 0.f;
#pragma unroll
                for (int c = 0; c < 3; ++c) row[col0 + (k - 1) * 3 + c] = bk * vc[c];
            }
            for (int j = col0 + (K - 1) * 3; j < col0 + (n_coeffs - 1) * 3; ++j) row[j] = 0.f;
            for (int j = col0 + (n_coeffs - 1) * 3; j < tile.rs; ++j) row[j] = 0.f;
        }
        for (int cam = 1; cam < C; ++cam) {
            load_camera(cam);
            if (!live) continue;
#pragma unroll
            for (int c = 0; c < 3; ++c) d0[c] += b[0] * vc[c];
            if (has_tile) {
#pragma unroll
                for (int k = 1; k < K; ++k) {
#pragma unroll
                    for (int c = 0; c < 3; ++c) row[col0 + (k - 1) * 3 + c] += b[k] * vc[c];
                }
            }
        }
        if (has_tile && tile.merged) { row[0] = d0[0]; row[1] = d0[1]; row[2] = d0[2]; }
        if (!tile.merged || !has_tile) {
            if constexpr (ADAM) {
#pragma unroll
                for (int c = 0; c < 3; ++c) {
                    const int64_t e = (int64_t)n * dc_stride + c;
                    float p = adam.dc.p[e], m = adam.dc.m[e], v = adam.dc.v[e];
                    adam_elem(p, d0[c], m, v, adam.dc.h);
                    adam.dc.p[e] = p; adam.dc.m[e] = m; adam.dc.v[e] = v;
                }
            } else {
#pragma unroll
                for (int c = 0; c < 3; ++c) v_dc[(int64_t)n * dc_stride + c] = d0[c];
            }
        }
    }
    if (has_tile) {
        __syncthreads();
        if constexpr (ADAM) {
            tile_adam(adam.tile, (int64_t)n0 * tile.rs, rows, tile.rs, tile.ls, 1.f / (float)tile.rs, lds, vec_ok_out != 0);
        } else {
            float* base = tile.merged ? v_dc + (int64_t)n0 * tile.rs : v_rest + (int64_t)n0 * tile.rs;
            if constexpr (PREZEROED) {
                static_assert(SH_BLOCK % 64 == 0, "a wave stores the rows its own lanes staged");
                unsigned long long todo = __ballot(r < rows && live);
                const int lane = r & 63, first = r - lane;
                while (todo) {
                    const int row = first + __builtin_ctzll(todo);
                    todo &= todo - 1;
                    for (int c = lane; c < tile.rs; c += 64) base[(int64_t)row * tile.rs + c] = lds[row * tile.ls + c];
                }
            } else {
                tile_store(base, rows, tile.rs, tile.ls, 1.f / (float)tile.rs, lds, vec_ok_out != 0);
            }
        }
    }
}

static inline bool aligned16(const void* p) { return (reinterpret_cast<uintptr_t>(p) & 15u) == 0; }

}

namespace gspl {
int sh_fwd_launch(int N, int C, int degree, const float* dirs, const float* origin, ShCoeffs sh,
                  const uint8_t* mask, const int32_t* mask32, int flags,
                  float* colors, uint8_t* clamped, void* stream, float* jac) {
    const float *dc = sh.dc, *rest = sh.rest;
    const int dc_stride = sh.dc_stride, rest_stride = sh.rest_stride;
    if (N < 0 || C < 1 || degree < 0 || degree > 4) return fail_arg("sh_fwd: bad N/C/degree");
    if (jac && C != 1) return fail_arg("sh_fwd: the direction Jacobian is kept for one camera only");
    if (C > 1 && !origin) return fail_arg("sh_fwd: several cameras need their origins");
    if (N == 0) return GSPL_OK;
    if (!dirs || !dc || !colors || (degree > 0 && !rest)) return fail_arg("sh_fwd: NULL required pointer");
    ShTile tile;
    tile.merged = (degree > 0 && rest == dc + 3 && dc_stride == rest_stride) ? 1 : 0;
    tile.rs = tile.merged ? dc_stride : rest_stride;
    if (degree > 0 && tile.rs < 3 * ((degree + 1) * (degree + 1) - 1) + (tile.merged ? 3 : 0)) return fail_arg("sh_fwd: row stride too small for degree");
    tile.ls = tile.rs | 1;
    const float* base = tile.merged ? dc : rest;
    const int vec_ok = (degree > 0 && aligned16(base)) ? 1 : 0;
    const size_t lds_bytes = degree > 0 ? (size_t)SH_BLOCK * tile.ls * sizeof(float) : 0;
    if (lds_bytes > 160 * 1024) return fail_arg("sh_fwd: coefficient row too long for LDS staging");
    const int grid = (N + SH_BLOCK - 1) / SH_BLOCK;
#define GSPL_SH_FWD(DEG)                                                                                              \
    case DEG: {                                                                                                       \
        if (lds_bytes > 64 * 1024) {                                                                                  \
            hipError_t e = hipFuncSetAttribute(reinterpret_cast<const void*>(sh_fwd_kernel<DEG>),                     \
                                               hipFuncAttributeMaxDynamicSharedMemorySize, (int)lds_bytes);           \
            if (e != hipSuccess) return check_hip(e, "sh_fwd: hipFuncSetAttribute");                                  \
        }                                                                                                             \
        hipLaunchKernelGGL(sh_fwd_kernel<DEG>, dim3(grid), dim3(SH_BLOCK), lds_bytes, (hipStream_t)stream, N, C, dirs, \
                           origin, dc, dc_stride, rest, mask, mask32, flags, tile, vec_ok, colors, clamped, jac);     \
    } break;
    switch (degree) { GSPL_SH_FWD(0) GSPL_SH_FWD(1) GSPL_SH_FWD(2) GSPL_SH_FWD(3) GSPL_SH_FWD(4) }
#undef GSPL_SH_FWD
    return check_launch("sh_fwd");
}
}

extern "C" int gspl_sh_fwd(int N, int degree,
                           const float* dirs, const float* origin,
                           const float* dc, int dc_stride, const float* rest, int rest_stride,
                           const uint8_t* mask, int flags,
                           float* colors, uint8_t* clamped, void* stream) {
    return gspl::sh_fwd_launch(N, 1, degree, dirs, origin, gspl::ShCoeffs{dc, dc_stride, rest, rest_stride}, mask, nullptr, flags, colors, clamped, stream, nullptr);
}

extern "C" int gspl_sh_fwd_batched(int C, int N, int degree,
                                   const float* means, const float* origins,
                                   const float* dc, int dc_stride, const float* rest, int rest_stride,
                                   const int32_t* radii, int flags,
                                   float* colors, uint8_t* clamped, void* stream) {
    return gspl::sh_fwd_launch(N, C, degree, means, origins, gspl::ShCoeffs{dc, dc_stride, rest, rest_stride}, nullptr, radii, flags, colors, clamped, stream, nullptr);
}

namespace gspl {
int sh_bwd_launch(int N, int C, int degree, int n_coeffs, const float* dirs, const float* origin, ShCoeffs sh,
                  const uint8_t* mask, const int32_t* mask32, int flags, const uint8_t* clamped,
                  const float* v_colors, int vc_stride, ShGrads v_sh, float* v_dirs, void* stream, const float* jac, const ShAdamHost* adam_host,
                  bool prezeroed) {
    const float *dc = sh.dc, *rest = sh.rest;
    const int dc_stride = sh.dc_stride, rest_stride = sh.rest_stride;
    float *v_dc = v_sh.dc, *v_rest = v_sh.rest;
    if (N < 0 || C < 1 || degree < 0 || degree > 4 || n_coeffs < (degree + 1) * (degree + 1)) return fail_arg("sh_bwd: bad N/C/degree/n_coeffs");
    ShAdam adam = {};
    if (adam_host) {
        if (C != 1 || !v_dirs) return fail_arg("sh_bwd: the Adam-applying form is the one-camera backward with the direction gradient");
        if (!v_dc || !adam_host->dc.exp_avg || !adam_host->dc.exp_avg_sq || (n_coeffs > 1 && (!v_rest || !adam_host->rest.exp_avg || !adam_host->rest.exp_avg_sq)))
            return fail_arg("sh_bwd: Adam targets missing");
    }
    if (prezeroed && (adam_host || C != 1 || !v_dirs)) return fail_arg("sh_bwd: the form for cleared outputs is the one-camera backward with the direction gradient and no optimizer");
    if (jac && !v_dirs) jac = nullptr;
    if (C > 1 && (v_dirs || !origin)) return fail_arg("sh_bwd: several cameras need their origins and give no direction gradient");
    if (N == 0) return GSPL_OK;
    if (!dirs || !v_colors || !v_dc || (n_coeffs > 1 && !v_rest)) return fail_arg("sh_bwd: NULL required pointer");
    if (v_dirs && !jac && (!dc || (degree > 0 && !rest))) return fail_arg("sh_bwd: v_dirs needs the coefficients (or the forward's Jacobian)");
    ShTile tile;
    tile.merged = (n_coeffs > 1 && v_rest == v_dc + 3 && dc_stride == rest_stride) ? 1 : 0;
    tile.rs = tile.merged ? dc_stride : rest_stride;
    if (n_coeffs > 1 && tile.rs < 3 * (n_coeffs - 1) + (tile.merged ? 3 : 0)) return fail_arg("sh_bwd: row stride too small");
    if (n_coeffs <= 1) tile.rs = 1;
    tile.ls = tile.rs | 1;
    if (v_dirs && !jac && degree > 0) {
        const int in_merged = (rest == dc + 3) ? 1 : 0;
        if (in_merged != tile.merged) return fail_arg("sh_bwd: input/output coefficient layouts differ");
    }
    const float* in_base = tile.merged ? dc : rest;
    float* out_base = tile.merged ? v_dc : v_rest;
    const int vec_in = (in_base && aligned16(in_base)) ? 1 : 0;
    int vec_out = (out_base && aligned16(out_base)) ? 1 : 0;
    if (adam_host) {
        auto target = [](float* p, const ShAdamTargetHost& t) {
            return AdamTarget{p, t.exp_avg, t.exp_avg_sq, AdamHyper{t.lr * (1.f / t.bias_correction1), t.beta1, t.beta2, 1.f / t.bias_correction2_sqrt, t.eps}};
        };
        adam.tile = tile.merged ? target(v_dc, adam_host->dc) : target(v_rest, adam_host->rest);
        adam.dc = target(v_dc, adam_host->dc);
        if (n_coeffs > 1 && !(aligned16(adam.tile.p) && aligned16(adam.tile.m) && aligned16(adam.tile.v))) vec_out = 0;
    }
    const size_t lds_bytes = n_coeffs > 1 ? (size_t)SH_BLOCK * tile.ls * sizeof(float) : 0;
    if (lds_bytes > 160 * 1024) return fail_arg("sh_bwd: coefficient row too long for LDS staging");
    const int grid = (N + SH_BLOCK - 1) / SH_BLOCK;
#define GSPL_SH_BWD(DEG, WD, AD, PZ)                                                                                  \
    {                                                                                                                 \
        if (lds_bytes > 64 * 1024) {                                                                                  \
            hipError_t e = hipFuncSetAttribute(reinterpret_cast<const void*>(sh_bwd_kernel<DEG, WD, AD, PZ>),             \
                                               hipFuncAttributeMaxDynamicSharedMemorySize, (int)lds_bytes);           \
            if (e != hipSuccess) return check_hip(e, "sh_bwd: hipFuncSetAttribute");                                  \
        }                                                                                                             \
        hipLaunchKernelGGL((sh_bwd_kernel<DEG, WD, AD, PZ>), dim3(grid), dim3(SH_BLOCK), lds_bytes, (hipStream_t)stream, N, C, \
                           n_coeffs, dirs, origin, dc, dc_stride, rest, mask, mask32, flags, clamped, v_colors, vc_stride, tile, vec_in, \
                           vec_out, v_dc, v_rest, v_dirs, jac, adam);                                                 \
    }
#define GSPL_SH_BWD_CASE(DEG) \
    case DEG:                 \
        if (adam_host) GSPL_SH_BWD(DEG, true, true, false) else if (prezeroed) GSPL_SH_BWD(DEG, true, false, true)       \
        else if (v_dirs) GSPL_SH_BWD(DEG, true, false, false) else GSPL_SH_BWD(DEG, false, false, false) break;
    switch (degree) { GSPL_SH_BWD_CASE(0) GSPL_SH_BWD_CASE(1) GSPL_SH_BWD_CASE(2) GSPL_SH_BWD_CASE(3) GSPL_SH_BWD_CASE(4) }
#undef GSPL_SH_BWD_CASE
#undef GSPL_SH_BWD
    return check_launch("sh_bwd");
}
}

extern "C" int gspl_sh_bwd(int N, int degree, int n_coeffs,
                           const float* dirs, const float* origin,
                           const float* dc, int dc_stride, const float* rest, int rest_stride,
                           const uint8_t* mask, int flags, const uint8_t* clamped,
                           const float* v_colors, int v_colors_stride,
                           float* v_dc, float* v_rest, float* v_dirs, void* stream) {
    return gspl::sh_bwd_launch(N, 1, degree, n_coeffs, dirs, origin, gspl::ShCoeffs{dc, dc_stride, rest, rest_stride}, mask, nullptr, flags, clamped, v_colors,
                               v_colors_stride > 0 ? v_colors_stride : 3, gspl::ShGrads{v_dc, v_rest}, v_dirs, stream, nullptr, nullptr, false);
}

extern "C" int gspl_sh_bwd_batched(int C, int N, int degree, int n_coeffs,
                                   const float* means, const float* origins,
                                   int dc_stride, int rest_stride,
                                   const int32_t* radii, int flags, const uint8_t* clamped,
                                   const float* v_colors, float* v_dc, float* v_rest, void* stream) {
    return gspl::sh_bwd_launch(N, C, degree, n_coeffs, means, origins, gspl::ShCoeffs{nullptr, dc_stride, nullptr, rest_stride}, nullptr, radii, flags, clamped,
                               v_colors, 3, gspl::ShGrads{v_dc, v_rest}, nullptr, stream, nullptr, nullptr, false);
}
```

Before: 861.4.

## Fold gradient zero-fill into backward composite launch and fuse SH backward into preprocess tail

The gradient zero-fill no longer runs as a separate kernel on a low-priority side stream joined by events. Extra workgroups are prepended to the first backward composite launch to do the fill. The SH backward is also folded into the preprocess backward kernel as a one-launch tail that stages coefficients in LDS. This removes kernel launches and cross-stream event synchronisation, but makes the composite grid larger and the preprocess kernel heavier, with possible pressure on registers and LDS.

```diff
diff --git a/gaussian-splatting-lightning_amd/csrc/composite_bwd.hip b/gaussian-splatting-lightning_amd/csrc/composite_bwd.hip
--- a/gaussian-splatting-lightning_amd/csrc/composite_bwd.hip
+++ b/gaussian-splatting-lightning_amd/csrc/composite_bwd.hip
@@ -17,7 +17,7 @@
 static_assert(B2CHUNK <= B2_NT || B2_NW == 2, "a round is staged by one pass of the workgroup's threads");
 
 
-template <int D, int MODE, bool CHW, bool ABS, bool PACKED, int SEGM = 0>
+template <int D, int MODE, bool CHW, bool ABS, bool PACKED, int SEGM = 0, bool FILL = false>
 __global__ __launch_bounds__(B2_NT, GSPL_BWD2_WAVES) void composite_bwd2_kernel(
     int n_tiles, int tile_w, int width, int height, int64_t n_isects,
     const float* __restrict__ means2d, const float* __restrict__ conics, const float* __restrict__ colors,
@@ -27,10 +27,16 @@
     const float* __restrict__ v_out_colors, const float* __restrict__ v_out_alphas,
     float* __restrict__ v_means2d, float* __restrict__ v_means2d_abs,
     float* __restrict__ v_conics, float* __restrict__ v_colors, float* __restrict__ v_opacities, int packed_stride,
-    uint8_t* __restrict__ hit_flags, SegState seg) {
+    uint8_t* __restrict__ hit_flags, SegState seg, FillJob fill) {
     using TR = ModeTraits<MODE>;
     constexpr int NV = BwdVals<D, ABS>::N;
     constexpr int RS = BwdRec<D>::STRIDE;
+    static_assert(!FILL || SEGM != 2, "the fill rides on the first launch");
+    int block = blockIdx.x;
+    if constexpr (FILL) {
+        if (block < fill.blocks) { zero_fill_body<B2_NT>(fill, (unsigned)block, (unsigned)fill.blocks); return; }
+        block -= fill.blocks;
+    }
     constexpr bool VO_REGS = D <= 4;
     constexpr int SLAB = 2 * P2_SLOTS * 128;
     static_assert(NV <= 16, "one ds_add round per batch");
@@ -47,11 +53,11 @@
     const int ws = w;
     int tile = 0, segidx = 0;
     if constexpr (SEGM == 2) {
-        if (blockIdx.x >= min(*seg.count(), seg.slots)) return;
-        const uint32_t item = seg.work()[blockIdx.x];
+        if ((uint32_t)block >= min(*seg.count(), seg.slots)) return;
+        const uint32_t item = seg.work()[block];
         tile = (int)(item >> 8); segidx = (int)(item & 255u);
     } else {
-        tile = xcd_remap(blockIdx.x, n_tiles);
+        tile = xcd_remap(block, n_tiles);
     }
     {
     const int tx = (tile % tile_w) * TILE, ty = (tile / tile_w) * TILE;
@@ -486,26 +492,41 @@
                       const float* final_Ts, const int32_t* last_ids,
                       const float* v_out_colors, const float* v_out_alphas,
                       float* v_means2d, float* v_means2d_abs, float* v_conics, float* v_colors, float* v_opacities,
-                      hipStream_t s, int packed_stride, uint8_t* hit_flags, ListTiles lt, const SegState* seg_in = nullptr) {
+                      hipStream_t s, int packed_stride, uint8_t* hit_flags, ListTiles lt, const SegState* seg_in = nullptr, const FillJob* fill = nullptr) {
 #define GSPL_BWD_ARGS n_tiles, tile_w, image.width, image.height, lists.n_isects, sp.means2d, sp.conics, sp.colors, sp.opacities, sp.backgrounds, \
                       lists.offsets, lists.flatten_ids, final_Ts, last_ids, v_out_colors, v_out_alphas, v_means2d, v_means2d_abs, v_conics, v_colors, v_opacities,   \
                       packed_stride, hit_flags
+    const FillJob no_fill{};
     if (lt.log2 != 4) {
+        if (fill) return fail_arg("composite_bwd: the fill rides on the 16-pixel kernel only");
         if (absgrad) hipLaunchKernelGGL((composite_bwd_block_kernel<D, MODE, CHW, true, PACKED>), dim3(4 * n_tiles), dim3(64), 0, s, GSPL_BWD_ARGS, lt);
         else hipLaunchKernelGGL((composite_bwd_block_kernel<D, MODE, CHW, false, PACKED>), dim3(4 * n_tiles), dim3(64), 0, s, GSPL_BWD_ARGS, lt);
         return check_launch("composite_bwd");
     }
     SegState plain = {};
     if (seg_in) { plain.host_flag = seg_in->host_flag; plain.walk = seg_in->walk; }
+    constexpr bool CAN_FILL = (D == 3 || D == 4) && MODE == GSPL_MODE_INRIA && CHW && PACKED;
+    if (fill && (!CAN_FILL || absgrad || fill->blocks <= 0 || (fill->blocks & 7)))
+        return fail_arg("composite_bwd: the fill rides on the Inria mode's CHW packed kernel (3 or 4 channels, no absgrad) with a multiple of 8 workgroups");
+    auto first_launch = [&](auto segm, const SegState& sg) {
+        if constexpr (CAN_FILL) {
+            if (fill) {
+                hipLaunchKernelGGL((composite_bwd2_kernel<D, MODE, CHW, false, PACKED, decltype(segm)::value, true>), dim3(n_tiles + fill->blocks), dim3(B2_NT), 0, s,
+                                   GSPL_BWD_ARGS, sg, *fill);
+                return;
+            }
+        }
+        hipLaunchKernelGGL((composite_bwd2_kernel<D, MODE, CHW, false, PACKED, decltype(segm)::value>), dim3(n_tiles), dim3(B2_NT), 0, s, GSPL_BWD_ARGS, sg, no_fill);
+    };
     if constexpr ((D == 3 || (D == 4 && MODE == GSPL_MODE_INRIA)) && CHW && PACKED) {
         if (seg_in && seg_in->ckpt && (D == 3 || seg_in->ckpt_x) && !absgrad && packed_stride > 0) {
-            hipLaunchKernelGGL((composite_bwd2_kernel<D, MODE, CHW, false, PACKED, 1>), dim3(n_tiles), dim3(B2_NT), 0, s, GSPL_BWD_ARGS, *seg_in);
-            hipLaunchKernelGGL((composite_bwd2_kernel<D, MODE, CHW, false, PACKED, 2>), dim3(seg_in->slots), dim3(B2_NT), 0, s, GSPL_BWD_ARGS, *seg_in);
+            first_launch(std::integral_constant<int, 1>{}, *seg_in);
+            hipLaunchKernelGGL((composite_bwd2_kernel<D, MODE, CHW, false, PACKED, 2>), dim3(seg_in->slots), dim3(B2_NT), 0, s, GSPL_BWD_ARGS, *seg_in, no_fill);
             return check_launch("composite_bwd(segmented)");
         }
     }
-    if (absgrad) hipLaunchKernelGGL((composite_bwd2_kernel<D, MODE, CHW, true, PACKED>), dim3(n_tiles), dim3(B2_NT), 0, s, GSPL_BWD_ARGS, plain);
-    else hipLaunchKernelGGL((composite_bwd2_kernel<D, MODE, CHW, false, PACKED>), dim3(n_tiles), dim3(B2_NT), 0, s, GSPL_BWD_ARGS, plain);
+    if (absgrad) hipLaunchKernelGGL((composite_bwd2_kernel<D, MODE, CHW, true, PACKED>), dim3(n_tiles), dim3(B2_NT), 0, s, GSPL_BWD_ARGS, plain, no_fill);
+    else first_launch(std::integral_constant<int, 0>{}, plain);
 #undef GSPL_BWD_ARGS
     return check_launch("composite_bwd");
 }
@@ -616,13 +637,14 @@
 
 int gspl::composite_bwd_packed_impl(int N, int D, int mode, int layout, const CompositeSplats& sp, ImageSize image, TileGrid grid, const TileLists& lists,
                                     const float* final_Ts, const int32_t* last_ids, const float* v_out_colors, const float* v_out_alphas,
-                                    float* v_packed, int packed_stride, int absgrad, uint8_t* hit_flags, void* stream, const SegState* seg) {
+                                    float* v_packed, int packed_stride, int absgrad, uint8_t* hit_flags, void* stream, const SegState* seg,
+                                    const FillJob* fill) {
     using namespace gspl;
     const int64_t n_isects = lists.n_isects;
     int rc = check_composite_args(N, n_isects, D, mode, layout, image, grid, "composite_bwd_packed: bad argument");
     if (rc != GSPL_OK) return rc;
     if (packed_stride < 6 + D + (absgrad ? 2 : 0)) return fail_arg("composite_bwd_packed: packed_stride smaller than the row");
-    if (n_isects == 0 || N == 0) return GSPL_OK;
+    if (n_isects == 0 || N == 0) return fill ? fail_arg("composite_bwd_packed: a fill needs a launch to ride on") : GSPL_OK;
     if (!sp.means2d || !sp.conics || !sp.colors || !sp.opacities || !lists.offsets || !lists.flatten_ids || !final_Ts || !last_ids || !v_out_colors || !v_packed)
         return fail_arg("composite_bwd_packed: NULL required pointer");
     const ListTiles lt = list_tiles(grid);
@@ -646,7 +668,7 @@
     rc = dispatch_composite(D, mode, layout, [&](auto d, auto m, auto chw) {
         return launch_bwd<d(), m(), chw(), true>(ag, n_tiles, ctw, image, sp, lists,
                                                  final_Ts, last_ids, v_out_colors, v_out_alphas, v_packed, nullptr, nullptr, nullptr, nullptr, s, packed_stride,
-                                                 hit_flags, lt, seg);
+                                                 hit_flags, lt, seg, fill);
     });
     if (ordered) {
         if (rc == GSPL_OK) rc = ordered_reduce(N, n_isects, nv, lists.flatten_ids, entries, v_packed_out, packed_stride_out, s, "composite_bwd_packed(ordered reduce)");
diff --git a/gaussian-splatting-lightning_amd/csrc/fused.hip b/gaussian-splatting-lightning_amd/csrc/fused.hip
--- a/gaussian-splatting-lightning_amd/csrc/fused.hip
+++ b/gaussian-splatting-lightning_amd/csrc/fused.hip
@@ -134,13 +134,12 @@
 #ifndef GSPL_EVENT_FLAGS
 #define GSPL_EVENT_FLAGS hipEventDisableTiming
 #endif
-struct FrameEvents { hipEvent_t geo = nullptr, col = nullptr, cnt = nullptr, fork = nullptr, filled = nullptr; bool ok = false; };
+struct FrameEvents { hipEvent_t geo = nullptr, col = nullptr, cnt = nullptr; bool ok = false; };
 static FrameEvents& frame_events() {
     static thread_local FrameEvents ev;
     if (!ev.ok)
         ev.ok = hipEventCreateWithFlags(&ev.geo, GSPL_EVENT_FLAGS) == hipSuccess && hipEventCreateWithFlags(&ev.col, GSPL_EVENT_FLAGS) == hipSuccess &&
-                hipEventCreateWithFlags(&ev.cnt, hipEventDisableTiming) == hipSuccess &&
-                hipEventCreateWithFlags(&ev.fork, GSPL_EVENT_FLAGS) == hipSuccess && hipEventCreateWithFlags(&ev.filled, GSPL_EVENT_FLAGS) == hipSuccess;
+                hipEventCreateWithFlags(&ev.cnt, hipEventDisableTiming) == hipSuccess;
     return ev;
 }
 
@@ -405,55 +404,19 @@
 #define GSPL_FILL_BLOCKS 32
 #endif
 static int fill_blocks() {
-    static const int n = [] { const char* e = getenv("GSPL_FILL_BLOCKS"); const int v = e ? atoi(e) : 0; return v > 0 && v <= 65536 ? v : GSPL_FILL_BLOCKS; }();
+    static const int n = [] { const char* e = getenv("GSPL_FILL_BLOCKS"); const int v = e ? atoi(e) : 0; return ((v > 0 && v <= 65536 ? v : GSPL_FILL_BLOCKS) + 7) & ~7; }();
     return n;
 }
-struct FillJob {
-    struct Span { float* p; uint64_t n; } a[9];
-    int count = 0;
-    void add(float* p, uint64_t n) { if (p && n) a[count++] = Span{p, n}; }
-};
-__global__ __launch_bounds__(256) void zero_fill_kernel(FillJob job) {
-    typedef float v4f __attribute__((ext_vector_type(4)));
-    const uint64_t tid = (uint64_t)blockIdx.x * 256 + threadIdx.x, stride = (uint64_t)gridDim.x * 256;
-    for (int k = 0; k < job.count; ++k) {
-        float* p = job.a[k].p;
-        const uint64_t n = job.a[k].n;
-        const uint64_t head = min(n, (uint64_t)(((16u - (unsigned)((uintptr_t)p & 15u)) & 15u) >> 2));
-        const uint64_t n4 = (n - head) >> 2, tail0 = head + (n4 << 2);
-        v4f* q = reinterpret_cast<v4f*>(p + head);
-        const v4f z = {0.f, 0.f, 0.f, 0.f};
-        for (uint64_t i = tid; i < n4; i += stride) __builtin_nontemporal_store(z, q + i);
-        if (tid < head) p[tid] = 0.f;
-        if (tid < n - tail0) p[tail0 + tid] = 0.f;
-    }
-}
-struct FillJoin {
-    hipStream_t s; hipEvent_t ev = nullptr;
-    explicit FillJoin(hipStream_t st) : s(st) {}
-    FillJoin(const FillJoin&) = delete;
-    void join() { if (ev) (void)hipStreamWaitEvent(s, ev, 0); ev = nullptr; }
-    ~FillJoin() { join(); }
-};
-static int zero_grads_beside(int N, const InriaParams& p, const InriaGrads& v, hipStream_t s, FillJoin& fill) {
+__global__ __launch_bounds__(256) void zero_fill_kernel(FillJob job) { zero_fill_body<256>(job, blockIdx.x, gridDim.x); }
+static FillJob grads_fill_job(int N, const InriaParams& p, const InriaGrads& v) {
     FillJob job;
     const uint64_t n = (uint64_t)N, sh_rows = (uint64_t)(p.n_coeffs > 0 ? p.n_coeffs : 0);
     job.add(v.means, 3 * n); job.add(v.means2d_ndc, 3 * n); job.add(v.opacities, n);
     job.add(v.scales, 3 * n); job.add(v.quats, 4 * n); job.add(v.cov3d_precomp, 6 * n); job.add(v.colors_precomp, 3 * n);
     if (v.shs_rest) { job.add(v.shs, 3 * n); job.add(v.shs_rest, 3 * (sh_rows > 0 ? sh_rows - 1 : 0) * n); }
     else job.add(v.shs, 3 * sh_rows * n);
-    FrameEvents& fe = frame_events();
-    if (!fe.ok) return check_hip(hipGetLastError(), "rasterize_inria_bwd: event");
-    hipStream_t ls = (hipStream_t)gspl_low_priority_stream();
-    const bool side = ls && ls != s;
-    if (side) {
-        (void)hipEventRecord(fe.fork, s);
-        (void)hipStreamWaitEvent(ls, fe.fork, 0);
-    }
-    hipLaunchKernelGGL(zero_fill_kernel, dim3(fill_blocks()), dim3(256), 0, side ? ls : s, job);
-    const int rc = check_launch("rasterize_inria_bwd: clear the gradients");
-    if (side) { (void)hipEventRecord(fe.filled, ls); fill.ev = fe.filled; }
-    return rc;
+    job.blocks = fill_blocks();
+    return job;
 }
 
 static int rasterize_inria_bwd_impl(InriaParams p, const float* opacities, InriaCamera cam, const float* bg,
@@ -471,12 +434,8 @@
     const bool aa = (st->flags & GSPL_INRIA_ANTIALIAS) != 0, invd = (st->flags & GSPL_INRIA_INVDEPTH) != 0;
     const int D = invd ? 4 : 3, prow = invd ? 10 : 9;
     const float* caller_opacities = opacities;
-    FillJoin fill(s);
-    if (grad_rows) {
-        if (plan) return fail_arg("rasterize_inria_bwd: grad_rows and the optimizer inside the backward exclude each other");
-        const int rc = zero_grads_beside(N, p, v, s, fill);
-        if (rc != GSPL_OK) return rc;
-    }
+    if (grad_rows && plan) return fail_arg("rasterize_inria_bwd: grad_rows and the optimizer inside the backward exclude each other");
+    const FillJob fill = grad_rows ? grads_fill_job(N, p, v) : FillJob{};
     if (!(st->flags & GSPL_INRIA_PACKED_READY)) {
         e = hipMemsetAsync(packed, 0, (size_t)N * prow * sizeof(float), s);
         if (e != hipSuccess) return check_hip(e, "rasterize_inria_bwd: clear");
@@ -506,10 +465,13 @@
         const int rc = composite_bwd_packed_impl(N, D, GSPL_MODE_INRIA, GSPL_LAYOUT_CHW, CompositeSplats{st->means2d, st->conics, st->colors, opacities, bg},
                                                  ImageSize{cam.width, cam.height}, tile_grid16(cam.width, cam.height),
                                                  TileLists{st->offsets, st->flatten_ids, st->n_isects}, st->final_Ts, st->last_ids, v_out_color, nullptr,
-                                                 packed, prow, 0, hit_flags, s, &seg);
+                                                 packed, prow, 0, hit_flags, s, &seg, grad_rows ? &fill : nullptr);
         if (rc != GSPL_OK) return rc;
-    }
-    fill.join();
+    } else if (grad_rows) {
+        hipLaunchKernelGGL(zero_fill_kernel, dim3(fill.blocks), dim3(256), 0, s, fill);
+        const int rc = check_launch("rasterize_inria_bwd: clear the gradients");
+        if (rc != GSPL_OK) return rc;
+    }
     return inria_preprocess_bwd_impl(N, p, cam, radii, st->clamped, SplatGradRows::packed(packed, prow), v, st->sh_jac,
                                      aa ? caller_opacities : (raw ? st->opacities : nullptr), s, plan, BwdStats{st->stats_accum, st->stats_denom, st->stats_max_radii},
                                      st->flags & (GSPL_INRIA_RAW_PARAMS | GSPL_INRIA_ANTIALIAS | GSPL_INRIA_INVDEPTH), grad_rows);
diff --git a/gaussian-splatting-lightning_amd/csrc/gspl_composite.h b/gaussian-splatting-lightning_amd/csrc/gspl_composite.h
--- a/gaussian-splatting-lightning_amd/csrc/gspl_composite.h
+++ b/gaussian-splatting-lightning_amd/csrc/gspl_composite.h
@@ -137,6 +137,29 @@
     end = (t + 1 < lt.n || n_isects < 0) ? offsets[t + 1] : (int)n_isects;
 }
 
+struct FillJob {
+    struct Span { float* p; uint64_t n; } a[9];
+    int count = 0;
+    int blocks = 0;
+    void add(float* p, uint64_t n) { if (p && n) a[count++] = Span{p, n}; }
+};
+template <int NT>
+__device__ __forceinline__ void zero_fill_body(const FillJob& job, unsigned block, unsigned blocks) {
+    typedef float v4f __attribute__((ext_vector_type(4)));
+    const uint64_t tid = (uint64_t)block * NT + threadIdx.x, stride = (uint64_t)blocks * NT;
+    for (int k = 0; k < job.count; ++k) {
+        float* p = job.a[k].p;
+        const uint64_t n = job.a[k].n;
+        const uint64_t head = min(n, (uint64_t)(((16u - (unsigned)((uintptr_t)p & 15u)) & 15u) >> 2));
+        const uint64_t n4 = (n - head) >> 2, tail0 = head + (n4 << 2);
+        v4f* q = reinterpret_cast<v4f*>(p + head);
+        const v4f z = {0.f, 0.f, 0.f, 0.f};
+        for (uint64_t i = tid; i < n4; i += stride) __builtin_nontemporal_store(z, q + i);
+        if (tid < head) p[tid] = 0.f;
+        if (tid < n - tail0) p[tail0 + tid] = 0.f;
+    }
+}
+
 template <int D, bool ABS> struct BwdVals { static constexpr int N = 6 + D + (ABS ? 2 : 0); };
 
 struct CompositeSplats { const float* means2d; const float* conics; const float* colors; const float* opacities; const float* backgrounds; };
@@ -149,7 +172,8 @@
                        float* out_colors, float* out_alphas, float* final_Ts, int32_t* last_ids, uint8_t* hit_flags, void* stream, const SegState* seg);
 int composite_bwd_packed_impl(int N, int D, int mode, int layout, const CompositeSplats& splats, ImageSize image, TileGrid grid, const TileLists& lists,
                               const float* final_Ts, const int32_t* last_ids, const float* v_out_colors, const float* v_out_alphas,
-                              float* v_packed, int packed_stride, int absgrad, uint8_t* hit_flags, void* stream, const SegState* seg);
+                              float* v_packed, int packed_stride, int absgrad, uint8_t* hit_flags, void* stream, const SegState* seg,
+                              const FillJob* fill = nullptr);
 
 template <class F>
 static int dispatch_composite(int D, int mode, int layout, F&& f) {
diff --git a/gaussian-splatting-lightning_amd/csrc/gspl_device.h b/gaussian-splatting-lightning_amd/csrc/gspl_device.h
--- a/gaussian-splatting-lightning_amd/csrc/gspl_device.h
+++ b/gaussian-splatting-lightning_amd/csrc/gspl_device.h
@@ -387,4 +387,49 @@
     return ((i / run) * 8 + x) * run + (i % run);
 }
 
-}
+__device__ __forceinline__ void sh_basis(int degree, float x, float y, float z, float* b) {
+    b[0] = 0.28209479177387814f;
+    if (degree < 1) return;
+    b[1] = -0.4886025119029199f * y;
+    b[2] = 0.4886025119029199f * z;
+    b[3] = -0.4886025119029199f * x;
+    if (degree < 2) return;
+    const float xx = x * x, yy = y * y, zz = z * z, xy = x * y, yz = y * z, xz = x * z;
+    b[4] = 1.0925484305920792f * xy;
+    b[5] = -1.0925484305920792f * yz;
+    b[6] = 0.31539156525252005f * (2.f * zz - xx - yy);
+    b[7] = -1.0925484305920792f * xz;
+    b[8] = 0.5462742152960396f * (xx - yy);
+    if (degree < 3) return;
+    b[9] = -0.5900435899266435f * y * (3.f * xx - yy);
+    b[10] = 2.890611442640554f * xy * z;
+    b[11] = -0.4570457994644658f * y * (4.f * zz - xx - yy);
+    b[12] = 0.3731763325901154f * z * (2.f * zz - 3.f * xx - 3.f * yy);
+    b[13] = -0.4570457994644658f * x * (4.f * zz - xx - yy);
+    b[14] = 1.445305721320277f * z * (xx - yy);
+    b[15] = -0.5900435899266435f * x * (xx - 3.f * yy);
+    if (degree < 4) return;
+    b[16] = 2.5033429417967046f * xy * (xx - yy);
+    b[17] = -1.7701307697799304f * yz * (3.f * xx - yy);
+    b[18] = 0.9461746957575601f * xy * (7.f * zz - 1.f);
+    b[19] = -0.6690465435572892f * yz * (7.f * zz - 3.f);
+    b[20] = 0.10578554691520431f * (zz * (35.f * zz - 30.f) + 3.f);
+    b[21] = -0.6690465435572892f * xz * (7.f * zz - 3.f);
+    b[22] = 0.47308734787878004f * (xx - yy) * (7.f * zz - 1.f);
+    b[23] = -1.7701307697799304f * xz * (xx - 3.f * yy);
+    b[24] = 0.6258357354491761f * (xx * (xx - 3.f * yy) - yy * (3.f * xx - yy));
+}
+
+__device__ __forceinline__ void sh_dir_grad_jac(const float* vc, const float* __restrict__ jac, float dx, float dy, float dz, float inv, float* g) {
+    float gx = 0.f, gy = 0.f, gz = 0.f;
+#pragma unroll
+    for (int c = 0; c < 3; ++c) {
+        gx += vc[c] * jac[c * 3 + 0];
+        gy += vc[c] * jac[c * 3 + 1];
+        gz += vc[c] * jac[c * 3 + 2];
+    }
+    const float dot = gx * dx + gy * dy + gz * dz;
+    g[0] = (gx - dx * dot) * inv; g[1] = (gy - dy * dot) * inv; g[2] = (gz - dz * dot) * inv;
+}
+
+}
diff --git a/gaussian-splatting-lightning_amd/csrc/gspl_host.h b/gaussian-splatting-lightning_amd/csrc/gspl_host.h
--- a/gaussian-splatting-lightning_amd/csrc/gspl_host.h
+++ b/gaussian-splatting-lightning_amd/csrc/gspl_host.h
@@ -80,6 +80,19 @@
     return shs_rest ? ShCoeffs{shs, 3, shs_rest, stride - 3} : ShCoeffs{shs, stride, shs + 3, stride};
 }
 inline ShGrads sh_grads(float* v_shs, float* v_shs_rest) { return v_shs_rest ? ShGrads{v_shs, v_shs_rest} : ShGrads{v_shs, v_shs + 3}; }
+struct ShTile {
+    int rs;
+    int ls;
+    int merged;
+};
+inline bool sh_grad_tile(const ShGrads& out, int dc_stride, int rest_stride, int n_coeffs, ShTile& tile) {
+    tile.merged = (n_coeffs > 1 && out.rest == out.dc + 3 && dc_stride == rest_stride) ? 1 : 0;
+    tile.rs = tile.merged ? dc_stride : rest_stride;
+    if (n_coeffs > 1 && tile.rs < 3 * (n_coeffs - 1) + (tile.merged ? 3 : 0)) return false;
+    if (n_coeffs <= 1) tile.rs = 1;
+    tile.ls = tile.rs | 1;
+    return true;
+}
 
 struct InriaCamera {
     const float* viewmatrix; const float* projmatrix; const float* campos;
diff --git a/gaussian-splatting-lightning_amd/csrc/inria.hip b/gaussian-splatting-lightning_amd/csrc/inria.hip
--- a/gaussian-splatting-lightning_amd/csrc/inria.hip
+++ b/gaussian-splatting-lightning_amd/csrc/inria.hip
@@ -205,7 +205,14 @@
         gp[e] = p; gm[e] = m; gv[e] = v;
     }
 }
-template <bool ACCUM, bool RAW, bool ADAM = false, bool AA = false, bool INVD = false, bool PREZEROED = false>
+struct TailSh {
+    const uint8_t* clamped; const float* jac; const float* campos;
+    float* v_dc; float* v_rest;
+    int dc_stride, rs, ls, merged, n_coeffs;
+};
+static constexpr int TAIL_SH_ROWS = 16;
+__device__ __forceinline__ float as_stored(float x) { asm volatile("" : "+v"(x)); return x; }
+template <bool ACCUM, bool RAW, bool ADAM = false, bool AA = false, bool INVD = false, bool PREZEROED = false, int SHDEG = -1>
 __global__ __launch_bounds__(256) void inria_preprocess_bwd_kernel(
     int N,
     const float* means, const float* scales, const float* quats,
@@ -217,9 +224,12 @@
     float* __restrict__ v_means, float* __restrict__ v_scales, float* __restrict__ v_quats,
     float* __restrict__ v_cov3d_precomp, float* __restrict__ v_means2d_ndc,
     const float* __restrict__ v_opac_src, float* __restrict__ v_opac_dst, const float* __restrict__ opac_act, PreAdam adam, BwdStats stats,
-    uint8_t* __restrict__ grad_rows) {
+    uint8_t* __restrict__ grad_rows, TailSh sh) {
+    constexpr bool TAIL = SHDEG >= 0;
+    static_assert(!TAIL || (PREZEROED && ACCUM && !AA && !INVD), "the one-launch tail is the plain sparse frame's");
     __shared__ __attribute__((aligned(16))) float s_grad[ADAM ? 256 * 11 : 4];
     int g = blockIdx.x * blockDim.x + threadIdx.x;
+    bool tail_row = true;
     if (!ADAM && !PREZEROED && g >= N) return;
     static_assert(!(ADAM && (AA || INVD)), "the optimizer inside the backward takes neither anti-aliasing nor inverse depth");
     static_assert(!(ADAM && PREZEROED), "the optimizer inside the backward writes no gradient rows");
@@ -251,8 +261,87 @@
         for (int k = 0; k < 4; ++k) { before += k < wave ? s_wave[k] : 0; total += s_wave[k]; }
         if (nz) s_rows[before + __popcll(mine & ((1ull << lane) - 1ull))] = g;
         __syncthreads();
-        if ((int)threadIdx.x >= total) return;
-        g = s_rows[threadIdx.x];
+        if ((int)(TAIL ? (threadIdx.x & ~63u) : threadIdx.x) >= total) return;
+        tail_row = (int)threadIdx.x < total;
+        if (tail_row) g = s_rows[threadIdx.x];
+    }
+    float vdir[3] = {0.f, 0.f, 0.f};
+    float pre_p[3] = {0.f, 0.f, 0.f}, pre_S6[6] = {0.f, 0.f, 0.f, 0.f, 0.f, 0.f}, pre_s[3] = {0.f, 0.f, 0.f}, pre_q[4] = {0.f, 0.f, 0.f, 0.f};
+    if constexpr (TAIL) {
+        extern __shared__ __attribute__((aligned(16))) float tail_lds[];
+        constexpr int K = (SHDEG + 1) * (SHDEG + 1);
+        const int lane = threadIdx.x & 63, wave = threadIdx.x >> 6;
+        const bool has_tile = sh.n_coeffs > 1;
+        if (tail_row) {
+#pragma unroll
+            for (int k = 0; k < 3; ++k) { pre_p[k] = means[g * 3 + k]; pre_s[k] = scales[g * 3 + k]; }
+#pragma unroll
+            for (int k = 0; k < 6; ++k) pre_S6[k] = cov3d[g * 6 + k];
+#pragma unroll
+            for (int k = 0; k < 4; ++k) pre_q[k] = quats[g * 4 + k];
+        }
+        float vc[3] = {0.f, 0.f, 0.f};
+        float dx = 0.f, dy = 0.f, dz = 1.f, inv = 1.f;
+        float b[K];
+#pragma unroll
+        for (int k = 0; k < K; ++k) b[k] = 0.f;
+        bool live = tail_row && radii[g] > 0;
+        if (live) {
+#pragma unroll
+            for (int c = 0; c < 3; ++c) {
+                vc[c] = v_means2d[(int64_t)g * gs2 + 6 + c];
+                if (sh.clamped[(int64_t)g * 3 + c]) vc[c] = 0.f;
+            }
+            live = vc[0] != 0.f || vc[1] != 0.f || vc[2] != 0.f;
+        }
+        if (live) {
+            dx = pre_p[0]; dy = pre_p[1]; dz = pre_p[2];
+            dx -= sh.campos[0]; dy -= sh.campos[1]; dz -= sh.campos[2];
+            inv = rsqrtf(dx * dx + dy * dy + dz * dz);
+            dx *= inv; dy *= inv; dz *= inv;
+            sh_basis(SHDEG, dx, dy, dz, b);
+            if (SHDEG > 0) sh_dir_grad_jac(vc, sh.jac + (int64_t)g * 9, dx, dy, dz, inv, vdir);
+            float d0[3];
+#pragma unroll
+            for (int c = 0; c < 3; ++c) d0[c] = b[0] * vc[c];
+            if (!sh.merged || !has_tile) {
+#pragma unroll
+                for (int c = 0; c < 3; ++c) sh.v_dc[(int64_t)g * sh.dc_stride + c] = d0[c];
+            }
+        }
+#pragma unroll
+        for (int j = 0; j < 3; ++j) vdir[j] = as_stored(vdir[j]);
+        if (has_tile) {
+            float* wl = tail_lds + wave * (TAIL_SH_ROWS * sh.ls);
+            float* base = sh.merged ? sh.v_dc : sh.v_rest;
+            const int col0 = sh.merged ? 3 : 0;
+            for (int l0 = 0; l0 < 64; l0 += TAIL_SH_ROWS) {
+                const bool mine = live && lane >= l0 && lane < l0 + TAIL_SH_ROWS;
+                unsigned long long todo = __ballot(mine);
+                if (!todo) continue;
+                if (mine) {
+                    float* row = wl + (lane - l0) * sh.ls;
+#pragma unroll
+                    for (int k = 1; k < K; ++k) {
+#pragma unroll
+                        for (int c = 0; c < 3; ++c) row[col0 + (k - 1) * 3 + c] = b[k] * vc[c];
+                    }
+                    for (int j = col0 + (K - 1) * 3; j < sh.rs; ++j) row[j] = 0.f;
+                    if (sh.merged) { row[0] = b[0] * vc[0]; row[1] = b[0] * vc[1]; row[2] = b[0] * vc[2]; }
+                }
+                __builtin_amdgcn_fence(__ATOMIC_RELEASE, "wavefront");
+                __builtin_amdgcn_wave_barrier();
+                while (todo) {
+                    const int src = __builtin_ctzll(todo);
+                    todo &= todo - 1;
+                    const int64_t dst = (int64_t)__shfl(g, src) * sh.rs;
+                    for (int c = lane; c < sh.rs; c += 64) base[dst + c] = wl[(src - l0) * sh.ls + c];
+                }
+                __builtin_amdgcn_fence(__ATOMIC_ACQ_REL, "wavefront");
+                __builtin_amdgcn_wave_barrier();
+            }
+        }
+        if (!tail_row) return;
     }
     const bool row = g < N;
     float aa_g = 0.f, aa_o = 0.f, aa_comp = 1.f;
@@ -269,10 +358,10 @@
     if (row && radii[g] > 0) {
         InriaCam cam;
         load_inria_cam(viewmatrix, projmatrix, cam);
-        const float p[3] = {means[g * 3 + 0], means[g * 3 + 1], means[g * 3 + 2]};
+        const float p[3] = {TAIL ? pre_p[0] : means[g * 3 + 0], TAIL ? pre_p[1] : means[g * 3 + 1], TAIL ? pre_p[2] : means[g * 3 + 2]};
         float S6[6];
 #pragma unroll
-        for (int k = 0; k < 6; ++k) S6[k] = cov3d[g * 6 + k];
+        for (int k = 0; k < 6; ++k) S6[k] = TAIL ? pre_S6[k] : cov3d[g * 6 + k];
         InriaGeom G;
         inria_geom(cam, p, S6, width, height, tanfovx, tanfovy, G);
 
@@ -308,8 +397,11 @@
         for (int r = 0; r < 3; ++r) vp[r] += cam.V[r * 4 + 0] * vpv[0] + cam.V[r * 4 + 1] * vpv[1] + cam.V[r * 4 + 2] * vpv[2];
 
         if (ADAM || v_scales) {
-            float s[3] = {scales[g * 3 + 0], scales[g * 3 + 1], scales[g * 3 + 2]};
-            float q[4] = {quats[g * 4 + 0], quats[g * 4 + 1], quats[g * 4 + 2], quats[g * 4 + 3]};
+            float s[3], q[4];
+#pragma unroll
+            for (int j = 0; j < 3; ++j) s[j] = TAIL ? pre_s[j] : scales[g * 3 + j];
+#pragma unroll
+            for (int j = 0; j < 4; ++j) q[j] = TAIL ? pre_q[j] : quats[g * 4 + j];
             float act_s[3] = {1.f, 1.f, 1.f}, inv_norm = 1.f;
             if constexpr (RAW) {
 #pragma unroll
@@ -356,7 +448,8 @@
     }
 #pragma unroll
     for (int j = 0; j < 3; ++j) {
-        if (ACCUM) v_means[g * 3 + j] += vp[j];
+        if (TAIL) v_means[g * 3 + j] = vdir[j] + vp[j];
+        else if (ACCUM) v_means[g * 3 + j] += vp[j];
         else v_means[g * 3 + j] = vp[j];
     }
     if (v_scales) {
@@ -492,7 +585,22 @@
     const int grid = (N + 255) / 256;
     const int gs2 = grad_stride > 0 ? grad_stride : 2, gs3 = grad_stride > 0 ? grad_stride : 3;
     bool accum = false;
-    if (v_shs) {
+    const bool one_launch = grad_rows && v_shs && sh_jac && v_scales && !v_cov3d_precomp && !v_colors_precomp && degree <= 3 &&
+                            !(ext & (GSPL_INRIA_ANTIALIAS | GSPL_INRIA_INVDEPTH));
+    TailSh tail = {};
+    if (v_shs && one_launch) {
+        if (!shs || !cam.campos || !clamped) return fail_arg("inria_preprocess_bwd: shs/campos/clamped missing");
+        if (degree < 0 || n_coeffs < (degree + 1) * (degree + 1)) return fail_arg("inria_preprocess_bwd: bad degree / n_coeffs");
+        if ((shs_rest == nullptr) != (v_shs_rest == nullptr)) return fail_arg("inria_preprocess_bwd: shs_rest and v_shs_rest go together");
+        const ShCoeffs in = sh_coeffs(shs, shs_rest, n_coeffs);
+        const ShGrads out = sh_grads(v_shs, v_shs_rest);
+        ShTile tile;
+        if (!sh_grad_tile(out, in.dc_stride, in.rest_stride, n_coeffs, tile)) return fail_arg("inria_preprocess_bwd: SH row stride too small");
+        tail.clamped = clamped; tail.jac = sh_jac; tail.campos = cam.campos;
+        tail.v_dc = out.dc; tail.v_rest = out.rest; tail.dc_stride = in.dc_stride; tail.n_coeffs = n_coeffs;
+        tail.merged = tile.merged; tail.rs = tile.rs; tail.ls = tile.ls;
+        accum = true;
+    } else if (v_shs) {
         if (!shs || !cam.campos || !clamped) return fail_arg("inria_preprocess_bwd: shs/campos/clamped missing");
         if (degree < 0 || degree > 4 || n_coeffs < (degree + 1) * (degree + 1)) return fail_arg("inria_preprocess_bwd: bad degree / n_coeffs");
         if ((shs_rest == nullptr) != (v_shs_rest == nullptr)) return fail_arg("inria_preprocess_bwd: shs_rest and v_shs_rest go together");
@@ -522,12 +630,31 @@
         pre.quats = target(v_quats, plan->rotations);
         pre.opac = target(v_opacities, plan->opacities);
     }
+    if (one_launch) {
+        const size_t lds_bytes = (size_t)4 * TAIL_SH_ROWS * tail.ls * sizeof(float);
+        if (lds_bytes > 64 * 1024) return fail_arg("inria_preprocess_bwd: coefficient row too long for LDS staging");
+        auto launch = [&](auto R, auto DEG) {
+            hipLaunchKernelGGL((inria_preprocess_bwd_kernel<true, R(), false, false, false, true, DEG()>), dim3(grid), dim3(256), lds_bytes, s,
+                               N, means, scales, quats, cov3d, cam.viewmatrix, cam.projmatrix, width, height, cam.tanfovx, cam.tanfovy, cam.scale_modifier,
+                               radii, v_means2d, v_conics, gs2, gs3, v_means, v_scales, v_quats, v_cov3d_precomp, v_means2d_ndc, v_opacities_packed,
+                               v_opacities, opac_act, pre, stats, grad_rows, tail);
+        };
+        dispatch_bools([&](auto R) {
+            switch (degree) {
+                case 0: launch(R, std::integral_constant<int, 0>{}); break;
+                case 1: launch(R, std::integral_constant<int, 1>{}); break;
+                case 2: launch(R, std::integral_constant<int, 2>{}); break;
+                default: launch(R, std::integral_constant<int, 3>{}); break;
+            }
+        }, raw);
+        return check_launch("inria_preprocess_bwd(one-launch tail)");
+    }
     dispatch_bools([&](auto A, auto R, auto AD, auto AAF, auto INVDF, auto PZ) {
         if constexpr (!AD() || (A() && !AAF() && !INVDF() && !PZ()))
             hipLaunchKernelGGL((inria_preprocess_bwd_kernel<A(), R(), AD(), AAF(), INVDF(), PZ()>), dim3(grid), dim3(256), 0, s,
                                N, means, scales, quats, cov3d, cam.viewmatrix, cam.projmatrix, width, height, cam.tanfovx, cam.tanfovy, cam.scale_modifier,
                                radii, v_means2d, v_conics, gs2, gs3, v_means, v_scales, v_quats, v_cov3d_precomp, v_means2d_ndc, v_opacities_packed,
-                               v_opacities, opac_act, pre, stats, grad_rows);
+                               v_opacities, opac_act, pre, stats, grad_rows, TailSh{});
     }, accum, raw, plan != nullptr, aa, invd, grad_rows != nullptr);
     return check_launch("inria_preprocess_bwd");
 }
diff --git a/gaussian-splatting-lightning_amd/csrc/sh.hip b/gaussian-splatting-lightning_amd/csrc/sh.hip
--- a/gaussian-splatting-lightning_amd/csrc/sh.hip
+++ b/gaussian-splatting-lightning_amd/csrc/sh.hip
@@ -19,38 +19,6 @@
 __device__ __constant__ const float kC0 = 0.28209479177387814f;
 __device__ __constant__ const float kC1 = 0.4886025119029199f;
 
-__device__ __forceinline__ void sh_basis(int degree, float x, float y, float z, float* b) {
-    b[0] = 0.28209479177387814f;
-    if (degree < 1) return;
-    b[1] = -0.4886025119029199f * y;
-    b[2] = 0.4886025119029199f * z;
-    b[3] = -0.4886025119029199f * x;
-    if (degree < 2) return;
-    const float xx = x * x, yy = y * y, zz = z * z, xy = x * y, yz = y * z, xz = x * z;
-    b[4] = 1.0925484305920792f * xy;
-    b[5] = -1.0925484305920792f * yz;
-    b[6] = 0.31539156525252005f * (2.f * zz - xx - yy);
-    b[7] = -1.0925484305920792f * xz;
-    b[8] = 0.5462742152960396f * (xx - yy);
-    if (degree < 3) return;
-    b[9] = -0.5900435899266435f * y * (3.f * xx - yy);
-    b[10] = 2.890611442640554f * xy * z;
-    b[11] = -0.4570457994644658f * y * (4.f * zz - xx - yy);
-    b[12] = 0.3731763325901154f * z * (2.f * zz - 3.f * xx - 3.f * yy);
-    b[13] = -0.4570457994644658f * x * (4.f * zz - xx - yy);
-    b[14] = 1.445305721320277f * z * (xx - yy);
-    b[15] = -0.5900435899266435f * x * (xx - 3.f * yy);
-    if (degree < 4) return;
-    b[16] = 2.5033429417967046f * xy * (xx - yy);
-    b[17] = -1.7701307697799304f * yz * (3.f * xx - yy);
-    b[18] = 0.9461746957575601f * xy * (7.f * zz - 1.f);
-    b[19] = -0.6690465435572892f * yz * (7.f * zz - 3.f);
-    b[20] = 0.10578554691520431f * (zz * (35.f * zz - 30.f) + 3.f);
-    b[21] = -0.6690465435572892f * xz * (7.f * zz - 3.f);
-    b[22] = 0.47308734787878004f * (xx - yy) * (7.f * zz - 1.f);
-    b[23] = -1.7701307697799304f * xz * (xx - 3.f * yy);
-    b[24] = 0.6258357354491761f * (xx * (xx - 3.f * yy) - yy * (3.f * xx - yy));
-}
 
 __device__ __forceinline__ void sh_basis_grad(int degree, float x, float y, float z, const float* w,
                                               float& gx, float& gy, float& gz) {
@@ -211,11 +179,6 @@
 
 struct ShAdam { AdamTarget tile, dc; };
 
-struct ShTile {
-    int rs;
-    int ls;
-    int merged;
-};
 
 template <int DEG>
 __global__ __launch_bounds__(SH_BLOCK) void sh_fwd_kernel(
@@ -338,15 +301,7 @@
         if (r < rows) {
             float g[3] = {0.f, 0.f, 0.f};
             if (live && degree > 0) {
-                float gx = 0.f, gy = 0.f, gz = 0.f;
-#pragma unroll
-                for (int c = 0; c < 3; ++c) {
-                    gx += vc[c] * jac[(int64_t)n * 9 + c * 3 + 0];
-                    gy += vc[c] * jac[(int64_t)n * 9 + c * 3 + 1];
-                    gz += vc[c] * jac[(int64_t)n * 9 + c * 3 + 2];
-                }
-                const float dot = gx * dx + gy * dy + gz * dz;
-                g[0] = (gx - dx * dot) * inv; g[1] = (gy - dy * dot) * inv; g[2] = (gz - dz * dot) * inv;
+                sh_dir_grad_jac(vc, jac + (int64_t)n * 9, dx, dy, dz, inv, g);
             }
             if (!PREZEROED || live) { v_dirs[n * 3 + 0] = g[0]; v_dirs[n * 3 + 1] = g[1]; v_dirs[n * 3 + 2] = g[2]; }
         }
@@ -521,11 +476,7 @@
     if (!dirs || !v_colors || !v_dc || (n_coeffs > 1 && !v_rest)) return fail_arg("sh_bwd: NULL required pointer");
     if (v_dirs && !jac && (!dc || (degree > 0 && !rest))) return fail_arg("sh_bwd: v_dirs needs the coefficients (or the forward's Jacobian)");
     ShTile tile;
-    tile.merged = (n_coeffs > 1 && v_rest == v_dc + 3 && dc_stride == rest_stride) ? 1 : 0;
-    tile.rs = tile.merged ? dc_stride : rest_stride;
-    if (n_coeffs > 1 && tile.rs < 3 * (n_coeffs - 1) + (tile.merged ? 3 : 0)) return fail_arg("sh_bwd: row stride too small");
-    if (n_coeffs <= 1) tile.rs = 1;
-    tile.ls = tile.rs | 1;
+    if (!sh_grad_tile(v_sh, dc_stride, rest_stride, n_coeffs, tile)) return fail_arg("sh_bwd: row stride too small");
     if (v_dirs && !jac && degree > 0) {
         const int in_merged = (rest == dc + 3) ? 1 : 0;
         if (in_merged != tile.merged) return fail_arg("sh_bwd: input/output coefficient layouts differ");
```

New measurement: 888.9, median of 6. +3.2%, better.
